# xianlopez/optical_flow

Measured on AMD Instinct MI355X. Metric: image-pairs/sec training, 384x512 batch=8 per GPU, higher is better.
Workload: dtype fp32

## Files before the change

include/oflow.h:

```cpp
#ifndef OFLOW_H
#define OFLOW_H

#include <stddef.h>
#include <stdint.h>

#ifdef __cplusplus
extern "C" {
#endif

#define OF_ABI_VERSION 1

enum { OF_OK = 0, OF_EINVAL = 1, OF_EHIP = 2, OF_EUNSUPPORTED = 3, OF_ETIMEOUT = 4 };
enum { OF_ACT_NONE = 0, OF_ACT_RELU = 1, OF_ACT_LEAKY = 2 };

typedef struct of_conv_desc {
  int32_t n, h, w;
  int32_t cin;
  int32_t cin_p;
  int32_t cout;
  int32_t kh, kw, stride;
  int32_t pad_top, pad_left;
  int32_t ho, wo;
} of_conv_desc;

int         of_abi_version(void);
const char* of_last_error(void);
int of_same_pads(int n, int k, int s, int* before, int* after, int* out);

int64_t of_conv_wfwd_elems(const of_conv_desc* d);
int64_t of_conv_wbwd_elems(const of_conv_desc* d);
int of_conv_pack_weights(const of_conv_desc* d, const float* w_hwio, float* w_fwd,
                         float* w_bwd, void* stream);

size_t of_conv_pack_table_bytes(int nconv);
int of_conv_pack_table(int nconv, const of_conv_desc* descs, const float* const* w_hwio,
                       float* const* w_fwd, float* const* w_bwd, void* host_table);
int of_conv_pack_many(const void* dev_table, int64_t total_work, void* stream);

size_t of_conv2d_fwd_workspace(const of_conv_desc* d);
int of_conv2d_fwd(const of_conv_desc* d, const float* x, int ldx, const float* w_fwd,
                  const float* bias, const float* bn_gamma, const float* bn_beta,
                  const float* bn_mean, const float* bn_var, float bn_eps,
                  const float* residual, int ldr, int act, float alpha,
                  float* z, int ldz, float* y, int ldy, void* workspace, size_t ws_bytes,
                  void* stream);


size_t of_conv2d_dgrad_workspace(const of_conv_desc* d);
int of_conv2d_dgrad(const of_conv_desc* d, const float* dy, int lddy, const float* w_bwd,
                    const float* act_src, int ld_act, int act, float alpha,
                    float* dx, int lddx, void* workspace, size_t ws_bytes, void* stream);

size_t of_conv2d_wgrad_workspace(const of_conv_desc* d);
int of_conv2d_wgrad(const of_conv_desc* d, const float* x, int ldx, const float* dy, int lddy,
                    float* dw, float* db, int accumulate, void* workspace, size_t ws_bytes,
                    void* stream);

int of_conv_path(const of_conv_desc* d);
int64_t of_conv_wfwd16_elems(const of_conv_desc* d);
int64_t of_conv_wbwd16_elems(const of_conv_desc* d);
int of_conv_pack_weights_bf16(const of_conv_desc* d, const float* w_hwio, void* w16_fwd,
                              void* w16_bwd, void* stream);
int of_conv_pack_table_ex(int nconv, const of_conv_desc* descs, const float* const* w_hwio,
                          void* const* w_fwd, void* const* w_bwd, const int* bf16,
                          void* host_table);
size_t of_conv2d_fwd_bf16_workspace(const of_conv_desc* d);
int of_conv2d_fwd_bf16(const of_conv_desc* d, const float* x, int ldx, const void* w16_fwd,
                       const float* bias, const float* bn_gamma, const float* bn_beta,
                       const float* bn_mean, const float* bn_var, float bn_eps,
                       const float* residual, int ldr, int act, float alpha, float* z, int ldz,
                       float* y, int ldy, void* workspace, size_t ws_bytes, void* stream);
size_t of_conv2d_wgrad_bf16_workspace(const of_conv_desc* d);
int of_conv2d_wgrad_bf16(const of_conv_desc* d, const float* x, int ldx, const float* dy,
                         int lddy, float* dw, float* db, int accumulate, void* workspace,
                         size_t ws_bytes, void* stream);
int of_conv2d_dgrad_add(const of_conv_desc* d, const float* dy, int lddy, const float* w_bwd,
                        const float* add, int ld_add, float* dx, int lddx, void* workspace,
                        size_t ws_bytes, void* stream);
int of_conv2d_dgrad_add_bf16(const of_conv_desc* d, const float* dy, int lddy,
                             const void* w16_bwd, const float* add, int ld_add, float* dx,
                             int lddx, void* workspace, size_t ws_bytes, void* stream);
size_t of_conv2d_dgrad_bf16_workspace(const of_conv_desc* d);
int of_conv2d_dgrad_bf16(const of_conv_desc* d, const float* dy, int lddy, const void* w16_bwd,
                         const float* act_src, int ld_act, int act, float alpha, float* dx,
                         int lddx, void* workspace, size_t ws_bytes, void* stream);

int of_conv_pack_weights_x3(const of_conv_desc* d, const float* w_hwio, void* w3_fwd,
                            void* w3_bwd, void* stream);
size_t of_conv2d_fwd_x3_workspace(const of_conv_desc* d);
size_t of_conv2d_dgrad_x3_workspace(const of_conv_desc* d);
int of_conv2d_fwd_x3(const of_conv_desc* d, const float* x, int ldx, const void* w3_fwd,
                     const float* bias, const float* bn_gamma, const float* bn_beta,
                     const float* bn_mean, const float* bn_var, float bn_eps,
                     const float* residual, int ldr, int act, float alpha, float* z, int ldz,
                     float* y, int ldy, void* workspace, size_t ws_bytes, void* stream);
int of_conv2d_dgrad_x3(const of_conv_desc* d, const float* dy, int lddy, const void* w3_bwd,
                       const float* act_src, int ld_act, int act, float alpha, float* dx,
                       int lddx, void* workspace, size_t ws_bytes, void* stream);
int of_conv2d_dgrad_add_x3(const of_conv_desc* d, const float* dy, int lddy,
                           const void* w3_bwd, const float* add, int ld_add, float* dx,
                           int lddx, void* workspace, size_t ws_bytes, void* stream);
size_t of_conv2d_wgrad_x3_workspace(const of_conv_desc* d);
int of_conv2d_wgrad_x3(const of_conv_desc* d, const float* x, int ldx, const float* dy,
                       int lddy, float* dw, float* db, int accumulate, void* workspace,
                       size_t ws_bytes, void* stream);

int of_act_bwd(const float* dy, const float* y, int act, float alpha, float* dz, int64_t n,
               void* stream);

size_t of_colsum_workspace(int64_t npix, int c);
int of_colsum(const float* x, int64_t npix, int c, int ld, float* out, int accumulate,
              void* workspace, void* stream);

size_t of_bn_act_bwd_workspace(int64_t npix, int c);
int of_bn_act_bwd(int64_t npix, int c, int act, const float* dy, const float* y,
                  const float* z, const float* gamma, const float* mean, const float* var,
                  float eps, float* dz, float* dres, float* dgamma, float* dbeta, float* dbias,
                  int accumulate, void* workspace, void* stream);
size_t of_maxpool_bn_act_bwd_workspace(int n, int h, int w, int c);
int of_maxpool_bn_act_bwd(int n, int h, int w, int c, const float* dyp, const float* g,
                          const float* y, const float* z, const float* gamma, const float* mean,
                          const float* var, float eps, float* dz, float* dgamma, float* dbeta,
                          float* dbias, int accumulate, void* workspace, void* stream);

int of_maxpool2_fwd(const float* x, int n, int h, int w, int c, float* y, void* stream);
int of_maxpool2_bwd(const float* x, const float* dy, int n, int h, int w, int c, float* dx,
                    void* stream);

size_t of_corr_fwd_workspace(int n, int h, int w, int c, int max_disp);
int of_corr_fwd(const float* f1, int ld1, const float* f2, int ld2, int n, int h, int w,
                int c, int max_disp, float* out, int ldo, void* workspace, size_t ws_bytes,
                void* stream);
int of_corr_bwd(const float* dcv, int lddcv, const float* f1, int ld1, const float* f2,
                int ld2, int n, int h, int w, int c, int max_disp, float* df1, int lddf1,
                int acc1, float* df2, int lddf2, int acc2, void* stream);
int of_corr_concat_fwd(const float* f1, const float* f2, const float* flow, int n, int h, int w,
                       int c, int max_disp, float* cat, int cp, void* workspace,
                       size_t ws_bytes, void* stream);
int of_corr_concat_fwd16(const float* f1, const float* f2, const float* flow, int n, int h,
                         int w, int c, int max_disp, void* cat16, int ld16, void* stream);
int of_corr_concat_fwd16_ok(int n, int h, int w, int c);
int of_corr_concat_bwd(const float* dcat, int cp, const float* f1, const float* f2, int n,
                       int h, int w, int c, int max_disp, float* df1, float* df2, float* dflow,
                       void* stream);

int of_warp_fwd(const float* inp, int n, int h, int w, int c, const float* flow, float* out,
                void* stream);
int of_warp_bwd(const float* dout, const float* inp, int n, int h, int w, int c,
                const float* flow, float* dinp, float* dflow, void* stream);
int of_warp_bwd_add(const float* dout, const float* inp, int n, int h, int w, int c,
                    const float* flow, float* dinp, float* dflow, const float* dflow_add,
                    int ld_add, void* stream);
int of_bilinear_fwd(const float* inp, int n, int h, int w, int c, const float* pts, float* out,
                    void* stream);
int of_bilinear_bwd(const float* dout, const float* inp, int n, int h, int w, int c,
                    const float* pts, float* dinp, float* dpts, void* stream);
size_t of_warp_bwd_det_workspace(int n, int h, int w, int c);
size_t of_warp_bwd_det_header(int n, int h, int w, int c);
int of_warp_bwd_det(const float* dout, const float* inp, int n, int h, int w, int c,
                    const float* flow, int absolute, float* dinp, float* dflow,
                    const float* dflow_add, int ld_add, void* workspace, size_t ws_bytes,
                    void* stream);

#define OF_WARP_REFERENCE 0
#define OF_WARP_IMAGE 1
int of_warp_fwd_cv(const float* inp, int n, int h, int w, int c, const float* flow, float* out,
                   int convention, void* stream);
int of_warp_bwd_cv(const float* dout, const float* inp, int n, int h, int w, int c,
                   const float* flow, float* dinp, float* dflow, const float* dflow_add,
                   int ld_add, int convention, void* stream);
int of_warp_bwd_det_cv(const float* dout, const float* inp, int n, int h, int w, int c,
                       const float* flow, float* dinp, float* dflow, const float* dflow_add,
                       int ld_add, int convention, void* workspace, size_t ws_bytes,
                       void* stream);

int of_upscale2x_fwd(const float* in, int n, int h, int w, int c, float scale, float* out,
                     int ldo, void* stream);
int of_upscale2x_bwd(const float* dout, int lddo, int n, int h, int w, int c, float scale,
                     float* din, int accumulate, void* stream);
int of_upscale2x_bwd_ld(const float* dout, int lddo, int n, int h, int w, int c, float scale,
                        float* din, int lddi, int accumulate, void* stream);

int of_pyramid6(const float* batch, int n, int h, int w, int levels, float* const* outs,
                void* stream);
int of_split_pair(const float* batch, int n, int h, int w, float* out, void* stream);

int of_photo_l1_partials(int n, int h, int w);
int of_photo_l1_fwd(const float* img6, const float* flow, int n, int h, int w,
                    float* partials, void* stream);
int of_photo_l1_bwd(const float* img6, const float* flow, int n, int h, int w, float coef,
                    const float* dloss, float* dflow, void* stream);
int of_photo_l1_bwd_ld(const float* img6, const float* flow, int n, int h, int w, float coef,
                       const float* dloss, float* dflow, int lddf, void* stream);
int of_photo_l1_fwd_multi(const float* const* img6s, const float* const* flows, int n,
                          const int* hs, const int* ws, int levels, float* partials,
                          void* stream);
int of_photo_l1_bwd_multi(const float* const* img6s, const float* const* flows, int n,
                          const int* hs, const int* ws, int levels, const float* coefs,
                          const float* dloss, float* const* dflows, const int* lds,
                          void* stream);
int of_photo_l1_fwd_multi_cv(const float* const* img6s, const float* const* flows, int n,
                             const int* hs, const int* ws, int levels, float* partials,
                             int convention, void* stream);
int of_photo_l1_bwd_multi_cv(const float* const* img6s, const float* const* flows, int n,
                             const int* hs, const int* ws, int levels, const float* coefs,
                             const float* dloss, float* const* dflows, const int* lds,
                             int convention, void* stream);
int of_sum_partials(const float* const* parts, const int* counts, const float* coefs,
                    int ngroups, float* out, void* stream);

int of_flow_smooth_partials(int n, int h, int w);
int of_flow_smooth_fwd_multi(const float* const* img6s, const float* const* flows, int n,
                             const int* hs, const int* ws, int levels, float edge_alpha,
                             float eps, const float* coefs_v, const float* coefs_h,
                             float* partials, void* stream);
int of_flow_smooth_bwd_multi(const float* const* img6s, const float* const* flows, int n,
                             const int* hs, const int* ws, int levels, float edge_alpha,
                             float eps, const float* coefs_v, const float* coefs_h,
                             const float* dloss, float* const* dflows, const int* lds,
                             int accumulate, void* stream);

int of_flow_smooth2_partials(int n, int h, int w);
int of_flow_smooth2_fwd_multi(const float* const* img6s, const float* const* flows, int n,
                              const int* hs, const int* ws, int levels, float edge_alpha,
                              float eps, const float* coefs_v, const float* coefs_h,
                              float* partials, void* stream);
int of_flow_smooth2_bwd_multi(const float* const* img6s, const float* const* flows, int n,
                              const int* hs, const int* ws, int levels, float edge_alpha,
                              float eps, const float* coefs_v, const float* coefs_h,
                              const float* dloss, float* const* dflows, const int* lds,
                              int accumulate, void* stream);

int of_census_partials(int n, int h, int w);
int of_census_workspace_floats(int n, int h, int w);
int of_census_fwd_multi(const float* const* img6s, const float* const* flows, int n,
                        const int* hs, const int* ws, int levels, int radius,
                        const float* coefs, float* const* workspaces, float* const* dcdfs,
                        float* partials, void* stream);
int of_census_fwd_multi_cv(const float* const* img6s, const float* const* flows, int n,
                           const int* hs, const int* ws, int levels, int radius,
                           const float* coefs, float* const* workspaces, float* const* dcdfs,
                           float* partials, int convention, void* stream);
int of_census_bwd_multi(const float* const* dcdfs, int n, const int* hs, const int* ws,
                        int levels, const float* coefs, const float* dloss,
                        float* const* dflows, const int* lds, int accumulate, void* stream);

#define OF_OCC_BORDER 1
#define OF_OCC_FB 2
int of_occ_mask_multi(const float* const* flows, int n, int pair_stride, const int* hs,
                      const int* ws, int levels, int mode, float alpha1, const float* alpha2s,
                      float* const* masks, void* stream);

int of_photo_l1_fwd_multi_w(const float* const* img6s, const float* const* flows,
                            const float* const* weights, int n, const int* hs, const int* ws,
                            int levels, float* partials, int convention, void* stream);
int of_photo_l1_bwd_multi_w(const float* const* img6s, const float* const* flows,
                            const float* const* weights, int n, const int* hs, const int* ws,
                            int levels, const float* coefs, const float* dloss,
                            float* const* dflows, const int* lds, int convention, void* stream);
int of_census_fwd_multi_w(const float* const* img6s, const float* const* flows,
                          const float* const* weights, int n, const int* hs, const int* ws,
                          int levels, int radius, const float* coefs, float* const* workspaces,
                          float* const* dcdfs, float* partials, int convention, void* stream);

int of_adam_keras(float* p, const float* g, float* m, float* v, int64_t n, float lr_t,
                  float beta1, float beta2, float eps, float gscale, void* stream);
int of_adam_keras_dev(float* p, const float* g, float* m, float* v, int64_t n, float* sched,
                      int32_t* iter, float beta1, float beta2, float eps, float gscale,
                      void* stream);

int of_grad_sumsq_partials(int64_t n);
int of_grad_sumsq(const float* g, int64_t n, double* partials, void* stream);
size_t of_adam_clip_state_bytes(void);
int of_adam_keras_dev_clip(float* p, const float* g, float* m, float* v, int64_t n, float* sched,
                           int32_t* iter, float beta1, float beta2, float eps, float grad_scale,
                           const double* partials, int npartials, float clip_norm,
                           int skip_nonfinite, void* state, void* stream);

int of_add_inplace(float* y, const float* x, int64_t n, void* stream);
int of_copy_strided(const float* src, int lds, float* dst, int ldd, int64_t npix, int c,
                    void* stream);
int of_fill(float* y, float v, int64_t n, void* stream);
int of_stream_wait(void* waiter, void* signaller);

int of_timing_enable(int on);
int of_set_tuning(int key, int value);
int of_timing_read(int max, int* kinds, double* flops, float* ms);

int of_to_bf16_image(const float* x, int64_t npix, int c, int ldx, void* y16, int ldo,
                     void* stream);
typedef struct of_b16i_io {
  const void* a16; int lda16;
  float* y; int ldy;
  void* y16; int ldy16;
  const float* aux; int ldr;
  const float* act_src; int ld_act;
  const void* act16; int ld_act16;
  float* col_part;
  void* mask_out;
  const void* mask_in;
} of_b16i_io;
int of_conv2d_b16i_tiles(int mode, const of_conv_desc* d);
size_t of_conv2d_b16i_mask_bytes(const of_conv_desc* d);
int of_conv2d_b16i(int mode, const of_conv_desc* d, const of_b16i_io* io, const void* w16,
                   const float* bias, const float* bn_gamma, const float* bn_beta,
                   const float* bn_mean, const float* bn_var, float bn_eps, int act, float alpha,
                   void* stream);
size_t of_conv2d_wgrad_b16i_workspace(const of_conv_desc* d);
int of_conv2d_wgrad_b16i(const of_conv_desc* d, const void* x16, int ldx16, const void* dy16,
                         int lddy16, float* dw, int accumulate, const float* bn_gamma,
                         const float* bn_var, float bn_eps, void* workspace, size_t ws_bytes,
                         void* stream);
int of_col_part_reduce(const float* part, int rows, int n, float* out, int accumulate,
                       void* stream);


typedef struct of_image_desc {
  int64_t offset;
  int32_t h, w;
} of_image_desc;

int of_png_info(const char* path, int* h, int* w, int* channels, int* depth);
int of_png_read_bgr(const char* path, uint8_t* out, int64_t cap, int* h, int* w);
int of_png_write(const char* path, const uint8_t* img, int h, int w, int c, int flags);
int of_png_scan(int n, const char* const* paths, int nthreads, int* max_h, int* max_w);

typedef struct of_reader of_reader;
int of_reader_create(int npairs, const char* const* path1, const char* const* path2, int batch,
                     int nworkers, int nslots, int max_h, int max_w, uint64_t seed, int pinned,
                     of_reader** out);
int64_t of_reader_raw_bytes(const of_reader* r);
int of_reader_nbatches(const of_reader* r);
int of_reader_next(of_reader* r, void* dev_raw, int64_t cap, float* out, int out_h, int out_w,
                   int32_t* pair_index, int32_t* swapped, void* stream);
int of_reader_next_host(of_reader* r, void* dst, int64_t cap, int32_t* pair_index,
                        int32_t* swapped);
int of_reader_destroy(of_reader* r);

int of_preprocess_pairs(const void* dev_raw, int npairs, int out_h, int out_w, float* out,
                        void* stream);

typedef struct of_augment {
  float m[6];
  float gain[3];
  float brightness;
  float contrast;
  float saturation;
  int32_t flags;
  int32_t pad[3];
} of_augment;
int of_augment_pairs(const void* dev_raw, int npairs, int out_h, int out_w,
                     const of_augment* dev_params, float* out, void* stream);
int of_reader_next_aug(of_reader* r, void* dev_raw, int64_t cap, const of_augment* host_params,
                       of_augment* dev_params, float* out, int out_h, int out_w,
                       int32_t* pair_index, int32_t* swapped, void* stream);


int of_png_read_u16(const char* path, uint16_t* out, int64_t cap, int* h, int* w);
int of_png_write_u16(const char* path, const uint16_t* rgb, int h, int w, int flags);

typedef struct of_flow_eval_result {
// ... 104 lines not shown
```

optical_flow_amd/_lib.py:

```python
from __future__ import annotations

import ctypes as C
import os
import threading

HERE = os.path.dirname(os.path.abspath(__file__))
LIB_PATH = os.environ.get("OFLOW_LIB") or os.path.join(HERE, "liboflow.so")

OF_OK, OF_EINVAL, OF_EHIP, OF_EUNSUPPORTED, OF_ETIMEOUT = 0, 1, 2, 3, 4
OF_REDUCE_SUM, OF_REDUCE_AVG = 0, 1
ACT_NONE, ACT_RELU, ACT_LEAKY = 0, 1, 2
WARP_REFERENCE, WARP_IMAGE = 0, 1
OCC_BORDER, OCC_FB = 1, 2


class B16iIO(C.Structure):
    _fields_ = [("a16", C.c_void_p), ("lda16", C.c_int), ("y", C.c_void_p), ("ldy", C.c_int),
                ("y16", C.c_void_p), ("ldy16", C.c_int), ("aux", C.c_void_p), ("ldr", C.c_int),
                ("act_src", C.c_void_p), ("ld_act", C.c_int), ("act16", C.c_void_p),
                ("ld_act16", C.c_int), ("col_part", C.c_void_p), ("mask_out", C.c_void_p),
                ("mask_in", C.c_void_p)]


class ConvDesc(C.Structure):
    _fields_ = [(n, C.c_int32) for n in
                ("n", "h", "w", "cin", "cin_p", "cout", "kh", "kw", "stride", "pad_top",
                 "pad_left", "ho", "wo")]


P = C.c_void_p
I = C.c_int
I64 = C.c_int64
F = C.c_float
SZ = C.c_size_t
PD = C.POINTER(ConvDesc)

PROTOTYPES = {
    "of_abi_version": (I, []),
    "of_last_error": (C.c_char_p, []),
    "of_same_pads": (I, [I, I, I, C.POINTER(I), C.POINTER(I), C.POINTER(I)]),
    "of_conv_wfwd_elems": (I64, [PD]),
    "of_conv_wbwd_elems": (I64, [PD]),
    "of_conv_pack_weights": (I, [PD, P, P, P, P]),
    "of_conv_pack_table_bytes": (SZ, [I]),
    "of_conv_pack_table": (I, [I, PD, C.POINTER(P), C.POINTER(P), C.POINTER(P), P]),
    "of_conv_pack_many": (I, [P, I64, P]),
    "of_conv2d_fwd_workspace": (SZ, [PD]),
    "of_conv2d_fwd": (I, [PD, P, I, P, P, P, P, P, P, F, P, I, I, F, P, I, P, I, P, SZ, P]),
    "of_conv2d_dgrad_workspace": (SZ, [PD]),
    "of_conv2d_dgrad": (I, [PD, P, I, P, P, I, I, F, P, I, P, SZ, P]),
    "of_conv2d_wgrad_workspace": (SZ, [PD]),
    "of_conv2d_wgrad": (I, [PD, P, I, P, I, P, P, I, P, SZ, P]),
    "of_conv_path": (I, [PD]),
    "of_conv_wfwd16_elems": (I64, [PD]),
    "of_conv_wbwd16_elems": (I64, [PD]),
    "of_conv_pack_weights_bf16": (I, [PD, P, P, P, P]),
    "of_conv_pack_table_ex": (I, [I, PD, C.POINTER(P), C.POINTER(P), C.POINTER(P),
                                  C.POINTER(I), P]),
    "of_conv2d_fwd_bf16_workspace": (SZ, [PD]),
    "of_conv2d_fwd_bf16": (I, [PD, P, I, P, P, P, P, P, P, F, P, I, I, F, P, I, P, I, P, SZ, P]),
    "of_conv2d_wgrad_bf16_workspace": (SZ, [PD]),
    "of_conv2d_wgrad_bf16": (I, [PD, P, I, P, I, P, P, I, P, SZ, P]),
    "of_conv2d_dgrad_bf16_workspace": (SZ, [PD]),
    "of_conv2d_dgrad_bf16": (I, [PD, P, I, P, P, I, I, F, P, I, P, SZ, P]),
    "of_conv2d_dgrad_add": (I, [PD, P, I, P, P, I, P, I, P, SZ, P]),
    "of_conv2d_dgrad_add_bf16": (I, [PD, P, I, P, P, I, P, I, P, SZ, P]),
    "of_conv_pack_weights_x3": (I, [PD, P, P, P, P]),
    "of_conv2d_fwd_x3_workspace": (SZ, [PD]),
    "of_conv2d_dgrad_x3_workspace": (SZ, [PD]),
    "of_conv2d_fwd_x3": (I, [PD, P, I, P, P, P, P, P, P, F, P, I, I, F, P, I, P, I, P, SZ, P]),
    "of_conv2d_dgrad_x3": (I, [PD, P, I, P, P, I, I, F, P, I, P, SZ, P]),
    "of_conv2d_dgrad_add_x3": (I, [PD, P, I, P, P, I, P, I, P, SZ, P]),
    "of_conv2d_wgrad_x3_workspace": (SZ, [PD]),
    "of_conv2d_wgrad_x3": (I, [PD, P, I, P, I, P, P, I, P, SZ, P]),
    "of_act_bwd": (I, [P, P, I, F, P, I64, P]),
    "of_colsum_workspace": (SZ, [I64, I]),
    "of_colsum": (I, [P, I64, I, I, P, I, P, P]),
    "of_bn_act_bwd_workspace": (SZ, [I64, I]),
    "of_bn_act_bwd": (I, [I64, I, I, P, P, P, P, P, P, F, P, P, P, P, P, I, P, P]),
    "of_min_abs_segments": (I, [P, P, I, P, P]),
    "of_maxpool_bn_act_bwd_workspace": (SZ, [I, I, I, I]),
    "of_maxpool_bn_act_bwd": (I, [I, I, I, I, P, P, P, P, P, P, P, F, P, P, P, P, I, P, P]),
    "of_maxpool2_fwd": (I, [P, I, I, I, I, P, P]),
    "of_maxpool2_bwd": (I, [P, P, I, I, I, I, P, P]),
    "of_corr_fwd_workspace": (SZ, [I, I, I, I, I]),
    "of_corr_fwd": (I, [P, I, P, I, I, I, I, I, I, P, I, P, SZ, P]),
    "of_corr_bwd": (I, [P, I, P, I, P, I, I, I, I, I, I, P, I, I, P, I, I, P]),
    "of_corr_concat_fwd": (I, [P, P, P, I, I, I, I, I, P, I, P, SZ, P]),
    "of_corr_concat_bwd": (I, [P, I, P, P, I, I, I, I, I, P, P, P, P]),
    "of_corr_concat_fwd16": (I, [P, P, P, I, I, I, I, I, P, I, P]),
    "of_corr_concat_fwd16_ok": (I, [I, I, I, I]),
    "of_warp_fwd": (I, [P, I, I, I, I, P, P, P]),
    "of_warp_bwd": (I, [P, P, I, I, I, I, P, P, P, P]),
    "of_warp_bwd_add": (I, [P, P, I, I, I, I, P, P, P, P, I, P]),
    "of_bilinear_fwd": (I, [P, I, I, I, I, P, P, P]),
    "of_bilinear_bwd": (I, [P, P, I, I, I, I, P, P, P, P]),
    "of_to_bf16_image": (I, [P, I64, I, I, P, I, P]),
    "of_conv2d_b16i_tiles": (I, [I, PD]),
    "of_conv2d_b16i_mask_bytes": (SZ, [PD]),
    "of_conv2d_b16i": (I, [I, PD, P, P, P, P, P, P, P, F, I, F, P]),
    "of_col_part_reduce": (I, [P, I, I, P, I, P]),
    "of_conv2d_wgrad_b16i_workspace": (SZ, [PD]),
    "of_conv2d_wgrad_b16i": (I, [PD, P, I, P, I, P, I, P, P, F, P, SZ, P]),
    "of_warp_bwd_det_workspace": (SZ, [I, I, I, I]),
    "of_warp_bwd_det_header": (SZ, [I, I, I, I]),
    "of_warp_bwd_det": (I, [P, P, I, I, I, I, P, I, P, P, P, I, P, SZ, P]),
    "of_warp_fwd_cv": (I, [P, I, I, I, I, P, P, I, P]),
    "of_warp_bwd_cv": (I, [P, P, I, I, I, I, P, P, P, P, I, I, P]),
    "of_warp_bwd_det_cv": (I, [P, P, I, I, I, I, P, P, P, P, I, I, P, SZ, P]),
    "of_upscale2x_fwd": (I, [P, I, I, I, I, F, P, I, P]),
    "of_upscale2x_bwd": (I, [P, I, I, I, I, I, F, P, I, P]),
    "of_upscale2x_bwd_ld": (I, [P, I, I, I, I, I, F, P, I, I, P]),
    "of_pyramid6": (I, [P, I, I, I, I, C.POINTER(P), P]),
    "of_split_pair": (I, [P, I, I, I, P, P]),
    "of_photo_l1_partials": (I, [I, I, I]),
    "of_photo_l1_fwd": (I, [P, P, I, I, I, P, P]),
    "of_photo_l1_bwd": (I, [P, P, I, I, I, F, P, P, P]),
    "of_photo_l1_bwd_ld": (I, [P, P, I, I, I, F, P, P, I, P]),
    "of_sum_partials": (I, [C.POINTER(P), C.POINTER(I), C.POINTER(F), I, P, P]),
    "of_adam_keras": (I, [P, P, P, P, I64, F, F, F, F, F, P]),
    "of_adam_keras_dev": (I, [P, P, P, P, I64, P, P, F, F, F, F, P]),
    "of_grad_sumsq_partials": (I, [I64]),
    "of_grad_sumsq": (I, [P, I64, P, P]),
    "of_adam_clip_state_bytes": (SZ, []),
    "of_adam_keras_dev_clip": (I, [P, P, P, P, I64, P, P, F, F, F, F, P, I, F, I, P, P]),
    "of_add_inplace": (I, [P, P, I64, P]),
    "of_copy_strided": (I, [P, I, P, I, I64, I, P]),
    "of_fill": (I, [P, F, I64, P]),
    "of_stream_wait": (I, [P, P]),
    "of_timing_enable": (I, [I]),
    "of_set_tuning": (I, [I, I]),
    "of_timing_read": (I, [I, C.POINTER(I), C.POINTER(C.c_double), C.POINTER(F)]),
    "of_png_info": (I, [C.c_char_p, C.POINTER(I), C.POINTER(I), C.POINTER(I), C.POINTER(I)]),
    "of_png_read_bgr": (I, [C.c_char_p, P, I64, C.POINTER(I), C.POINTER(I)]),
    "of_png_write": (I, [C.c_char_p, P, I, I, I, I]),
    "of_png_scan": (I, [I, C.POINTER(C.c_char_p), I, C.POINTER(I), C.POINTER(I)]),
    "of_reader_create": (I, [I, C.POINTER(C.c_char_p), C.POINTER(C.c_char_p), I, I, I, I, I,
                             C.c_uint64, I, C.POINTER(P)]),
    "of_reader_raw_bytes": (I64, [P]),
    "of_reader_nbatches": (I, [P]),
    "of_reader_next": (I, [P, P, I64, P, I, I, C.POINTER(C.c_int32), C.POINTER(C.c_int32), P]),
    "of_reader_next_host": (I, [P, P, I64, C.POINTER(C.c_int32), C.POINTER(C.c_int32)]),
    "of_reader_destroy": (I, [P]),
    "of_preprocess_pairs": (I, [P, I, I, I, P, P]),
    "of_augment_pairs": (I, [P, I, I, I, P, P, P]),
    "of_reader_next_aug": (I, [P, P, I64, P, P, P, I, I, C.POINTER(C.c_int32),
                               C.POINTER(C.c_int32), P]),
    "of_png_read_u16": (I, [C.c_char_p, P, I64, C.POINTER(I), C.POINTER(I)]),
    "of_png_write_u16": (I, [C.c_char_p, P, I, I, I]),
    "of_flow_eval_partials": (I, [I, I, I]),
    "of_flow_eval": (I, [P, I, I, I, P, P, I64, P, I, P, P]),
    "of_flow_upsample": (I, [P, I, I, I, I, I, P, P]),
    "of_flow_color": (I, [P, I, I, I, P, P, P]),
    "of_flow_intensity": (I, [P, I64, P, P]),
    "of_crc32c": (C.c_uint32, [P, I64, C.c_uint32]),
    "of_conv_pack_weights_bn": (I, [PD, I, P, P, P, P, P, F, P]),
    "of_conv_pack_table_bn": (I, [I, PD, C.POINTER(P), C.POINTER(P), C.POINTER(P), C.POINTER(I),
                                  C.POINTER(P), C.POINTER(P), F, P]),
    "of_conv2d_wgrad_bn_workspace": (SZ, [PD, I]),
    "of_conv2d_wgrad_bn": (I, [PD, I, P, I, P, I, P, I, P, P, F, P, SZ, P]),
    "of_conv2d_dgrad_add_act": (I, [PD, I, P, I, P, P, I, P, I, I, F, P, I, P, SZ, P]),
    "of_conv2d_dgrad_bnp_bytes": (SZ, [PD]),
    "of_conv2d_dgrad_add_act_bnp": (I, [PD, I, P, I, P, P, I, P, I, I, F, P, I, P, P, P, I, P,
                                        SZ, P, P, SZ, P]),
    "of_bn_bwd_final": (I, [P, I, I, P, P, F, P, P, P, I, P]),
    "of_bn_bwd_reduce": (I, [I64, I, I, P, P, P, P, P, P, F, P, P, P, P, I, P, P]),
    "of_maxpool_bn_relu_bwd": (I, [I, I, I, I, P, P, P, P, P, P, F, P, P, P, P, I, P, P]),
    "of_conv2d_fwd_pool": (I, [PD, I, P, I, P, P, P, P, P, P, F, I, F, P, I, P, I, P, P, SZ, P]),
    "of_photo_l1_fwd_multi": (I, [C.POINTER(P), C.POINTER(P), I, C.POINTER(I), C.POINTER(I), I, P,
                                  P]),
    "of_photo_l1_bwd_multi": (I, [C.POINTER(P), C.POINTER(P), I, C.POINTER(I), C.POINTER(I), I,
                                  C.POINTER(F), P, C.POINTER(P), C.POINTER(I), P]),
    "of_photo_l1_fwd_multi_cv": (I, [C.POINTER(P), C.POINTER(P), I, C.POINTER(I), C.POINTER(I), I,
                                     P, I, P]),
    "of_photo_l1_bwd_multi_cv": (I, [C.POINTER(P), C.POINTER(P), I, C.POINTER(I), C.POINTER(I), I,
                                     C.POINTER(F), P, C.POINTER(P), C.POINTER(I), I, P]),
    "of_flow_smooth_partials": (I, [I, I, I]),
    "of_flow_smooth_fwd_multi": (I, [C.POINTER(P), C.POINTER(P), I, C.POINTER(I), C.POINTER(I), I,
                                     F, F, C.POINTER(F), C.POINTER(F), P, P]),
    "of_flow_smooth_bwd_multi": (I, [C.POINTER(P), C.POINTER(P), I, C.POINTER(I), C.POINTER(I), I,
                                     F, F, C.POINTER(F), C.POINTER(F), P, C.POINTER(P),
                                     C.POINTER(I), I, P]),
    "of_flow_smooth2_partials": (I, [I, I, I]),
    "of_flow_smooth2_fwd_multi": (I, [C.POINTER(P), C.POINTER(P), I, C.POINTER(I), C.POINTER(I), I,
                                      F, F, C.POINTER(F), C.POINTER(F), P, P]),
    "of_flow_smooth2_bwd_multi": (I, [C.POINTER(P), C.POINTER(P), I, C.POINTER(I), C.POINTER(I), I,
                                      F, F, C.POINTER(F), C.POINTER(F), P, C.POINTER(P),
                                      C.POINTER(I), I, P]),
    "of_census_partials": (I, [I, I, I]),
    "of_census_workspace_floats": (I, [I, I, I]),
    "of_census_fwd_multi": (I, [C.POINTER(P), C.POINTER(P), I, C.POINTER(I), C.POINTER(I), I, I,
                                C.POINTER(F), C.POINTER(P), C.POINTER(P), P, P]),
    "of_census_fwd_multi_cv": (I, [C.POINTER(P), C.POINTER(P), I, C.POINTER(I), C.POINTER(I), I, I,
                                   C.POINTER(F), C.POINTER(P), C.POINTER(P), P, I, P]),
    "of_census_bwd_multi": (I, [C.POINTER(P), I, C.POINTER(I), C.POINTER(I), I, C.POINTER(F), P,
                                C.POINTER(P), C.POINTER(I), I, P]),
    "of_occ_mask_multi": (I, [C.POINTER(P), I, I, C.POINTER(I), C.POINTER(I), I, I, F,
                              C.POINTER(F), C.POINTER(P), P]),
    "of_photo_l1_fwd_multi_w": (I, [C.POINTER(P), C.POINTER(P), C.POINTER(P), I, C.POINTER(I),
                                    C.POINTER(I), I, P, I, P]),
    "of_photo_l1_bwd_multi_w": (I, [C.POINTER(P), C.POINTER(P), C.POINTER(P), I, C.POINTER(I),
                                    C.POINTER(I), I, C.POINTER(F), P, C.POINTER(P), C.POINTER(I),
                                    I, P]),
    "of_census_fwd_multi_w": (I, [C.POINTER(P), C.POINTER(P), C.POINTER(P), I, C.POINTER(I),
                                  C.POINTER(I), I, I, C.POINTER(F), C.POINTER(P), C.POINTER(P), P,
                                  I, P]),
    "of_stem_bwd_fused_workspace": (SZ, [PD, I]),
    "of_stem_bwd_fused": (I, [PD, I, P, I, P, P, P, P, P, P, F, P, P, P, P, I, P, SZ, P]),
    "of_bn_train_workspace": (SZ, [I64, I, I]),
    "of_bn_train_stats": (I, [I64, I, I, P, F, F, P, P, P, P, P, P]),
    "of_bn_train_apply": (I, [I64, I, I, P, P, P, P, P, P, I, P, P]),
    "of_bn_train_bwd": (I, [I64, I, I, I, P, P, P, P, P, P, P, P, P, P, I, P, P]),
    "of_comm_id_bytes": (I, []),
    "of_comm_get_unique_id": (I, [P]),
    "of_comm_probe": (I, []),
    "of_comm_init": (I, [C.POINTER(P), P, I, I]),
    "of_comm_init_timeout": (I, [C.POINTER(P), P, I, I, C.c_double]),
    "of_comm_info": (I, [P, C.POINTER(I), C.POINTER(I), C.POINTER(I)]),
    "of_comm_allreduce_async": (I, [P, P, P, I64, P]),
    "of_comm_allreduce_ex_async": (I, [P, P, P, I64, I, P]),
    "of_comm_async_error": (I, [P]),
    "of_comm_abort": (I, [P]),
    "of_comm_destroy": (I, [P, I]),
}


class OflowError(RuntimeError):
    pass


class OflowTimeout(OflowError):
    """OF_ETIMEOUT: a collective setup or wait passed its deadline (and was aborted)."""


_lib = None
_lock = threading.Lock()


def load(path: str = LIB_PATH):
    global _lib
    with _lock:
        if _lib is not None:
            return _lib
        if not os.path.exists(path):
            raise OflowError("liboflow.so not found at %s: run `python -m optical_flow_amd.build` "
                             "(the HIP path has no fallback)" % path)
        lib = C.CDLL(path)
        for name, (res, args) in PROTOTYPES.items():
            fn = getattr(lib, name)
            fn.restype = res
            fn.argtypes = args
        if lib.of_abi_version() != 1:
            raise OflowError("liboflow ABI mismatch")
        for kv in filter(None, os.environ.get("OFLOW_TUNE", "").split(",")):
            k, v = kv.split("=")
            if lib.of_set_tuning(int(k), int(v)) != OF_OK:
                raise OflowError("OFLOW_TUNE: " + lib.of_last_error().decode(errors="replace"))
        _lib = lib
        return lib


def lib():
    return _lib if _lib is not None else load()


def check(status: int, what: str = ""):
    if status != OF_OK:
        msg = lib().of_last_error().decode(errors="replace")
        if status == OF_EINVAL:
            raise AssertionError("%s: %s" % (what, msg))
        if status == OF_ETIMEOUT:
            raise OflowTimeout("%s timed out: %s" % (what, msg))
        raise OflowError("%s failed (%d): %s" % (what, status, msg))


def call(name: str, *args):
    st = getattr(lib(), name)(*args)
    check(st, name)
    return st
```

optical_flow_amd/csrc/conv_f32.hip:

```cpp
#include "common.h"
#include "conv_dev.h"
#include "conv_narrow.h"

#include <algorithm>

namespace oflow {

template <int BM, int BN, int WAVES_M, int WAVES_N, int MODE>
__global__ __launch_bounds__(256, 2) void conv_gemm_f32(GemmArgs a) {
  constexpr int WM = BM / WAVES_M, WN = BN / WAVES_N;
  constexpr int TM = WM / 32, TN = WN / 32;
  static_assert(WAVES_M * WAVES_N == 4, "4 waves");
  static_assert(TM >= 1 && TN >= 1 && WM % 32 == 0 && WN % 32 == 0, "tile");
  constexpr bool A_KCONTIG = (MODE != MODE_WGRAD);
  constexpr int SA = BM + 4;
  constexpr int SB = BN + 4;
  constexpr int A_SLOTS = BM * BK / 4 / 256;
  constexpr int B_QUADS = BK * BN / 4;
  constexpr int B_SLOTS = (B_QUADS + 255) / 256;
  static_assert(A_SLOTS >= 1, "BM >= 64");

  static_assert(2 * BK * (SA + SB) >= 4 * 1024, "epilogue images fit LDS");
  __shared__ float smem[2 * BK * (SA + SB)];
  float (*As)[BK * SA] = reinterpret_cast<float (*)[BK * SA]>(smem);
// ... 723 lines not shown
  const int trem = tile_m - b * tiles_x * tiles_y;
  const int oy0 = (trem / tiles_x) * TH, ox0 = (trem % tiles_x) * TF_W;
  const int hy0 = MODE == MODE_FWD ? oy0 - a.pt : oy0 + a.pt - (KS - 1);
  const int hx0 = MODE == MODE_FWD ? ox0 - a.pl : ox0 + a.pl - (KS - 1);
  const int c_begin = split * a.k_per_split;
  const int c_end = min(a.K, c_begin + a.k_per_split);
  const int steps = c_end > c_begin ? (c_end - c_begin) * KS : 0;

  const rsrc_t ra_src = make_rsrc(a.A, a.a_bytes);
  const rsrc_t rb_src = make_rsrc(a.B, a.b_bytes);

  int h_off[HS];
  unsigned h_ok = 0;
  const int hcq = tid & 7;
#pragma unroll
  for (int j = 0; j < HS; ++j) {
    const int q = tid + NT * j;
    const int hp = q >> 3;
    const int sy = hy0 + hp / HW, sx = hx0 + hp % HW;
    const bool ok = q < HQ && (unsigned)sy < (unsigned)SH && (unsigned)sx < (unsigned)SW;
    h_off[j] = ok ? (((b * SH + sy) * SW + sx) * a.lda + 4 * hcq) * 4 : 0;
    h_ok |= (ok ? 1u : 0u) << j;
  }
  float4 hv[HS];
  auto load_halo = [&](int c) {
    const bool cok = 32 * c + 4 * hcq < a.kc;
#pragma unroll
    for (int j = 0; j < HS; ++j)
      hv[j] = bload4(ra_src, cok && ((h_ok >> j) & 1) ? (uint32_t)(h_off[j] + 128 * c) : kOOB);
  };
  auto store_halo = [&]() {
#pragma unroll
    for (int j = 0; j < HS; ++j) {
      const int q = tid + NT * j;
      if (q < HQ) {
        bf16x8 t;
        const float4 v = hv[j];
        typedef __bf16 bf16x4 __attribute__((ext_vector_type(4)));
        bf16x4 u;
        u[0] = (__bf16)v.x;
        u[1] = (__bf16)v.y;
        u[2] = (__bf16)v.z;
        u[3] = (__bf16)v.w;
        (void)t;
        *reinterpret_cast<bf16x4*>(reinterpret_cast<char*>(Ah) + (q >> 3) * (SROW16 * 16) +
                                   8 * (q & 7)) = u;
      }
    }
  };
  uint4 rb[BSL];
  auto load_b = [&](int c, int r) {
#pragma unroll
    for (int j = 0; j < BSL; ++j) {
      const int o = tid + NT * j;
      const int s = o / (BN * 4), rem = o - s * (BN * 4);
      const int n = n0 + (rem >> 2), oct = rem & 3;
      const bool ok = o < BOCT && n < a.nb;
      const int k = (r * KS + s) * a.kc + 32 * c + 8 * oct;
      rb[j] = __builtin_bit_cast(uint4,
                                 bload4(rb_src, ok ? (uint32_t)(((int64_t)n * a.ldb + k) * 2) : kOOB));
    }
  };
  auto store_b = [&](int buf) {
#pragma unroll
    for (int j = 0; j < BSL; ++j) {
      const int o = tid + NT * j;
      if (o < BOCT) {
        const int s = o / (BN * 4), rem = o - s * (BN * 4);
        Bs[buf][(s * BN + (rem >> 2)) * SROW16 + (rem & 3)] = rb[j];
      }
    }
  };

  f32x16 acc[TM][TN];
#pragma unroll
  for (int i = 0; i < TM; ++i)
#pragma unroll
    for (int j = 0; j < TN; ++j)
#pragma unroll
      for (int r = 0; r < 16; ++r) acc[i][j][r] = 0.f;
  const int wm0 = (wave / WAVES_N) * WM;
  const int wn0 = (wave % WAVES_N) * WN;
  const int lrow = lane & 31, lk = lane >> 5;
  int a_hp[TM];
#pragma unroll
  for (int i = 0; i < TM; ++i) {
    const int m = wm0 + 32 * i + lrow;
    const int ty = m / TF_W, tx = m % TF_W;
    a_hp[i] = MODE == MODE_FWD ? ty * HW + tx : (ty + KS - 1) * HW + tx + KS - 1;
  }

  if (steps > 0) {
    load_halo(c_begin);
    load_b(c_begin, 0);
    store_halo();
    store_b(0);
  }
  __syncthreads();
  for (int q = 0; q < steps; ++q) {
    const int r = q % KS, buf = q & 1;
    const bool more = q + 1 < steps;
    const int nq = q + 1;
    const int nc = c_begin + nq / KS, nr = nq % KS;
    if (more) load_b(nc, nr);
    if (r == 0 && q + KS < steps) load_halo(c_begin + q / KS + 1);
    auto frags = [&](int k, bf16x8 (&av)[TM], bf16x8 (&bv)[TN]) {
      const int s = k >> 1, st = k & 1;
      const int dh = MODE == MODE_FWD ? r * HW + s : -(r * HW + s);
#pragma unroll
      for (int i = 0; i < TM; ++i)
        av[i] = __builtin_bit_cast(bf16x8, Ah[(a_hp[i] + dh) * SROW16 + 2 * st + lk]);
#pragma unroll
      for (int j = 0; j < TN; ++j)
        bv[j] = __builtin_bit_cast(
            bf16x8, Bs[buf][(s * BN + wn0 + 32 * j + lrow) * SROW16 + 2 * st + lk]);
    };
    if (g_tile16_pf_dev) {
      bf16x8 av[2][TM], bv[2][TN];
      frags(0, av[0], bv[0]);
#pragma unroll
      for (int k = 0; k < 2 * KS; ++k) {
        const int cur = k & 1;
        if (k + 1 < 2 * KS) frags(k + 1, av[cur ^ 1], bv[cur ^ 1]);
        __builtin_amdgcn_sched_barrier(0);
#pragma unroll
        for (int i = 0; i < TM; ++i)
#pragma unroll
          for (int j = 0; j < TN; ++j)
            acc[i][j] = __builtin_amdgcn_mfma_f32_32x32x16_bf16(av[cur][i], bv[cur][j], acc[i][j],
                                                                0, 0, 0);
        __builtin_amdgcn_sched_barrier(0);
      }
    } else {
#pragma unroll
      for (int k = 0; k < 2 * KS; ++k) {
        bf16x8 av[TM], bv[TN];
        frags(k, av, bv);
#pragma unroll
        for (int i = 0; i < TM; ++i)
#pragma unroll
          for (int j = 0; j < TN; ++j)
            acc[i][j] = __builtin_amdgcn_mfma_f32_32x32x16_bf16(av[i], bv[j], acc[i][j], 0, 0, 0);
      }
    }
    if (more && nr == 0) __syncthreads();
    if (more) {
      store_b(buf ^ 1);
      if (nr == 0) store_halo();
    }
    __syncthreads();
  }

  const int64_t img = (int64_t)b * OH * OW;
  if (a.vec_ep && !EPC_BATCH) {
    float* E = reinterpret_cast<float*>(smem) + wave * 1024;
#pragma unroll
    for (int i = 0; i < TM; ++i)
#pragma unroll
      for (int j = 0; j < TN; ++j)
        transpose32(E, acc[i][j], lane, [&](int row, int c4, float4 v) {
          const int mt = wm0 + 32 * i + row, n = n0 + wn0 + 32 * j + 4 * c4;
          const int oy = oy0 + mt / TF_W, ox = ox0 + mt % TF_W;
          if (oy < OH && ox < OW && n < a.N)
            epilogue_store4<MODE>(a, split, img + (int64_t)oy * OW + ox, n, v);
        });
    return;
  }
  if (MODE == MODE_DGRAD && a.vec_ep && a.bnp != nullptr) {
    float* E = reinterpret_cast<float*>(smem) + wave * 1024;
    const int c4 = lane & 7;
    float4 bsb[TN], bsg[TN], bt[TN], ig[TN];
#pragma unroll
    for (int j = 0; j < TN; ++j) {
      bsb[j] = bsg[j] = bt[j] = ig[j] = make_float4(0.f, 0.f, 0.f, 0.f);
      const int n = n0 + wn0 + 32 * j + 4 * c4;
      if (n < a.N) {
        bt[j] = *reinterpret_cast<const float4*>(&a.bnp_b[n]);
        const float4 gm = *reinterpret_cast<const float4*>(&a.bnp_g[n]);
        ig[j] = make_float4(1.f / gm.x, 1.f / gm.y, 1.f / gm.z, 1.f / gm.w);
      }
    }
#pragma unroll
    for (int i = 0; i < TM; ++i)
#pragma unroll
      for (int j = 0; j < TN; ++j) {
        float4 vv[4];
        int64_t rows[4];
        unsigned ok = 0;
        int ncol = 0;
        transpose32(E, acc[i][j], lane, [&](int row, int c4r, float4 v) {
          const int q = row >> 3;
          const int mt = wm0 + 32 * i + row, n = n0 + wn0 + 32 * j + 4 * c4r;
          const int oy = oy0 + mt / TF_W, ox = ox0 + mt % TF_W;
          rows[q] = img + (int64_t)min(oy, OH - 1) * OW + min(ox, OW - 1);
          ok |= (oy < OH && ox < OW && n < a.N ? 1u : 0u) << q;
          vv[q] = v;
          ncol = n;
        });
        dgrad_rows4c_bnp<4>(a, rows, ok, ncol, min(ncol, a.N - 4), vv, bt[j], ig[j], bsb[j], bsg[j]);
      }
#pragma unroll
    for (int j = 0; j < TN; ++j)
#pragma unroll
      for (int o = 8; o < 64; o <<= 1) {
        bsb[j].x += __shfl_xor(bsb[j].x, o, 64), bsb[j].y += __shfl_xor(bsb[j].y, o, 64);
        bsb[j].z += __shfl_xor(bsb[j].z, o, 64), bsb[j].w += __shfl_xor(bsb[j].w, o, 64);
        bsg[j].x += __shfl_xor(bsg[j].x, o, 64), bsg[j].y += __shfl_xor(bsg[j].y, o, 64);
        bsg[j].z += __shfl_xor(bsg[j].z, o, 64), bsg[j].w += __shfl_xor(bsg[j].w, o, 64);
      }
    __syncthreads();
    float4* red = reinterpret_cast<float4*>(smem);
    const int wmi = wave / WAVES_N;
    if (lane < 8) {
#pragma unroll
      for (int j = 0; j < TN; ++j) {
        const int lq = (wn0 + 32 * j) / 4 + c4;
        red[wmi * (BN / 4) + lq] = bsb[j];
        red[(WAVES_M + wmi) * (BN / 4) + lq] = bsg[j];
      }
    }
    __syncthreads();
    if (tid < BN / 4 && n0 + 4 * tid < a.N) {
      float4 sb = red[tid], sg = red[WAVES_M * (BN / 4) + tid];
      for (int w2 = 1; w2 < WAVES_M; ++w2) {
        add4(sb, red[w2 * (BN / 4) + tid]);
        add4(sg, red[(WAVES_M + w2) * (BN / 4) + tid]);
      }
      float* prow = a.bnp + (int64_t)tile_m * 2 * a.N + n0 + 4 * tid;
      *reinterpret_cast<float4*>(prow) = sb;
      *reinterpret_cast<float4*>(prow + a.N) = sg;
    }
    return;
  }
  if (a.vec_ep) {
    float* E = reinterpret_cast<float*>(smem) + wave * 1024;
#pragma unroll
    for (int i = 0; i < TM; ++i)
#pragma unroll
      for (int j = 0; j < TN; ++j) {
        float4 vv[4];
        int64_t rows[4];
        unsigned ok = 0;
        int ncol = 0;
        transpose32(E, acc[i][j], lane, [&](int row, int c4, float4 v) {
          const int q = row >> 3;
          const int mt = wm0 + 32 * i + row, n = n0 + wn0 + 32 * j + 4 * c4;
          const int oy = oy0 + mt / TF_W, ox = ox0 + mt % TF_W;
          rows[q] = img + (int64_t)min(oy, OH - 1) * OW + min(ox, OW - 1);
          ok |= (oy < OH && ox < OW && n < a.N ? 1u : 0u) << q;
          vv[q] = v;
          ncol = n;
        });
        epilogue_rows4c<MODE, 4>(a, split, rows, ok, ncol, min(ncol, a.N - 4), vv);
      }
    return;
  }
#pragma unroll
  for (int j = 0; j < TN; ++j) {
    const int n = n0 + wn0 + 32 * j + lrow;
    if (n >= a.N) continue;
    float bias = 0.f, scale = 1.f, shift = 0.f;
    if (a.splits == 1) column_params<MODE>(a, n, bias, scale, shift);
#pragma unroll
    for (int i = 0; i < TM; ++i) {
      EpAux aux[16];
#pragma unroll
      for (int rr = 0; rr < 16; ++rr) {
        const int m = wm0 + 32 * i + (rr & 3) + 8 * (rr >> 2) + 4 * lk;
        const int oy = oy0 + m / TF_W, ox = ox0 + m % TF_W;
        aux[rr] = a.splits == 1 && oy < OH && ox < OW
                      ? epilogue_aux<MODE>(a, img + (int64_t)oy * OW + ox, n) : EpAux{0.f, 0.f};
      }
#pragma unroll
      for (int rr = 0; rr < 16; ++rr) {
        const int m = wm0 + 32 * i + (rr & 3) + 8 * (rr >> 2) + 4 * lk;
        const int oy = oy0 + m / TF_W, ox = ox0 + m % TF_W;
        if (oy >= OH || ox >= OW) continue;
        const int64_t row = img + (int64_t)oy * OW + ox;
        if (a.splits > 1)
          a.slab[(int64_t)split * a.split_stride + row * a.slab_ld + n] = acc[i][j][rr];
        else
          epilogue_store<MODE>(a, row, n, acc[i][j][rr], bias, scale, shift, aux[rr]);
      }
    }
  }
}

__device__ __forceinline__ void split3x4(const float4& v, uint2& h, uint2& m, uint2& l) {
  const float x[4] = {v.x, v.y, v.z, v.w};
  uint32_t hb[4], mb[4], lb[4];
#pragma unroll
  for (int e = 0; e < 4; ++e) {
    hb[e] = __float_as_uint(x[e]) & 0xffff0000u;
    const float r = x[e] - __uint_as_float(hb[e]);
    mb[e] = __float_as_uint(r) & 0xffff0000u;
    lb[e] = __float_as_uint(r - __uint_as_float(mb[e]));
  }
  auto hi2 = [](uint32_t e0, uint32_t e1) { return __builtin_amdgcn_perm(e1, e0, 0x07060302u); };
  h = make_uint2(hi2(hb[0], hb[1]), hi2(hb[2], hb[3]));
  m = make_uint2(hi2(mb[0], mb[1]), hi2(mb[2], mb[3]));
  l = make_uint2(hi2(lb[0], lb[1]), hi2(lb[2], lb[3]));
}

template <int BN, int WAVES_M, int WAVES_N, int MODE, int TH, int NB, int NP>
__device__ __forceinline__ void tile_x3_body(const GemmArgs& a) {
  constexpr int BM = TH * TF_W, KS = 3;
  static_assert(NP == 1 || NP == 3, "planes");
  constexpr int HH = TH + KS - 1, HW = TF_W + KS - 1, HP = HH * HW;
  constexpr int WM = BM / WAVES_M, WN = BN / WAVES_N;
  constexpr int SM = WM / 16, SN = WN / 16;
  constexpr int NT = 64 * WAVES_M * WAVES_N;
  static_assert(NT % 64 == 0 && NT <= 1024 && WM % 16 == 0 && WN % 16 == 0 && SM >= 1 && SN >= 1,
                "tile");
  constexpr int HQ = HP * 8, HS = (HQ + NT - 1) / NT;
  constexpr int BOCT = NP * BN * 4, BSL = (BOCT + NT - 1) / NT;
  constexpr int AH_U4 = NP * HP * 4, BS_U4 = NB * NP * BN * 4;
  constexpr int EP1_U4 = (NT / 64) * WM * 16 * 4 / 16;
  constexpr int SM_U4 = AH_U4 + BS_U4 > EP1_U4 ? AH_U4 + BS_U4 : EP1_U4;
  constexpr int LDS_B = SM_U4 * 16;
  constexpr int EJ = (NT / 64) * WM * 16 * SN * 4 <= LDS_B ? SN
                     : (NT / 64) * WM * 8 * SN * 4 <= LDS_B ? SN / 2 : 1;
  constexpr int EPW = 16 * EJ;
  static_assert(SN % EJ == 0 && (NT / 64) * WM * EPW * 4 <= LDS_B, "epilogue image fits LDS");
  __shared__ uint4 smem[SM_U4];
  uint4* Ah = smem;
  uint4* Bs = smem + AH_U4;

  const int tid = threadIdx.x;
  const int lane = tid & 63;
  const int wave = __builtin_amdgcn_readfirstlane(tid >> 6);
  const int wgid = xcd_remap(blockIdx.x, gridDim.x);
  const int split = wgid / a.tiles_total;
  const int tile = wgid - split * a.tiles_total;
  const int tile_n = tile % a.n_tiles;
  const int tile_m = tile / a.n_tiles;
  const int n0 = tile_n * BN;
  const int OH = MODE == MODE_FWD ? a.ho : a.h, OW = MODE == MODE_FWD ? a.wo : a.w;
  const int SH = MODE == MODE_FWD ? a.h : a.ho, SW = MODE == MODE_FWD ? a.w : a.wo;
  const int tiles_x = (OW + TF_W - 1) / TF_W, tiles_y = (OH + TH - 1) / TH;
  const int b = tile_m / (tiles_x * tiles_y);
  const int trem = tile_m - b * tiles_x * tiles_y;
  const int oy0 = (trem / tiles_x) * TH, ox0 = (trem % tiles_x) * TF_W;
  const int hy0 = MODE == MODE_FWD ? oy0 - a.pt : oy0 + a.pt - (KS - 1);
  const int hx0 = MODE == MODE_FWD ? ox0 - a.pl : ox0 + a.pl - (KS - 1);
  const int c_begin = split * a.k_per_split;
  const int c_end = min(a.K, c_begin + a.k_per_split);

  const rsrc_t ra_src = make_rsrc(a.A, a.a_bytes);
  const rsrc_t rb_src = make_rsrc(a.B, a.b_bytes);

  float4 hv[HS];
  constexpr bool HREC = X3_HREC && NT == 256 && NP == 3;
  int h_off[HREC ? 1 : HS];
  unsigned h_ok = 0;
  const int hcq = tid & 7;
  auto halo_slot = [&](int t, int j, bool& ok) {
    const int q = t + NT * j;
    const int hp = q >> 3;
    const int sy = hy0 + hp / HW, sx = hx0 + hp % HW;
    ok = q < HQ && (unsigned)sy < (unsigned)SH && (unsigned)sx < (unsigned)SW;
    return ok ? (((b * SH + sy) * SW + sx) * a.lda + 4 * (t & 7)) * 4 : 0;
  };
  if constexpr (!HREC) {
#pragma unroll
    for (int j = 0; j < HS; ++j) {
      bool ok;
      h_off[j] = halo_slot(tid, j, ok);
      h_ok |= (ok ? 1u : 0u) << j;
    }
  }
  auto load_halo = [&](int c) {
    const bool cok = 32 * c + 4 * hcq < a.kc;
    if constexpr (HREC) {
      int t = tid;
      asm volatile("" : "+v"(t));
#pragma unroll
      for (int j = 0; j < HS; ++j) {
        bool ok;
        const int off = halo_slot(t, j, ok);
        hv[j] = bload4(ra_src, cok && ok ? (uint32_t)(off + 128 * c) : kOOB);
      }
    } else {
#pragma unroll
      for (int jj = 0; jj < HS; ++jj)
        hv[jj] = bload4(ra_src, cok && ((h_ok >> jj) & 1) ? (uint32_t)(h_off[jj] + 128 * c) : kOOB);
    }
  };
  auto store_halo = [&]() {
#pragma unroll
    for (int j = 0; j < HS; ++j) {
      const int q = tid + NT * j;
      if (q < HQ) {
        const int hp = q >> 3;
        const int off = hp * 64 + ((((q & 7) >> 1) ^ x3_sw(hp)) << 4) + 8 * (q & 1);
        char* base = reinterpret_cast<char*>(Ah);
        if constexpr (NP == 1) {
          *reinterpret_cast<uint2*>(base + off) = pack_bf16x4(hv[j]);
        } else {
          uint2 h, m, l;
          split3x4(hv[j], h, m, l);
          *reinterpret_cast<uint2*>(base + off) = h;
          *reinterpret_cast<uint2*>(base + HP * 64 + off) = m;
          *reinterpret_cast<uint2*>(base + 2 * HP * 64 + off) = l;
        }
      }
    }
  };
  uint32_t b_off[BSL];
  int b_lds[BSL];
#pragma unroll
  for (int j = 0; j < BSL; ++j) {
    const int o = tid + NT * j;
    const int p = o / (BN * 4), rem = o - p * (BN * 4);
    const int row = rem >> 2, oct = rem & 3;
    const int n = n0 + row;
    const bool ok = o < BOCT && n < a.nb;
    b_off[j] = ok ? (uint32_t)(((int64_t)p * a.b_plane + (int64_t)n * a.ldb + 8 * oct) * 2) : kOOB;
    b_lds[j] = o < BOCT ? (p * BN + row) * 4 + (oct ^ x3_sw(row)) : -1;
  }
  uint4 rb[BSL];
  auto load_b = [&](int c, int t) {
    const int so = (t * a.kc + 32 * c) * 2;
#pragma unroll
    for (int j = 0; j < BSL; ++j)
      rb[j] = __builtin_bit_cast(uint4, __builtin_amdgcn_raw_buffer_load_b128(rb_src, b_off[j], so, 0));
  };
  auto store_b = [&](int buf) {
#pragma unroll
    for (int j = 0; j < BSL; ++j)
      if (BOCT % NT == 0 || b_lds[j] >= 0) Bs[buf * NP * BN * 4 + b_lds[j]] = rb[j];
  };
  constexpr bool BDMA = X3_BDMA && NB == 2;
  constexpr int NW = NT / 64, BDI = NP * BN / 16, BDW = (BDI + NW - 1) / NW;
  uint32_t bd_off[BDW];
  int bd_lds[BDW];
#pragma unroll
  for (int k = 0; k < BDW; ++k) {
    const int g = wave + NW * k;
    const int p = g / (BN / 16), rbk = g % (BN / 16);
    const int n = rbk * 16 + (lane >> 2), o = (lane & 3) ^ x3_sw(lane >> 2);
    bd_off[k] = g < BDI && n0 + n < a.nb
                    ? (uint32_t)(((int64_t)p * a.b_plane + (int64_t)(n0 + n) * a.ldb + 8 * o) * 2)
                    : kOOB;
    bd_lds[k] = g < BDI ? (p * BN + rbk * 16) * 4 : -1;
  }
  auto dma_b = [&](int c, int t, int buf) {
    const int so = (t * a.kc + 32 * c) * 2;
#pragma unroll
    for (int k = 0; k < BDW; ++k)
      if (BDI % NW == 0 || bd_lds[k] >= 0)
        dma16_to_lds(rb_src, Bs + buf * NP * BN * 4 + bd_lds[k], bd_off[k], so);
  };

  f32x4 acc4[SM][SN];
#pragma unroll
  for (int i = 0; i < SM; ++i)
#pragma unroll
    for (int j = 0; j < SN; ++j)
#pragma unroll
      for (int r = 0; r < 4; ++r) acc4[i][j][r] = 0.f;
  const int wm0 = (wave / WAVES_N) * WM;
  const int wn0 = (wave % WAVES_N) * WN;
  const int l16 = lane & 15, lq = lane >> 4;
  int a_hp16[SM];
#pragma unroll
  for (int i = 0; i < SM; ++i) {
    const int m = wm0 + 16 * i + l16;
    const int ty = m / TF_W, tx = m % TF_W;
    a_hp16[i] = MODE == MODE_FWD ? ty * HW + tx : (ty + KS - 1) * HW + tx + KS - 1;
  }
  const int b_frag = (wn0 + l16) * 4 + (lq ^ x3_sw(l16));

  if (c_end > c_begin) {
    load_halo(c_begin);
    if constexpr (BDMA) dma_b(c_begin, 0, 0);
    else load_b(c_begin, 0);
    store_halo();
    if constexpr (!BDMA) store_b(0);
  }
  if constexpr (BDMA) asm volatile("s_waitcnt vmcnt(0)" ::: "memory");
  __syncthreads();
  for (int c = c_begin; c < c_end; ++c) {
    const int cc = c - c_begin;
    const bool more_c = c + 1 < c_end;
    if (more_c && !(X3_ABL & 4)) load_halo(c + 1);
#pragma unroll
    for (int t = 0; t < KS * KS; ++t) {
      const int buf = NB == 2 ? (cc + t) & 1 : 0;
      const bool more = t + 1 < KS * KS || more_c;
      if (more && !(X3_ABL & 2)) {
        if constexpr (BDMA) dma_b(t + 1 < KS * KS ? c : c + 1, t + 1 < KS * KS ? t + 1 : 0, buf ^ 1);
        else load_b(t + 1 < KS * KS ? c : c + 1, t + 1 < KS * KS ? t + 1 : 0);
      }
      __builtin_amdgcn_sched_barrier(0);
      const int r = t / KS, s = t % KS;
      const int dh = MODE == MODE_FWD ? r * HW + s : -(r * HW + s);
      bf16x8 av[NP][SM], bv[NP][SN];
#pragma unroll
      for (int i = 0; i < SM; ++i) {
        const int px = a_hp16[i] + dh;
        const int ai = px * 4 + (lq ^ x3_sw(px));
#pragma unroll
        for (int p = 0; p < NP; ++p) av[p][i] = __builtin_bit_cast(bf16x8, Ah[p * HP * 4 + ai]);
      }
#pragma unroll
      for (int p = 0; p < NP; ++p)
#pragma unroll
        for (int j = 0; j < SN; ++j)
          bv[p][j] = __builtin_bit_cast(bf16x8, Bs[(buf * NP + p) * BN * 4 + 64 * j + b_frag]);
#pragma unroll
      for (int i = 0; i < SM; ++i)
#pragma unroll
        for (int j = 0; j < SN; ++j) {
          f32x4 x = acc4[i][j];
          if constexpr (NP == 1) {
            acc4[i][j] = __builtin_amdgcn_mfma_f32_16x16x32_bf16(av[0][i], bv[0][j], x, 0, 0, 0);
            continue;
          } else {
          if (X3_ABL & 8) {
            asm volatile("" ::"v"(av[1][i]), "v"(av[2][i]), "v"(bv[1][j]), "v"(bv[2][j]));
            acc4[i][j] = __builtin_amdgcn_mfma_f32_16x16x32_bf16(av[0][i], bv[0][j], x, 0, 0, 0);
            continue;
          }
          x = __builtin_amdgcn_mfma_f32_16x16x32_bf16(av[2][i], bv[0][j], x, 0, 0, 0);
          x = __builtin_amdgcn_mfma_f32_16x16x32_bf16(av[0][i], bv[2][j], x, 0, 0, 0);
          x = __builtin_amdgcn_mfma_f32_16x16x32_bf16(av[1][i], bv[1][j], x, 0, 0, 0);
          x = __builtin_amdgcn_mfma_f32_16x16x32_bf16(av[1][i], bv[0][j], x, 0, 0, 0);
          x = __builtin_amdgcn_mfma_f32_16x16x32_bf16(av[0][i], bv[1][j], x, 0, 0, 0);
          acc4[i][j] = __builtin_amdgcn_mfma_f32_16x16x32_bf16(av[0][i], bv[0][j], x, 0, 0, 0);
          }
        }
      __builtin_amdgcn_sched_barrier(0);
      if (!(X3_ABL & 1) && (NB == 1 ? more : (t + 1 == KS * KS && more_c))) __syncthreads();
      if (more) {
        if (!(X3_ABL & 2) && !BDMA) store_b(NB == 2 ? buf ^ 1 : 0);
        if (t + 1 == KS * KS && more_c && !(X3_ABL & 4)) store_halo();
      }
      if constexpr (BDMA) asm volatile("s_waitcnt vmcnt(0)" ::: "memory");
      if (!(X3_ABL & 1)) __syncthreads();
    }
  }

  const int64_t img = (int64_t)b * OH * OW;
  if constexpr (X3_ABL & 16) {
    float v = 0.f;
#pragma unroll
    for (int i = 0; i < SM; ++i)
#pragma unroll
      for (int j = 0; j < SN; ++j) v += acc4[i][j][0] + acc4[i][j][1] + acc4[i][j][2] + acc4[i][j][3];
    a.C[(img + (int64_t)oy0 * OW + ox0) * a.ldc + (n0 + wn0 + (lane & 31)) % a.N] = v;
    return;
  }
  if constexpr (MODE == MODE_FWD && SM % 2 == 0 &&
                (NT / 64) * (WM / 2) * (WN * 4 + 32) <= LDS_B &&
                ((WM / 2) * (WN / 4)) % 64 == 0) {
    if (a.direct16) {
      direct_fwd_f32<SM, SN, WM, WN, TF_W>(
          a, acc4, reinterpret_cast<char*>(smem) + wave * (WM / 2) * (WN * 4 + 32), lane, wm0,
          wn0, n0, oy0, ox0, OH, OW, img);
      return;
    }
  }
  if constexpr (MODE == MODE_DGRAD && NT >= 512 && SM % 2 == 0 &&
                (NT / 64) * (WM / 2) * (WN * 4 + 32) <= LDS_B &&
                ((WM / 2) * (WN / 4)) % 64 == 0) {
    if (a.direct16) {
      direct_dgrad_f32<SM, SN, WM, WN, TF_W>(
          a, acc4, reinterpret_cast<char*>(smem) + wave * (WM / 2) * (WN * 4 + 32), lane, wm0,
          wn0, n0, oy0, ox0, OH, OW, img);
      return;
    }
  }
  if (a.vec_ep) {
    float* E = reinterpret_cast<float*>(smem) + wave * WM * EPW;
    constexpr int LPR = 4 * EJ, RPI = 64 / LPR;
    const int c4 = lane % LPR, rr = lane / LPR;
    constexpr int NPASS = SN / EJ;
    const bool bnp = MODE == MODE_DGRAD && a.bnp != nullptr;
    float4 bsb[NPASS], bsg[NPASS];
#pragma unroll
    for (int p = 0; p < NPASS; ++p) bsb[p] = bsg[p] = make_float4(0.f, 0.f, 0.f, 0.f);
#pragma unroll
    for (int jp = 0; jp < SN; jp += EJ) {
#pragma unroll
      for (int i = 0; i < SM; ++i)
#pragma unroll
        for (int j = 0; j < EJ; ++j)
#pragma unroll
          for (int r = 0; r < 4; ++r)
            E[(16 * i + 4 * lq + r) * EPW + 16 * j + l16] = acc4[i][jp + j][r];
      __builtin_amdgcn_fence(__ATOMIC_RELEASE, "wavefront");
      __builtin_amdgcn_wave_barrier();
      __builtin_amdgcn_fence(__ATOMIC_ACQUIRE, "wavefront");
      const int n = n0 + wn0 + 16 * jp + 4 * c4;
      if constexpr (X3_EPB > 1 && (WM / RPI) % X3_EPB == 0) {
#pragma unroll
        for (int q0 = 0; q0 < WM / RPI; q0 += X3_EPB) {
          float4 v[X3_EPB];
          int64_t row[X3_EPB];
          unsigned ok = 0;
#pragma unroll
          for (int g = 0; g < X3_EPB; ++g) {
            const int m = (q0 + g) * RPI + rr;
            v[g] = *reinterpret_cast<const float4*>(&E[m * EPW + 4 * c4]);
            const int mt = wm0 + m;
            const int oy = oy0 + mt / TF_W, ox = ox0 + mt % TF_W;
            row[g] = img + (int64_t)min(oy, OH - 1) * OW + min(ox, OW - 1);
            ok |= (oy < OH && ox < OW && n < a.N ? 1u : 0u) << g;
          }
          epilogue_rows4c<MODE, X3_EPB>(a, split, row, ok, n, min(n, a.N - 4), v);
        }
      } else if (MODE == MODE_DGRAD && bnp) {
        float4 bt = make_float4(0.f, 0.f, 0.f, 0.f), ig = bt;
        if (n < a.N) {
          bt = *reinterpret_cast<const float4*>(&a.bnp_b[n]);
          const float4 gm = *reinterpret_cast<const float4*>(&a.bnp_g[n]);
          ig = make_float4(1.f / gm.x, 1.f / gm.y, 1.f / gm.z, 1.f / gm.w);
        }
#pragma unroll
        for (int q = 0; q < WM / RPI; ++q) {
          const int m = q * RPI + rr;
          const float4 v = *reinterpret_cast<const float4*>(&E[m * EPW + 4 * c4]);
          const int mt = wm0 + m;
          const int oy = oy0 + mt / TF_W, ox = ox0 + mt % TF_W;
          if (oy < OH && ox < OW && n < a.N)
            dgrad_store4_bnp(a, img + (int64_t)oy * OW + ox, n, v, bt, ig, bsb[jp / EJ],
                             bsg[jp / EJ]);
        }
      } else {
#pragma unroll
        for (int q = 0; q < WM / RPI; ++q) {
          const int m = q * RPI + rr;
          const float4 v = *reinterpret_cast<const float4*>(&E[m * EPW + 4 * c4]);
          const int mt = wm0 + m;
          const int oy = oy0 + mt / TF_W, ox = ox0 + mt % TF_W;
          if (oy < OH && ox < OW && n < a.N)
            epilogue_store4<MODE>(a, split, img + (int64_t)oy * OW + ox, n, v);
        }
      }
      __builtin_amdgcn_fence(__ATOMIC_RELEASE, "wavefront");
      __builtin_amdgcn_wave_barrier();
      __builtin_amdgcn_fence(__ATOMIC_ACQUIRE, "wavefront");
    }
    if (MODE == MODE_DGRAD && bnp) {
      constexpr int NWM = (NT / 64) / WAVES_N;
#pragma unroll
      for (int p = 0; p < NPASS; ++p)
#pragma unroll
        for (int o = LPR; o < 64; o <<= 1) {
          bsb[p].x += __shfl_xor(bsb[p].x, o, 64), bsb[p].y += __shfl_xor(bsb[p].y, o, 64);
          bsb[p].z += __shfl_xor(bsb[p].z, o, 64), bsb[p].w += __shfl_xor(bsb[p].w, o, 64);
          bsg[p].x += __shfl_xor(bsg[p].x, o, 64), bsg[p].y += __shfl_xor(bsg[p].y, o, 64);
          bsg[p].z += __shfl_xor(bsg[p].z, o, 64), bsg[p].w += __shfl_xor(bsg[p].w, o, 64);
        }
      __syncthreads();
      float4* red = reinterpret_cast<float4*>(smem);
      const int wmi = wave / WAVES_N;
      if (rr == 0) {
#pragma unroll
        for (int p = 0; p < NPASS; ++p) {
          const int lq = (wn0 + 16 * EJ * p) / 4 + c4;
          red[wmi * (BN / 4) + lq] = bsb[p];
          red[(NWM + wmi) * (BN / 4) + lq] = bsg[p];
        }
      }
      __syncthreads();
      const int tid = threadIdx.x;
      if (tid < BN / 4 && n0 + 4 * tid < a.N) {
        float4 sb = red[tid], sg = red[NWM * (BN / 4) + tid];
        for (int w2 = 1; w2 < NWM; ++w2) {
          add4(sb, red[w2 * (BN / 4) + tid]);
          add4(sg, red[(NWM + w2) * (BN / 4) + tid]);
        }
        float* prow = a.bnp + (int64_t)tile_m * 2 * a.N + n0 + 4 * tid;
        *reinterpret_cast<float4*>(prow) = sb;
        *reinterpret_cast<float4*>(prow + a.N) = sg;
      }
    }
    return;
  }
#pragma unroll
  for (int j = 0; j < SN; ++j) {
    const int n = n0 + wn0 + 16 * j + l16;
    if (n >= a.N) continue;
    float bias = 0.f, scale = 1.f, shift = 0.f;
    if (a.splits == 1) column_params<MODE>(a, n, bias, scale, shift);
    EpAux aux[SM * 4];
#pragma unroll
    for (int q = 0; q < SM * 4; ++q) {
      const int m = wm0 + 16 * (q >> 2) + 4 * lq + (q & 3);
      const int oy = oy0 + m / TF_W, ox = ox0 + m % TF_W;
      aux[q] = a.splits == 1 && oy < OH && ox < OW
                   ? epilogue_aux<MODE>(a, img + (int64_t)oy * OW + ox, n) : EpAux{0.f, 0.f};
    }
#pragma unroll
    for (int q = 0; q < SM * 4; ++q) {
      const int m = wm0 + 16 * (q >> 2) + 4 * lq + (q & 3);
      const int oy = oy0 + m / TF_W, ox = ox0 + m % TF_W;
      if (oy >= OH || ox >= OW) continue;
      const int64_t row = img + (int64_t)oy * OW + ox;
      const float v = acc4[q >> 2][j][q & 3];
      if (a.splits > 1)
        a.slab[(int64_t)split * a.split_stride + row * a.slab_ld + n] = v;
      else
        epilogue_store<MODE>(a, row, n, v, bias, scale, shift, aux[q]);
    }
  }
}

template <int BN, int WAVES_M, int WAVES_N, int MODE, int TH, int NB = 2>
__global__ __launch_bounds__(64 * WAVES_M * WAVES_N, NB == 1 ? 2 : 1) void conv_tile_x3(GemmArgs a) {
  tile_x3_body<BN, WAVES_M, WAVES_N, MODE, TH, NB, 3>(a);
}

constexpr int b16_min_waves(int w, int acc) { return w <= 8 && acc <= 48 ? (w + 1) / 2 : (w + 3) / 4; }
template <int BN, int WAVES_M, int WAVES_N, int MODE, int TH>
__global__ __launch_bounds__(64 * WAVES_M * WAVES_N,
                             b16_min_waves(WAVES_M * WAVES_N,
                                           (TH * TF_W / WAVES_M / 16) * (BN / WAVES_N / 16) * 4))
void conv_tile_b16(GemmArgs a) {
  tile_x3_body<BN, WAVES_M, WAVES_N, MODE, TH, 2, 1>(a);
}

constexpr int ST_TH = 8, ST_TW = 32;
constexpr int ST_HH = 2 * ST_TH + 5, ST_HW = 2 * ST_TW + 6, ST_HWP = 72;
constexpr int ST_BROW = 232;

template <int CO, int NP = 3>
__global__ __launch_bounds__(CO * 8, CO == 64 ? 1 : NP == 1 ? 4 : 2) void conv_stem_x3(GemmArgs a, int ntiles) {
  constexpr int SM = 4, SN = 2, WM = 64, WN = 32, NW = CO / 8, NT = 64 * NW;
  static_assert(NP == 3 || NP == 1, "three split planes (fp32) or one (bf16)");
  constexpr int B_U4 = CO * ST_BROW / 8;
  constexpr int HWP = ST_HW;
  constexpr int H_PIX = ST_HH * HWP;
  constexpr int HB_U4 = NP * H_PIX / 2, EP_U4 = NW * WM * WN * 4 / 16;
  constexpr int W_U4 = HB_U4 > EP_U4 ? HB_U4 : EP_U4;
  __shared__ uint4 smem[NP * B_U4 + W_U4];
  char* Bs = reinterpret_cast<char*>(smem);
  char* Hs = reinterpret_cast<char*>(smem + NP * B_U4);

  const int tid = threadIdx.x, lane = tid & 63;
  const int wave = __builtin_amdgcn_readfirstlane(tid >> 6);
  constexpr int GROUPS = 64 / CO;
  const int wgid0 = xcd_remap(blockIdx.x, gridDim.x);
  const int co0 = (wgid0 % GROUPS) * CO;
  const int tstride = gridDim.x / GROUPS;
  const int tiles_x = (a.wo + ST_TW - 1) / ST_TW, tiles_y = (a.ho + ST_TH - 1) / ST_TH;
  int t = wgid0 / GROUPS;
  if (t >= ntiles) return;

  constexpr int BE = NP * CO * 28, BQ = (BE + NT - 1) / NT;
  constexpr int HE = ST_HH * ST_HW, HQ = (HE + NT - 1) / NT;
  const rsrc_t rb = make_rsrc(a.B, a.b_bytes);
  const rsrc_t ra = make_rsrc(a.A, a.a_bytes);
  float4 hv[HQ];
  auto load_halo = [&](int tt) {
    const int b = tt / (tiles_x * tiles_y);
    const int trem = tt - b * tiles_x * tiles_y;
    const int iy0 = 2 * ((trem / tiles_x) * ST_TH) - a.pt, ix0 = 2 * ((trem % tiles_x) * ST_TW) - a.pl;
#pragma unroll
    for (int k = 0; k < HQ; ++k) {
      const int q = tid + NT * k;
      const int hy = q / ST_HW, hx = q - hy * ST_HW;
      const int iy = iy0 + hy, ix = ix0 + hx;
      const bool ok = q < HE && (unsigned)iy < (unsigned)a.h && (unsigned)ix < (unsigned)a.w;
      hv[k] = bload4(ra, ok ? (uint32_t)((((int64_t)b * a.h + iy) * a.w + ix) * a.lda * 4) : kOOB);
    }
  };
  auto store_halo = [&]() {
#pragma unroll
    for (int k = 0; k < HQ; ++k) {
      const int q = tid + NT * k;
      if (HE % NT == 0 || q < HE) {
        const int hy = q / ST_HW, hx = q - hy * ST_HW;
        const int o = (hy * HWP + hx) * 8;
        if (NP == 1) {
          *reinterpret_cast<uint2*>(Hs + o) = pack_bf16x4(hv[k]);
        } else {
          uint2 h, m, l;
          split3x4(hv[k], h, m, l);
          *reinterpret_cast<uint2*>(Hs + o) = h;
          *reinterpret_cast<uint2*>(Hs + H_PIX * 8 + o) = m;
          *reinterpret_cast<uint2*>(Hs + 2 * H_PIX * 8 + o) = l;
        }
      }
    }
  };
  {
    uint2 blo[BQ], bhi[BQ];
#pragma unroll
    for (int k = 0; k < BQ; ++k) {
      const int e = tid + NT * k;
      const int p = e / (CO * 28), rem = e - p * (CO * 28);
      const int co = rem / 28, rs = rem - co * 28, r = rs >> 2, sp = rs & 3;
      const uint32_t src =
          (uint32_t)((p * a.b_plane + (int64_t)(co0 + co) * a.ldb + (r * 7 + 2 * sp) * 4) * 2);
      const bool ok = e < BE && co0 + co < a.nb;
      blo[k] = __builtin_bit_cast(uint2, __builtin_amdgcn_raw_buffer_load_b64(rb, ok ? src : kOOB, 0, 0));
      bhi[k] = __builtin_bit_cast(uint2, __builtin_amdgcn_raw_buffer_load_b64(rb, ok && sp < 3 ? src + 8 : kOOB, 0, 0));
    }
    load_halo(t);
#pragma unroll
    for (int k = 0; k < BQ; ++k) {
      const int e = tid + NT * k;
      if (BE % NT == 0 || e < BE) {
        const int p = e / (CO * 28), rem = e - p * (CO * 28);
        const int co = rem / 28, rs = rem - co * 28, r = rs >> 2, sp = rs & 3;
        *reinterpret_cast<uint4*>(Bs + ((p * CO + co) * ST_BROW + r * 32 + sp * 8) * 2) =
            make_uint4(blo[k].x, blo[k].y, bhi[k].x, bhi[k].y);
      }
    }
  }

  const int wm = CO == 64 ? wave >> 1 : wave, wn = CO == 64 ? wave & 1 : 0;
  const int l16 = lane & 15, sp = lane >> 4;
  int a_off[SM];
#pragma unroll
  for (int i = 0; i < SM; ++i)
    a_off[i] = ((2 * (2 * wm + (i >> 1))) * HWP + 2 * (16 * (i & 1) + l16) + 2 * sp) * 8;
  const int b_off = ((wn * WN + l16) * ST_BROW + sp * 8) * 2;
  constexpr int EPW = 32, LPR = 8, RPI = 8;
  float* E = reinterpret_cast<float*>(smem + NP * B_U4) + wave * WM * EPW;
  const int lq = lane >> 4;
  const int c4 = lane % LPR, rr = lane / LPR;
  const int n = co0 + wn * WN + 4 * c4;

  for (; t < ntiles; t += tstride) {
    const int b = t / (tiles_x * tiles_y);
    const int trem = t - b * tiles_x * tiles_y;
    const int oy0 = (trem / tiles_x) * ST_TH, ox0 = (trem % tiles_x) * ST_TW;
    store_halo();
    __syncthreads();
    if (t + tstride < ntiles) load_halo(t + tstride);

    f32x4 acc4[SM][SN];
#pragma unroll
    for (int i = 0; i < SM; ++i)
#pragma unroll
      for (int j = 0; j < SN; ++j)
#pragma unroll
        for (int r = 0; r < 4; ++r) acc4[i][j][r] = 0.f;
#pragma unroll
    for (int r = 0; r < 7; ++r) {
      bf16x8 av[NP][SM], bv[NP][SN];
#pragma unroll
      for (int p = 0; p < NP; ++p) {
#pragma unroll
        for (int i = 0; i < SM; ++i)
          av[p][i] = *reinterpret_cast<const bf16x8*>(Hs + p * H_PIX * 8 + a_off[i] + r * HWP * 8);
#pragma unroll
        for (int j = 0; j < SN; ++j)
          bv[p][j] = *reinterpret_cast<const bf16x8*>(Bs + p * B_U4 * 16 + b_off + (16 * j * ST_BROW + r * 32) * 2);
      }
#pragma unroll
      for (int i = 0; i < SM; ++i)
#pragma unroll
        for (int j = 0; j < SN; ++j) {
          f32x4 x = acc4[i][j];
          if (NP == 3) {
            x = __builtin_amdgcn_mfma_f32_16x16x32_bf16(av[NP - 1][i], bv[0][j], x, 0, 0, 0);
            x = __builtin_amdgcn_mfma_f32_16x16x32_bf16(av[0][i], bv[NP - 1][j], x, 0, 0, 0);
            x = __builtin_amdgcn_mfma_f32_16x16x32_bf16(av[NP / 2][i], bv[NP / 2][j], x, 0, 0, 0);
            x = __builtin_amdgcn_mfma_f32_16x16x32_bf16(av[NP / 2][i], bv[0][j], x, 0, 0, 0);
            x = __builtin_amdgcn_mfma_f32_16x16x32_bf16(av[0][i], bv[NP / 2][j], x, 0, 0, 0);
          }
          acc4[i][j] = __builtin_amdgcn_mfma_f32_16x16x32_bf16(av[0][i], bv[0][j], x, 0, 0, 0);
        }
    }
    __syncthreads();

#pragma unroll
    for (int i = 0; i < SM; ++i)
#pragma unroll
      for (int j = 0; j < SN; ++j)
#pragma unroll
        for (int r = 0; r < 4; ++r) E[(16 * i + 4 * lq + r) * EPW + 16 * j + l16] = acc4[i][j][r];
    __builtin_amdgcn_fence(__ATOMIC_RELEASE, "wavefront");
    __builtin_amdgcn_wave_barrier();
    __builtin_amdgcn_fence(__ATOMIC_ACQUIRE, "wavefront");
    const int64_t img = (int64_t)b * a.ho * a.wo;
#pragma unroll
    for (int q = 0; q < WM / RPI; ++q) {
      const int m = q * RPI + rr;
      const float4 v = *reinterpret_cast<const float4*>(&E[m * EPW + 4 * c4]);
      const int oy = oy0 + 2 * wm + m / 32, ox = ox0 + m % 32;
      if (oy < a.ho && ox < a.wo && n < a.N)
        epilogue_store4<MODE_FWD>(a, 0, img + (int64_t)oy * a.wo + ox, n, v);
    }
    if (a.pool_out) {
      const int pho = a.ho / 2, pwo = a.wo / 2;
#pragma unroll
      for (int u = 0; u < 2; ++u) {
        const int it = lane + 64 * u;
        const int pc = it >> 3, qq = it & 7;
        const int nn = co0 + wn * WN + 4 * qq;
        const int py = (oy0 + 2 * wm) / 2, px = ox0 / 2 + pc;
        if (py >= pho || px >= pwo || nn >= a.N) continue;
        float bias[4], scale[4], shift[4];
#pragma unroll
        for (int e = 0; e < 4; ++e) column_params<MODE_FWD>(a, nn + e, bias[e], scale[e], shift[e]);
        float rv[4][4];
#pragma unroll
        for (int k = 0; k < 4; ++k) {
          const int m = (k >> 1) * 32 + 2 * pc + (k & 1);
          const float4 v = *reinterpret_cast<const float4*>(&E[m * EPW + 4 * qq]);
          const float vv[4] = {v.x, v.y, v.z, v.w};
#pragma unroll
          for (int e = 0; e < 4; ++e) {
            float x = vv[e] + bias[e];
            if (a.bn_g) x = x * scale[e] + shift[e];
            rv[k][e] = act_fwd(x, a.act, a.alpha);
          }
        }
        float o[4];
#pragma unroll
        for (int e = 0; e < 4; ++e) o[e] = fmaxf(fmaxf(rv[0][e], rv[1][e]), fmaxf(rv[2][e], rv[3][e]));
        *reinterpret_cast<float4*>(&a.pool_out[(((int64_t)b * pho + py) * pwo + px) * a.N + nn]) =
            make_float4(o[0], o[1], o[2], o[3]);
      }
    }
    __syncthreads();
  }
}

static int g_stem_x3 = 1;
static int g_stem_persist = -1;
static int g_stem_bf16 = 1;
static int g_tall16_dgrad = 0;
static int g_tile16_pf = 1;
bool stem_x3_ok(const of_conv_desc* d) {
  return d->kh == 7 && d->kw == 7 && d->stride == 2 && d->cin_p == 4 && d->cout == 64 &&
         d->pad_top >= 0 && d->pad_top <= 3 && d->pad_left >= 0 && d->pad_left <= 3;
}

template <int BM, int BN, int WAVES_M, int WAVES_N, int MODE, int NP = 3, int RING = 3>
__global__ __launch_bounds__(64 * WAVES_M * WAVES_N, NP == 1 || RING == 2 ? 2 : 1)
void conv_gemm_x3(GemmArgs a) {
  static_assert(MODE == MODE_FWD || MODE == MODE_DGRAD, "x3 GEMM: fwd / dgrad");
  static_assert(NP == 3 || NP == 1, "three split planes (fp32) or one (bf16)");
  constexpr int NT = 64 * WAVES_M * WAVES_N, NW = NT / 64;
  constexpr int WM = BM / WAVES_M, WN = BN / WAVES_N, SM = WM / 16, SN = WN / 16;
  static_assert(NW % 4 == 0 && SM >= 1 && SN >= 1 && WM % 16 == 0 && WN % 16 == 0, "tile");
  constexpr int RG = NW / 4;
  constexpr int A_SL = BM / (64 * RG);
  static_assert(A_SL >= 1 && BM % (64 * RG) == 0, "BM");
  constexpr int A_U4 = NP * BM * 4, B_U4 = NP * BN * 4;
  constexpr int BDI = NP * BN / 16, BDW = (BDI + NW - 1) / NW;
  constexpr int OP_U4 = 2 * (A_U4 + B_U4), EP_U4 = NW * WM * WN * 4 / 16;
  constexpr int AF_U4 = BM * 8, SLOT_U4 = AF_U4 + B_U4;
  constexpr int NS = RING == 2 && 2 * 2 * SLOT_U4 * 16 <= 160 * 1024 ? 2
                   : RING && 3 * SLOT_U4 * 16 * (NP == 1 ? 2 : 1) <= 160 * 1024 ? 3 : 0;
  constexpr bool DA = NS > 0;
  constexpr int OPS_U4 = DA ? NS * SLOT_U4 : OP_U4;
  __shared__ uint4 smem[OPS_U4 > EP_U4 ? OPS_U4 : EP_U4];

  const int tid = threadIdx.x;
  const int lane = tid & 63;
  const int wave = __builtin_amdgcn_readfirstlane(tid >> 6);
  const int wgid = a.phase ? (int)blockIdx.x : xcd_remap(blockIdx.x, gridDim.x);
  const int split = wgid / a.tiles_total;
  const int tile = wgid - split * a.tiles_total;
  const int tile_n = tile % a.n_tiles;
  const int tile_mg = tile / a.n_tiles;
  int gi = 0;
#pragma unroll
  for (int g = 1; g < MAX_GROUPS; ++g)
    if (g < a.ngroups && tile_mg >= a.grp[g].tiles_begin) gi = g;
  const Group& G = a.grp[gi];
  const int tile_m = tile_mg - G.tiles_begin;
  const int m0 = tile_m * BM, n0 = tile_n * BN;
  const int M = G.M;
  const int k_begin = split * a.k_per_split;
  const int k_end = min(G.K, k_begin + a.k_per_split);
  const int nchunks = k_end > k_begin ? (k_end - k_begin + BKH - 1) / BKH : 0;
  const rsrc_t ra_src = make_rsrc(a.A, a.a_bytes);
  const rsrc_t rb_src = make_rsrc(a.B, a.b_bytes);

  const int oct = wave & 3, rgrp = wave >> 2;
  const int src_h = (MODE == MODE_DGRAD) ? a.ho : a.h;
  const int src_w = (MODE == MODE_DGRAD) ? a.wo : a.w;
  int a_off[A_SL];
  uint64_t a_msk[A_SL];
#pragma unroll
  for (int i = 0; i < A_SL; ++i) {
    const int m = m0 + 64 * (rgrp + RG * i) + lane;
    const bool okm = m < M;
    const int mm = okm ? m : 0;
    int b, yb, xb;
    if (MODE == MODE_FWD) {
      const int hw = a.ho * a.wo;
      b = mm / hw;
      const int rem = mm - b * hw;
      const int oy = rem / a.wo, ox = rem - oy * a.wo;
      yb = oy * a.stride - a.pt;
      xb = ox * a.stride - a.pl;
    } else if (a.phase) {
      const int hw = G.hc * G.wc;
      b = mm / hw;
      const int rem = mm - b * hw;
      const int u = rem / G.wc, v = rem - u * G.wc;
      yb = (2 * u + G.ry + a.pt - G.r0) >> 1;
      xb = (2 * v + G.rx + a.pl - G.s0) >> 1;
    } else {
      const int hw = a.h * a.w;
      b = mm / hw;
      const int rem = mm - b * hw;
      const int iy = rem / a.w, ix = rem - iy * a.w;
      yb = iy + a.pt;
      xb = ix + a.pl;
    }
    a_off[i] = (int)(((int64_t)(b * src_h + yb) * src_w + xb) * a.lda * 4);
    uint64_t msk = 0;
    if (okm) {
      uint64_t colmask = 0;
      for (int ts = 0; ts < G.ns; ++ts) {
// ... 2678 lines not shown
  a.nb = bf16 ? d->cout : g.nf;
  return a;
}

GemmArgs dgrad_args(const of_conv_desc* d, const Geo& g, bool bf16 = false,
                    bool skip_empty = false) {
  GemmArgs a = base_args(d);
  a.kc = g.cout_p;
  a.N = g.cin_p;
  a.ldb = bf16 ? (int)g.kd16 : g.nd;
  a.nb = g.nd;
  int kmax = 0;
  if (g.phase) {
    a.phase = 1;
    a.dt = 2;
    a.ngroups = 4;
    a.bm = pick_bm(a.N);
    a.n_tiles = (int)cdiv(a.N, pick_bn(a.N));
    int tiles = 0;
    for (int c = 0; c < 4; ++c) {
      Group& G = a.grp[c];
      G = Group{};
      const int qy = c >> 1, qx = c & 1;
      G.ry = (((qy - d->pad_top) % 2) + 2) % 2;
      G.rx = (((qx - d->pad_left) % 2) + 2) % 2;
      G.hc = std::max(0, (d->h - G.ry + 1) / 2);
      G.wc = std::max(0, (d->w - G.rx + 1) / 2);
      G.M = d->n * G.hc * G.wc;
      G.m_tiles = (int)cdiv(G.M, a.bm);
      G.tiles_begin = tiles;
      tiles += G.m_tiles;
      G.r0 = g.pg.r0[c];
      G.s0 = g.pg.s0[c];
      G.ns = g.pg.ns[c];
      G.ntaps = g.pg.ntaps[c];
      const int64_t* rb = bf16 ? g.pg.row_begin16 : g.pg.row_begin;
      G.K = (int)(rb[c + 1] - rb[c]);
      G.b_off = rb[c];
      kmax = std::max(kmax, G.K);
    }
    a.tiles_total = tiles * a.n_tiles;
    a.M = d->n * d->h * d->w;
  } else {
    a.M = d->n * d->h * d->w;
    kmax = (int)(bf16 ? g.kd16 : g.kd);
    single_group(a, d, a.M, kmax);
  }
  plan_splits(a, kmax, bf16 ? BKH : BK);
  if (skip_empty && a.phase) {
    int tiles = 0;
    for (int c = 0; c < 4; ++c) {
      Group& G = a.grp[c];
      if (G.ntaps == 0) G.m_tiles = 0;
      G.tiles_begin = tiles;
      tiles += G.m_tiles;
    }
    a.tiles_total = tiles * a.n_tiles;
  }
  return a;
}

bool al16(const void* p) { return ((uintptr_t)p & 15) == 0; }

static int g_vec_ep = 1;
static int g_wgx3b = 1;
static int g_wgx3b_mi = 1;
static int g_wgx3b_stage = 1;
static int g_wgx3_min_tiles = 2;
static int g_wgx3_c4 = 1;
static int g_wgx3_gemm = 1;
static int g_wgrad_b16 = 0;
bool vec_ep_ok(const GemmArgs& a) {
  if (!g_vec_ep || a.N % 4) return false;
  if (a.slab && !(a.slab_ld % 4 == 0 && a.split_stride % 4 == 0 && al16(a.slab))) return false;
  if (a.splits > 1) return a.slab != nullptr;
  auto ok = [](const float* p, int ld) { return !p || (ld % 4 == 0 && al16(p)); };
  return ok(a.C, a.ldc) && ok(a.res, a.ldr) && ok(a.z, a.ldz) && ok(a.act_src, a.ld_act);
}

template <int MODE>
int launch_splitk_epilogue(const GemmArgs& a, hipStream_t s) {
  const int64_t items = slab_rows(a) * cdiv(a.N, 4);
  if (a.splits > 8 && items < 65536) {
    hipLaunchKernelGGL(splitk_epilogue_kernel<MODE>, dim3(cdiv(items, EP_ITEMS)), dim3(256), 0,
                       s, a);
    return check_launch("conv_splitk_epilogue");
  }
  bool vec = a.N % 4 == 0 && a.ldc % 4 == 0 && al16(a.C);
  if (a.res) vec = vec && a.ldr % 4 == 0 && al16(a.res);
  if (MODE == MODE_FWD && a.z) vec = vec && a.ldz % 4 == 0 && al16(a.z);
  if (MODE == MODE_DGRAD && a.act_src) vec = vec && a.ld_act % 4 == 0 && al16(a.act_src);
  const dim3 grid((unsigned)std::min<int64_t>(cdiv(items, 256), 8 * device_cus()));
  if (vec) hipLaunchKernelGGL((splitk_epilogue_flat<MODE, true>), grid, dim3(256), 0, s, a);
  else hipLaunchKernelGGL((splitk_epilogue_flat<MODE, false>), grid, dim3(256), 0, s, a);
  return check_launch("conv_splitk_epilogue");
}

constexpr int KIND_F32 = 0, KIND_TILE_F32 = 32, KIND_BF16 = 64, KIND_TILE_BF16 = 96,
              KIND_TILE_X3 = 128, KIND_GEMM_X3 = 160, KIND_TILE_B16 = 192, KIND_WGRAD_B16 = 216,
              KIND_TILE_WS = 224, KIND_GEMM_B16 = 240;
constexpr int KIND_STEM_X3 = 184, KIND_STEM_WG_X3 = 185;
constexpr int KIND_STEM_B16 = 186, KIND_STEM_WG_B16 = 187;
constexpr int KIND_NARROW = 7;
constexpr int kind(int base, int mode, int cfg) { return base + mode * 8 + cfg; }
constexpr int KIND_WGRAD_X3B = kind(KIND_TILE_X3, MODE_WGRAD, 4);

constexpr Launch with_cfg(Launch l, int cfg) { return {l.fn, l.threads, l.kind + cfg, l.name}; }

template <int MODE>
int launch(const Launch& l, const GemmArgs& a, hipStream_t s, double flops, unsigned grid = 0) {
  if (timing_on()) timing_begin(s);
  hipLaunchKernelGGL(l.fn, dim3(grid ? grid : a.tiles_total * a.splits), dim3(l.threads), 0, s, a);
  if (timing_on()) timing_end(s, l.kind, flops);
  int st = check_launch(l.name);
  if (st || MODE == MODE_WGRAD || a.splits == 1) return st;
  return launch_splitk_epilogue<MODE>(a, s);
}
struct StemLaunch {
  void (*fn)(GemmArgs, int);
  int threads, kind;
};
template <int CO, int NP = 3>
constexpr StemLaunch stem_rec() {
  return {conv_stem_x3<CO, NP>, CO * 8, NP == 1 ? KIND_STEM_B16 : KIND_STEM_X3};
}

int bn_cfg(int N) { return N > 96 ? 0 : N > 64 ? 1 : N > 32 ? 2 : 3; }

template <int BM, int BN, int WM, int WN, int MODE>
constexpr Launch gemm_f32_rec() {
  return {conv_gemm_f32<BM, BN, WM, WN, MODE>, 256, kind(KIND_F32, MODE, 0), "conv_gemm_f32"};
}
template <int BM, int BN, int WM, int WN, int MODE>
constexpr Launch gemm_bf16_rec() {
  return {conv_gemm_bf16<BM, BN, WM, WN, MODE>, 256, kind(KIND_BF16, MODE, 0), "conv_gemm_bf16"};
}
template <int BM, int BN, int WM, int WN>
constexpr Launch wgrad_bf16_rec() {
  return {conv_wgrad_bf16<BM, BN, WM, WN>, 256, kind(KIND_BF16, MODE_WGRAD, 0), "conv_wgrad_bf16"};
}

template <int MODE>
Launch gemm_f32_launch(const GemmArgs& a) {
  static const Launch T[4] = {gemm_f32_rec<128, 128, 2, 2, MODE>(), gemm_f32_rec<128, 96, 4, 1, MODE>(),
                              gemm_f32_rec<256, 64, 4, 1, MODE>(), gemm_f32_rec<256, 32, 4, 1, MODE>()};
  return with_cfg(T[bn_cfg(a.N)], bn_cfg(a.N));
}
template <int MODE>
Launch gemm_bf16_launch(const GemmArgs& a) {
  static const Launch T[4] = {gemm_bf16_rec<128, 128, 2, 2, MODE>(), gemm_bf16_rec<128, 96, 4, 1, MODE>(),
                              gemm_bf16_rec<256, 64, 4, 1, MODE>(), gemm_bf16_rec<256, 32, 4, 1, MODE>()};
  return with_cfg(T[bn_cfg(a.N)], bn_cfg(a.N));
}
Launch wgrad_bf16_launch(const GemmArgs& a) {
  static const Launch T[4] = {wgrad_bf16_rec<128, 128, 2, 2>(), wgrad_bf16_rec<128, 96, 4, 1>(),
                              wgrad_bf16_rec<256, 64, 4, 1>(), wgrad_bf16_rec<256, 32, 4, 1>()};
  return with_cfg(T[bn_cfg(a.N)], bn_cfg(a.N));
}

bool tile_ok(const of_conv_desc* d) { return d->kh == 3 && d->kw == 3 && d->stride == 1; }

bool x3_tall(int n, int oh, int ow, int N) {
  const int bn = pick_bn(N);
  return (bn == 128 || bn == 96) && (int64_t)n * cdiv(oh, X3_TH0) * cdiv(ow, TF_W) >= 4 * device_cus();
}

constexpr int X3_NB1_MIN = 384;
bool x3_nb1_candidate(const GemmArgs& a, bool tall) {
  return !tall && a.bn_tile == 0 && pick_bn(a.N) == 128 && a.tiles_total >= X3_NB1_MIN;
}
bool x3_nb1(const GemmArgs& a) {
  return a.bm != X3_TH0 * TF_W && a.splits == 1 && x3_nb1_candidate(a, false);
}

static int g_tile_b16 = 0;
bool ws_ok(const of_conv_desc* d, int mode) {
  const int N = mode == MODE_FWD ? d->cout : d->cin_p;
  return (g_tile_b16 == 2 || (g_tile_b16 == 3 && mode == MODE_FWD)) && pick_bn(N) >= 96;
}

static int g_x3t_ep = 5;
static int g_x3g_ep = 5;
static int g_x3_small_bn = 1200;
static int g_x3_bn64 = 0;
static int g_abl_noact = 0;
int best_split(int chunks, int64_t tiles, int slots, int ep) {
  int best = 1;
  double best_cost = 1e30;
  for (int sp = 1; sp <= std::min(8, chunks); ++sp) {
    const int per = (int)cdiv(chunks, sp);
    if (cdiv(chunks, per) != sp) continue;
    const double cost = (double)cdiv(tiles * sp, slots) * (per + 1.0) +
                        (sp > 1 ? 0.1 * ep * sp * tiles / (double)slots : 0.0);
    if (cost < best_cost - 1e-9) {
      best_cost = cost;
      best = sp;
    }
  }
  return best;
}

GemmArgs tile_args(const of_conv_desc* d, const Geo& g, int mode, bool x3 = false,
                   bool b16 = false, bool ws = false) {
  GemmArgs a = base_args(d);
  const bool fwd = mode == MODE_FWD;
  a.kc = fwd ? g.cin_p : g.cout_p;
  a.N = fwd ? d->cout : g.cin_p;
  a.nb = fwd ? d->cout : g.nd;
  a.ldb = fwd ? g.kf16 : (int)g.kd16;
  const int OH = fwd ? d->ho : d->h, OW = fwd ? d->wo : d->w;
  if (x3 && !b16 && !ws && g_x3_small_bn > 0 && pick_bn(a.N) == 128 &&
      (int64_t)d->n * cdiv(OH, TF_H) * cdiv(OW, TF_W) * cdiv(a.N, 128) < g_x3_small_bn)
    a.bn_tile = 64;
  const bool tall64 = x3 && !b16 && !ws && !a.bn_tile && g_x3_bn64 == 1 && pick_bn(a.N) == 64 &&
                      (int64_t)d->n * cdiv(OH, X3_TH0) * cdiv(OW, TF_W) >= 4 * device_cus();
  const bool tall = tall64 ? true : a.bn_tile ? false : ws ? true
                  : x3 || b16 ? x3_tall(d->n, OH, OW, a.N)
                             : (fwd || g_tall16_dgrad) && pick_bn(a.N) == 128 &&
                                   x3_tall(d->n, OH, OW, a.N);
  const int th = tall ? X3_TH0 : TF_H;
  const int m_tiles = d->n * (int)cdiv(OH, th) * (int)cdiv(OW, TF_W);
  a.bm = th * TF_W;
  a.ngroups = 1;
  Group& G = a.grp[0];
  G = Group{};
  G.M = d->n * OH * OW;
  G.m_tiles = m_tiles;
  G.ns = 3;
  G.ntaps = 9;
  a.M = G.M;
  a.n_tiles = (int)cdiv(a.N, a.bn_tile ? a.bn_tile : pick_bn(a.N));
  a.tiles_total = m_tiles * a.n_tiles;
  a.K = (int)cdiv(a.kc, 32);
  G.K = a.K;
  a.splits = 1;
  a.k_per_split = a.K;
  if (x3 || b16 || ws) {
    const bool bn64 = x3 && !b16 && !ws && (a.bn_tile ? a.bn_tile : pick_bn(a.N)) == 64;
    const int slots = !ws && ((b16 && !tall) || x3_nb1_candidate(a, tall) || a.bn_tile == 64 ||
                              (g_x3_bn64 && bn64))
                          ? 2 * device_cus() : device_cus();
    a.k_per_split = (int)cdiv(a.K, best_split(a.K, a.tiles_total, slots, g_x3t_ep));
    a.splits = (int)cdiv(a.K, a.k_per_split);
  } else if (a.tiles_total < 2 * device_cus()) {
    int sp = std::max(1, (4 * device_cus()) / a.tiles_total);
    sp = std::min(sp, std::max(1, a.K / 2));
    a.k_per_split = (int)cdiv(a.K, sp);
    a.splits = (int)cdiv(a.K, a.k_per_split);
  }
  return a;
}

bool tall_tile(const GemmArgs& a) { return a.bm == X3_TH0 * TF_W; }

template <int BN, int WM, int WN, int MODE, int TH = OF_TF_H, int PF = 1>
constexpr Launch tile_bf16_rec() {
  return {conv_tile_bf16<BN, WM, WN, MODE, TH, PF>, 64 * WM * WN, kind(KIND_TILE_BF16, MODE, 0),
          "conv_tile_bf16"};
}
template <int BN, int WM, int WN, int MODE, int TH, int NB = 2>
constexpr Launch tile_x3_rec() {
  return {conv_tile_x3<BN, WM, WN, MODE, TH, NB>, 64 * WM * WN, kind(KIND_TILE_X3, MODE, 0), "conv_tile_x3"};
}
template <int BN, int WM, int WN, int MODE, int TH>
constexpr Launch tile_b16_rec() {
  return {conv_tile_b16<BN, WM, WN, MODE, TH>, 64 * WM * WN, kind(KIND_TILE_B16, MODE, 0), "conv_tile_b16"};
}

template <int MODE>
Launch tile_bf16_launch(const GemmArgs& a) {
  static const Launch T[2][5] = {
      {tile_bf16_rec<128, 2, 2, MODE, OF_TF_H, 0>(), tile_bf16_rec<96, 4, 1, MODE, OF_TF_H, 0>(),
       tile_bf16_rec<64, 2, 2, MODE, OF_TF_H, 0>(), tile_bf16_rec<32, 4, 1, MODE, OF_TF_H, 0>(),
       tile_bf16_rec<128, 4, 2, MODE, X3_TH0, 0>()},
      {tile_bf16_rec<128, 2, 2, MODE>(), tile_bf16_rec<96, 4, 1, MODE>(), tile_bf16_rec<64, 2, 2, MODE>(),
       tile_bf16_rec<32, 4, 1, MODE>(), tile_bf16_rec<128, 4, 2, MODE, X3_TH0>()}};
  const int cfg = bn_cfg(a.N) == 0 && tall_tile(a) ? 4 : bn_cfg(a.N);
  return with_cfg(T[g_tile16_pf != 0][cfg], cfg);
}

struct WgradPlan {
  int splits, k_per_split, M, ldc;
  int64_t split_stride;
};

template <int MODE>
Launch tile_x3_launch(const GemmArgs& a) {
  static const Launch T[7] = {
      tile_x3_rec<128, 4, 2, MODE, X3_TH0>(), tile_x3_rec<96, 2, 3, MODE, 4>(),
      tile_x3_rec<64, 4, 2, MODE, 4>(), tile_x3_rec<32, 4, 1, MODE, 4>(),
      tile_x3_rec<128, 2, 2, MODE, 4, 1>(), tile_x3_rec<96, 4, 3, MODE, X3_TH0>(),
      tile_x3_rec<128, 2, 4, MODE, 4>()};
  static const Launch T7[3] = {tile_x3_rec<64, 4, 1, MODE, X3_TH0, 1>(),
                               tile_x3_rec<64, 4, 1, MODE, 4, 1>(),
                               tile_x3_rec<64, 2, 2, MODE, 4, 1>()};
  const int bn = a.bn_tile ? a.bn_tile : pick_bn(a.N);
  const bool tall = tall_tile(a);
  if (bn == 64 && (tall || g_x3_bn64 >= 2))
    return with_cfg(T7[tall ? 0 : g_x3_bn64 == 2 ? 1 : 2], 7);
  const int cfg = bn == 128 ? (tall ? 0 : x3_nb1(a) ? 4 : 6) : bn == 96 ? (tall ? 5 : 1) : bn == 64 ? 2 : 3;
  return with_cfg(T[cfg], cfg);
}

template <int MODE>
Launch tile_b16_launch(const GemmArgs& a) {
  static const Launch T[7] = {
      tile_b16_rec<128, 4, 2, MODE, X3_TH0>(), tile_b16_rec<96, 2, 3, MODE, 4>(),
      tile_b16_rec<64, 4, 2, MODE, 4>(), tile_b16_rec<32, 4, 1, MODE, 4>(), Launch{},
      tile_b16_rec<96, 4, 3, MODE, X3_TH0>(), tile_b16_rec<128, 2, 4, MODE, 4>()};
  const int bn = bn_cfg(a.N);
  const int cfg = bn == 0 ? (tall_tile(a) ? 0 : 6) : bn == 1 ? (tall_tile(a) ? 5 : 1) : bn;
  return with_cfg(T[cfg], cfg);
}

void gemm_x3_plan(GemmArgs& a) {
  const int bm = a.N > 64 ? 128 : 256, bn = a.N > 64 ? 128 : 64;
  int tiles = 0, tiles_all = 0, kmax = 0;
  for (int g = 0; g < a.ngroups; ++g) {
    Group& G = a.grp[g];
    if (G.m_tiles) G.m_tiles = (int)cdiv(G.M, bm);
    G.tiles_begin = tiles;
    tiles += G.m_tiles;
    tiles_all += (int)cdiv(G.M, bm);
    kmax = std::max(kmax, G.K);
  }
  a.bm = bm;
  a.n_tiles = (int)cdiv(a.N, bn);
  a.tiles_total = tiles * a.n_tiles;
  const int64_t plan_tiles = (int64_t)tiles_all * a.n_tiles;
  const int chunks = (int)cdiv(kmax, BKH);
  const int best = best_split(chunks, plan_tiles, device_cus(), g_x3g_ep);
  a.k_per_split = (int)cdiv(chunks, best) * BKH;
  a.splits = (int)cdiv(kmax, a.k_per_split);
}

static int g_gx3_ring = 2;
template <int BM, int BN, int WM, int WN, int MODE, int NP, int RING>
constexpr Launch gemm_x3_rec() {
  return {conv_gemm_x3<BM, BN, WM, WN, MODE, NP, RING>, 64 * WM * WN,
          kind(NP == 1 ? KIND_GEMM_B16 : KIND_GEMM_X3, MODE, 0), "conv_gemm_x3"};
}
template <int BM, int BN, int WM, int WN, int NP>
constexpr Launch wgrad_x3_rec() {
  return {conv_wgrad_x3<BM, BN, WM, WN, NP>, 64 * WM * WN,
          kind(NP == 1 ? KIND_GEMM_B16 : KIND_GEMM_X3, MODE_WGRAD, 0),
          NP == 1 ? "conv_wgrad_x3_b16" : "conv_wgrad_x3"};
}
template <int MODE, int NP = 3>
Launch gemm_x3_launch(const GemmArgs& a) {
  static const Launch T[3][2] = {
      {gemm_x3_rec<128, 128, 4, 2, MODE, NP, 0>(), gemm_x3_rec<256, 64, 8, 1, MODE, NP, 0>()},
      {gemm_x3_rec<128, 128, 4, 2, MODE, NP, 3>(), gemm_x3_rec<256, 64, 8, 1, MODE, NP, 3>()},
      {gemm_x3_rec<128, 128, 4, 2, MODE, NP, 2>(), gemm_x3_rec<256, 64, 8, 1, MODE, NP, 2>()}};
  const int cfg = a.N > 64 ? 0 : 1;
  return with_cfg(T[g_gx3_ring][cfg], cfg);
}
template <int NP>
Launch wgrad_x3_launch(const of_conv_desc* d) {
  static const Launch T[2] = {wgrad_x3_rec<128, 128, 4, 2, NP>(), wgrad_x3_rec<128, 64, 4, 2, NP>()};
  const int cfg = d->cout > 64 ? 0 : 1;
  return with_cfg(T[cfg], cfg);
}

bool wgt_ok(const of_conv_desc* d, bool bf16) {
  if (!tile_ok(d)) return false;
  if (bf16) return true;
  const int64_t npix = (int64_t)d->n * d->ho * d->wo;
  return d->cout == 64 || (d->cout % 128 == 0 && npix <= 8 * 96 * 128);
}
int wgt_cfg(const of_conv_desc* d) { return d->cout > 64 ? 0 : 2; }
void wgt_blocks(const of_conv_desc* d, int& cib, int& cob) {
  cib = wgt_cfg(d) == 0 ? 32 : 64;
  cob = wgt_cfg(d) == 0 ? 128 : 64;
}

int wgx3_cfg(const of_conv_desc* d) {
  if (!tile_ok(d)) return -1;
  if (d->cout == 64) return d->cin_p % 64 == 0 || !g_wgx3_c4 ? 2 : 4;
  return d->cout % 128 == 0 ? 0 : d->cout == 96 ? 1 : d->cout == 32 ? 3 : -1;
}
bool wgx3_ok(const of_conv_desc* d) { return wgx3_cfg(d) >= 0; }
void wgx3_blocks(const of_conv_desc* d, int& cib, int& cob) {
  const int c = wgx3_cfg(d);
  cib = c == 2 || c == 3 ? 64 : 32;
  cob = c == 0 ? 128 : c == 1 ? 96 : c == 2 || c == 4 ? 64 : 32;
}

static int g_stem_wg = 1;
bool stem_wg_ok(const of_conv_desc* d) { return g_stem_wg && stem_x3_ok(d) && d->cin == 3; }
int stem_wg_tiles(const of_conv_desc* d) {
  return d->n * (int)cdiv(d->ho, SW_TH) * (int)cdiv(d->wo, SW_TW);
}

static int g_wgrad_wgs = 4;
static int g_x3_direct = 1;
static int g_bnp_b16 = 0;

static int g_gemm_b16 = 6;
static int g_wgt_pf = 1;

enum class Fam { narrow, gemm_f32, gemm_bf16, gemm_x3, gemm_b16, tile_bf16, tile_x3, tile_b16,
                 tile_ws, stem };
enum class WFam { narrow, stem, tile_x3, tile_b16, gemm_x3, gemm_b16, tile, gemm_bf16, gemm_f32 };

Fam gemm_family(int prec, int mode) {
  if (!prec) return Fam::gemm_f32;
  if (prec == 2) return Fam::gemm_x3;
  return (g_gemm_b16 & (mode == MODE_FWD ? 1 : 2)) ? Fam::gemm_b16 : Fam::gemm_bf16;
}
Fam tile_family(const of_conv_desc* d, int prec, int mode, bool bnp = false) {
  if (prec == 2) return Fam::tile_x3;
  if (ws_ok(d, mode)) return Fam::tile_ws;
  return g_tile_b16 == 1 || (bnp && g_bnp_b16) ? Fam::tile_b16 : Fam::tile_bf16;
}
Fam fwd_family(const of_conv_desc* d, int prec, bool plain, bool stem_kernel = true) {
  if (!prec) return narrow_ok(d) && plain ? Fam::narrow : Fam::gemm_f32;
  if (tile_ok(d)) return tile_family(d, prec, MODE_FWD);
  if (stem_kernel && (prec == 2 || g_stem_bf16) && g_stem_x3 && stem_x3_ok(d)) return Fam::stem;
  return gemm_family(prec, MODE_FWD);
}
Fam dgrad_family(const of_conv_desc* d, int prec, bool bnp = false) {
  if (!prec) return narrow_ok(d) ? Fam::narrow : Fam::gemm_f32;
  return tile_ok(d) ? tile_family(d, prec, MODE_DGRAD, bnp) : gemm_family(prec, MODE_DGRAD);
}

GemmArgs plan_args(const of_conv_desc* d, const Geo& g, int mode, Fam f, bool in_place = false) {
  if (f == Fam::tile_bf16 || f == Fam::tile_x3 || f == Fam::tile_b16 || f == Fam::tile_ws)
    return tile_args(d, g, mode, f == Fam::tile_x3, f == Fam::tile_b16, f == Fam::tile_ws);
  const bool k16 = f != Fam::gemm_f32 && f != Fam::narrow;
  GemmArgs a = mode == MODE_FWD ? fwd_args(d, g, k16) : dgrad_args(d, g, k16, in_place);
  if (f == Fam::gemm_x3 || f == Fam::gemm_b16) gemm_x3_plan(a);
  return a;
}

template <int MODE>
int launch_family(Fam f, const GemmArgs& a, hipStream_t s, double flops) {
  switch (f) {
    case Fam::tile_x3: return launch<MODE>(tile_x3_launch<MODE>(a), a, s, flops);
    case Fam::tile_ws:
      return launch<MODE>(with_cfg(tile_ws_launch(a, MODE), kind(KIND_TILE_WS, MODE, 0)), a, s, flops);
    case Fam::tile_b16: return launch<MODE>(tile_b16_launch<MODE>(a), a, s, flops);
    case Fam::tile_bf16: return launch<MODE>(tile_bf16_launch<MODE>(a), a, s, flops);
    case Fam::gemm_x3: return launch<MODE>(gemm_x3_launch<MODE>(a), a, s, flops);
    case Fam::gemm_b16: return launch<MODE>(gemm_x3_launch<MODE, 1>(a), a, s, flops);
    case Fam::gemm_bf16: return launch<MODE>(gemm_bf16_launch<MODE>(a), a, s, flops);
    case Fam::gemm_f32: return launch<MODE>(gemm_f32_launch<MODE>(a), a, s, flops);
    default: return fail(OF_EINVAL, "conv: no GEMM launch for this family");
  }
}

WFam wgrad_family(const of_conv_desc* d, int prec) {
  const bool bf16 = prec == 1;
  if (narrow_ok(d)) return WFam::narrow;
  if (stem_wg_ok(d) && (!bf16 || g_stem_bf16)) return WFam::stem;
  if (prec == 2 && wgx3_ok(d)) return WFam::tile_x3;
  if (bf16 && g_wgrad_b16 && wgx3_ok(d)) return WFam::tile_b16;
  if (prec == 2 && g_wgx3_gemm) return WFam::gemm_x3;
  if (bf16 && (g_gemm_b16 & 4) && !tile_ok(d)) return WFam::gemm_b16;
  if (wgt_ok(d, bf16)) return WFam::tile;
  return bf16 ? WFam::gemm_bf16 : WFam::gemm_f32;
}

void wgrad_tiles(GemmArgs& a, const of_conv_desc* d, const Geo& g, bool x3) {
  int cib, cob;
  x3 ? wgx3_blocks(d, cib, cob) : wgt_blocks(d, cib, cob);
  a.K = d->n * (int)cdiv(d->ho, x3 ? wgx3_rows(wgx3_cfg(d)) : TT_H) * (int)cdiv(d->wo, TT_W);
  a.n_tiles = (int)cdiv(d->cout, cob);
  a.tiles_total = (int)cdiv(g.cin_p, cib) * a.n_tiles;
}

WgradPlan wgrad_plan(const of_conv_desc* d, int prec) {
  Geo g = geo(d);
  const WFam f = wgrad_family(d, prec);
  WgradPlan p;
  p.M = g.taps * g.cin_p;
  p.ldc = g.cout_p;
  p.split_stride = (int64_t)(p.M + 1) * p.ldc;
  auto slice = [&p](int units, int splits, int step = 1) {
    p.k_per_split = (int)round_up(cdiv(units, std::max(1, splits)), step);
    p.splits = (int)cdiv(units, p.k_per_split);
    return p;
  };
  if (f == WFam::stem)
    return slice(stem_wg_tiles(d), std::min(stem_wg_tiles(d), SW_WGS_PER_CU * device_cus()));
  if (f == WFam::tile_x3 || f == WFam::tile_b16 || f == WFam::tile) {
    GemmArgs t{};
    wgrad_tiles(t, d, g, f != WFam::tile);
    const int splits = std::min(t.K, device_cus() / t.tiles_total);
    return slice(t.K, f == WFam::tile ? splits : std::min(splits, t.K / g_wgx3_min_tiles));
  }
  const int K = d->n * d->ho * d->wo;
  if (f == WFam::gemm_x3 || f == WFam::gemm_b16) {
    const int tiles = (int)(cdiv(p.M, 128) * cdiv(d->cout, d->cout > 64 ? 128 : 64));
    const int splits = std::max(1, (f == WFam::gemm_b16 ? 2 : 1) * device_cus() / tiles);
    return slice(K, std::min(splits, (int)std::max<int64_t>(1, cdiv(K, 8 * BKH))), BKH);
  }
  const int bk = prec == 1 ? BKH : BK;
  const int tiles = (int)(cdiv(p.M, pick_bm(d->cout)) * cdiv(d->cout, pick_bn(d->cout)));
  const int splits = std::max(1, (g_wgrad_wgs * device_cus()) / tiles);
  return slice(K, std::min(splits, (int)std::max<int64_t>(1, cdiv(K, 8 * bk))), bk);
}
size_t wgrad_workspace(const of_conv_desc* d, int prec) {
  if (validate(d) != OF_OK) return 0;
  if (narrow_ok(d)) return narrow_wgrad_ws(d);
  const WgradPlan p = wgrad_plan(d, prec);
  return (size_t)p.splits * p.split_stride * sizeof(float);
}

template <int NP, bool FUSED = false>
constexpr Launch wgrad_stem_rec() {
  return {conv_wgrad_stem_x3<NP, FUSED>, SW_NT, NP == 1 ? KIND_STEM_WG_B16 : KIND_STEM_WG_X3,
          FUSED ? "conv_wgrad_stem_x3 fused" : "conv_wgrad_stem_x3"};
}
template <int STAGE, int CI, int CO, int R, int XH>
constexpr Launch wgrad_tile_x3_rec() {
  return {STAGE ? conv_wgrad_tile_x3<CI, CO, R, XH> : conv_wgrad_tile_x3_c3<CI, CO, R, XH>,
          64 * CI * CO * R, kind(KIND_TILE_X3, MODE_WGRAD, 0), "conv_wgrad_tile_x3"};
}
template <int STAGE, int CI, int CO, int XH, int MI = 1>
constexpr Launch wgrad_x3b_rec() {
  return {STAGE ? conv_wgrad_tile_x3b<CI, CO, XH, MI> : conv_wgrad_tile_x3b_c3<CI, CO, XH, MI>,
          64 * CI * CO, KIND_WGRAD_X3B, "conv_wgrad_tile_x3"};
}
template <int STAGE, int CI, int CO, int XH>
constexpr Launch wgrad_b16_rec() {
  return {STAGE ? conv_wgrad_tile_b16<CI, CO, XH> : conv_wgrad_tile_b16_c3<CI, CO, XH>,
          64 * CI * CO, KIND_WGRAD_B16, "conv_wgrad_tile_b16"};
}
template <int CI, int CO, int PF = 1>
constexpr Launch wgrad_tile_bf16_rec() {
  return {conv_wgrad_tile_bf16<CI, CO, PF>, 256, kind(KIND_TILE_BF16, MODE_WGRAD, 0), "conv_wgrad_tile"};
}
template <int CI, int CO>
constexpr Launch wgrad_tile_f32_rec() {
  return {conv_wgrad_tile_f32<CI, CO>, 256, kind(KIND_TILE_F32, MODE_WGRAD, 0), "conv_wgrad_tile"};
}

Launch wgrad_tile_x3_launch(int cfg) {
  static const Launch B[2][2][5] = {
      {{wgrad_x3b_rec<0, 2, 4, 8>(), wgrad_x3b_rec<0, 2, 3, 8>(), wgrad_x3b_rec<0, 4, 2, 4>(),
        wgrad_x3b_rec<0, 4, 1, 4>(), wgrad_x3b_rec<0, 2, 2, 8>()},
       {wgrad_x3b_rec<0, 1, 8, 8, 2>(), wgrad_x3b_rec<0, 1, 6, 8, 2>(), wgrad_x3b_rec<0, 2, 4, 4, 2>(),
        wgrad_x3b_rec<0, 2, 2, 4, 2>(), wgrad_x3b_rec<0, 1, 4, 8, 2>()}},
      {{wgrad_x3b_rec<1, 2, 4, 8>(), wgrad_x3b_rec<1, 2, 3, 8>(), wgrad_x3b_rec<1, 4, 2, 4>(),
        wgrad_x3b_rec<1, 4, 1, 4>(), wgrad_x3b_rec<1, 2, 2, 8>()},
       {wgrad_x3b_rec<1, 1, 8, 8, 2>(), wgrad_x3b_rec<1, 1, 6, 8, 2>(), wgrad_x3b_rec<1, 2, 4, 4, 2>(),
        wgrad_x3b_rec<1, 2, 2, 4, 2>(), wgrad_x3b_rec<1, 1, 4, 8, 2>()}}};
  static const Launch T[2][4] = {
      {wgrad_tile_x3_rec<0, 1, 4, 3, 8>(), wgrad_tile_x3_rec<0, 1, 3, 3, 8>(),
       wgrad_tile_x3_rec<0, 2, 2, 3, 4>(), wgrad_tile_x3_rec<0, 2, 1, 3, 4>()},
      {wgrad_tile_x3_rec<1, 1, 4, 3, 8>(), wgrad_tile_x3_rec<1, 1, 3, 3, 8>(),
       wgrad_tile_x3_rec<1, 2, 2, 3, 4>(), wgrad_tile_x3_rec<1, 2, 1, 3, 4>()}};
  const bool x3b = g_wgx3b == 2 || (g_wgx3b == 1 && cfg == 0) || cfg == 4;
  return with_cfg(x3b ? B[g_wgx3b_stage][g_wgx3b_mi - 1][cfg] : T[g_wgx3b_stage][cfg], cfg);
}
Launch wgrad_tile_b16_launch(int cfg) {
  static const Launch T[2][5] = {
      {wgrad_b16_rec<0, 2, 4, 8>(), wgrad_b16_rec<0, 2, 3, 8>(), wgrad_b16_rec<0, 4, 2, 4>(),
       wgrad_b16_rec<0, 4, 1, 4>(), wgrad_b16_rec<0, 2, 2, 8>()},
      {wgrad_b16_rec<1, 2, 4, 8>(), wgrad_b16_rec<1, 2, 3, 8>(), wgrad_b16_rec<1, 4, 2, 4>(),
       wgrad_b16_rec<1, 4, 1, 4>(), wgrad_b16_rec<1, 2, 2, 8>()}};
  return with_cfg(T[g_wgx3b_stage][cfg], cfg);
}
Launch wgrad_tile_launch(int cfg, bool bf16) {
  static const Launch T16[2][2] = {{wgrad_tile_bf16_rec<1, 4, 0>(), wgrad_tile_bf16_rec<2, 2, 0>()},
                                   {wgrad_tile_bf16_rec<1, 4>(), wgrad_tile_bf16_rec<2, 2>()}};
  static const Launch T32[2] = {wgrad_tile_f32_rec<1, 4>(), wgrad_tile_f32_rec<2, 2>()};
  return with_cfg(bf16 ? T16[g_wgt_pf != 0][cfg / 2] : T32[cfg / 2], cfg);
}

}
}

using namespace oflow;

extern "C" {

int64_t of_conv_wfwd_elems(const of_conv_desc* d) {
  if (validate(d) != OF_OK) return -1;
  Geo g = geo(d);
  return (int64_t)g.kf * g.nf;
}

int64_t of_conv_wbwd_elems(const of_conv_desc* d) {
  if (validate(d) != OF_OK) return -1;
  Geo g = geo(d);
  return g.kd * g.nd;
}

int64_t of_conv_wfwd16_elems(const of_conv_desc* d) {
  if (validate(d) != OF_OK) return -1;
  Geo g = geo(d);
  return (int64_t)g.cout_p * g.kf16;
}

int64_t of_conv_wbwd16_elems(const of_conv_desc* d) {
  if (validate(d) != OF_OK) return -1;
  Geo g = geo(d);
  return g.kd16 * g.nd;
}

static PackEntry pack_entry(const of_conv_desc* d, const float* w, void* wf, void* wd,
                            int bf16) {
  const Geo g = geo(d);
  PackEntry E{};
  E.w = w;
  E.wf = static_cast<float*>(wf);
  E.wd = static_cast<float*>(wd);
  E.taps = g.taps;
  E.kw = d->kw;
  E.cin = d->cin;
  E.cout = d->cout;
  E.cin_p = g.cin_p;
  E.cout_p = g.cout_p;
  E.kf = g.kf;
  E.nf = g.nf;
  E.nd = g.nd;
  E.bf16 = bf16;
  E.kf16 = g.kf16;
  E.kd16 = g.kd16;
  E.pg = g.pg;
  return E;
}

static int64_t pack_work(const of_conv_desc* d, int bf16) {
  const Geo g = geo(d);
  return bf16 ? (int64_t)g.cout_p * g.kf16 + g.kd16 * g.nd : (int64_t)g.kf * g.nf + g.kd * g.nd;
}

static int64_t pack_work_many(const of_conv_desc* d, int bf16) {
  const Geo g = geo(d);
  return bf16 ? g.kd16 * g.nd : (int64_t)g.kf * g.nf + g.kd * g.nd;
}
static int64_t pack_tiles16(const of_conv_desc* d, int bf16) {
  const Geo g = geo(d);
  return bf16 ? cdiv(g.cout_p, PK_TN) * cdiv(g.kf16, PK_TK) : 0;
}

int of_conv_pack_weights_bf16(const of_conv_desc* d, const float* w_hwio, void* w16_fwd,
                              void* w16_bwd, void* stream) {
  int st = validate(d);
  if (st) return st;
  OF_CHECK_ARG(w_hwio && w16_fwd && w16_bwd, "pack bf16: NULL pointer");
  const int64_t total = pack_work(d, 1);
  OF_CHECK_ARG(total < INT32_MAX, "pack: layer too large");
  const int blocks = (int)std::min<int64_t>(cdiv(total, 256), 4096);
  hipLaunchKernelGGL(pack_one_kernel, dim3(blocks), dim3(256), 0, as_stream(stream),
                     pack_entry(d, w_hwio, w16_fwd, w16_bwd, 1), total);
  return check_launch("pack_bf16");
}

int of_conv_pack_weights(const of_conv_desc* d, const float* w_hwio, float* w_fwd,
                         float* w_bwd, void* stream) {
  int st = validate(d);
  if (st) return st;
  OF_CHECK_ARG(w_hwio && w_fwd, "pack: NULL pointer");
  Geo g = geo(d);
  hipStream_t s = as_stream(stream);
  {
    const int64_t total = (int64_t)g.kf * g.nf;
    const int blocks = (int)std::min<int64_t>(cdiv(total, 256), 4096);
    hipLaunchKernelGGL(pack_fwd_kernel, dim3(blocks), dim3(256), 0, s, w_hwio, g.taps, d->cin,
                       d->cout, g.cin_p, g.kf, g.nf, w_fwd);
    if ((st = check_launch("pack_fwd"))) return st;
  }
  if (w_bwd) {
    const int64_t total = g.kd * g.nd;
    const int blocks = (int)std::min<int64_t>(cdiv(total, 256), 4096);
    hipLaunchKernelGGL(pack_bwd_kernel, dim3(blocks), dim3(256), 0, s, w_hwio, g.pg, d->kw,
                       d->cin, d->cout, g.cout_p, g.nd, w_bwd);
    if ((st = check_launch("pack_bwd"))) return st;
  }
  return OF_OK;
}

int of_set_tuning(int key, int value) {
  if (key == 8 && value >= 0 && value <= 2) { g_stem_x3 = value; return OF_OK; }
  if (key == 7 && (value == 0 || value == 1)) { g_warp_win = value; return OF_OK; }
  if (key == 9 && value >= 0 && value <= 7) { g_corr_blk = value; return OF_OK; }
  if (key == 19 && (value == 0 || value == 1)) { g_corr_ty8 = value; return OF_OK; }
  if (key == 10 && value >= 1 && value <= 16) { g_wgrad_wgs = value; return OF_OK; }
  if (key == 11 && (value == 0 || value == 1)) { g_wgx3_c4 = value; return OF_OK; }
  if (key == 1 && value >= 1 && value <= 16) { g_split_wgs = value; return OF_OK; }
  if (key == 2 && value >= 2 && value <= 64) { g_split_min_chunks = value; return OF_OK; }
  if (key == 3 && (value == 0 || value == 1)) { g_vec_ep = value; return OF_OK; }
  if (key == 4 && value >= 0 && value <= 2) { g_wgx3b = value; return OF_OK; }
  if (key == 5 && (value == 1 || value == 2)) { g_wgx3b_mi = value; return OF_OK; }
  if (key == 6 && (value == 0 || value == 1)) { g_wgx3_gemm = value; return OF_OK; }
  if (key == 12 && value >= 0 && value <= 3) { g_tile_b16 = value; return OF_OK; }
  if (key == 13 && (value == 0 || value == 1)) { g_wgrad_b16 = value; return OF_OK; }
  if (key == 14 && (value == 0 || value == 1)) { g_stem_wg = value; return OF_OK; }
  if (key == 15 && (value == 0 || value == 1)) { g_stem_bf16 = value; return OF_OK; }
  if (key == 16 && value >= 0 && value <= 7) { g_gemm_b16 = value; return OF_OK; }
  if (key == 18 && (value == 0 || value == 1)) { g_tall16_dgrad = value; return OF_OK; }
  if (key == 17 && (value == 0 || value == 1)) { g_wgt_pf = value; return OF_OK; }
  if (key == 20 && (value == 0 || value == 1)) { g_tile16_pf = value; return OF_OK; }
  if (key == 21 && value >= 0 && value <= 3) { g_b16i_abl = value; return OF_OK; }
  if (key == 22 && (value == 0 || value == 1)) { g_b16i_direct = value; return OF_OK; }
  if (key == 23 && value >= 0 && value <= 3) { g_x3_direct = value; return OF_OK; }
  if (key == 24 && value >= 0 && value <= 2) { g_b16i_persist = value; return OF_OK; }
  if (key == 25 && value >= 0 && value <= 1000) { g_x3t_ep = value; return OF_OK; }
  if (key == 26 && value >= 0 && value <= 1000) { g_x3g_ep = value; return OF_OK; }
  if (key == 27 && value >= 0 && value <= 100000) { g_x3_small_bn = value; return OF_OK; }
  if (key == 28 && value >= 0 && value <= 64) { g_det_rmax = value; return OF_OK; }
  if (key == 29 && value >= 0 && value <= 4) { g_wgr_lanes = value; return OF_OK; }
  if (key == 30 && value >= 0 && value <= 2) { g_gx3_ring = value; return OF_OK; }
  if (key == 31 && value >= -1 && value <= 8) { g_stem_persist = value; return OF_OK; }
  if (key == 32 && (value == 0 || value == 1)) { g_bnp_b16 = value; return OF_OK; }
  if (key == 33 && value >= 1 && value <= 256) { g_wgx3_min_tiles = value; return OF_OK; }
  if (key == 34 && value >= 0 && value <= 2) { g_det_tile = value; return OF_OK; }
  if (key == 35 && (value == 0 || value == 1)) { g_det_tpre = value; return OF_OK; }
  if (key == 36 && value >= 0 && value <= 3) { g_x3_bn64 = value; return OF_OK; }
  if (key == 37 && value >= 0 && value <= 16) { g_det_fx_grid = value; return OF_OK; }
  if (key == 38 && value >= 0 && value <= 131072) { g_det_lds_probe = value; return OF_OK; }
  if (key == 39 && (value == 0 || value == 1)) { g_abl_noact = value; return OF_OK; }
  if (key == 40 && (value == 0 || value == 1)) { g_wgx3b_stage = value; return OF_OK; }
  return fail(OF_EINVAL, "of_set_tuning: unknown key/value " + std::to_string(key));
}

size_t of_conv_pack_table_bytes(int nconv) {
  return sizeof(PackTableHeader) + (size_t)std::max(nconv, 0) * sizeof(PackEntry);
}

int of_conv_pack_table_ex(int nconv, const of_conv_desc* descs, const float* const* w_hwio,
                          void* const* w_fwd, void* const* w_bwd, const int* bf16,
                          void* host_table) {
  OF_CHECK_ARG(nconv > 0 && descs && w_hwio && w_fwd && w_bwd && host_table, "pack table: args");
  PackTableHeader* h = static_cast<PackTableHeader*>(host_table);
  PackEntry* e = reinterpret_cast<PackEntry*>(static_cast<char*>(host_table) +
                                              sizeof(PackTableHeader));
  int64_t work = 0, tiles = 0;
  for (int i = 0; i < nconv; ++i) {
    int st = validate(&descs[i]);
    if (st) return st;
    OF_CHECK_ARG(w_hwio[i] && w_fwd[i] && w_bwd[i], "pack table: NULL weight pointer");
    const int b16 = bf16 ? (bf16[i] == 2 ? 2 : bf16[i] != 0) : 0;
    e[i] = pack_entry(&descs[i], w_hwio[i], w_fwd[i], w_bwd[i], b16);
    e[i].work_begin = work;
    e[i].tile_begin = (int)tiles;
    OF_CHECK_ARG(pack_work(&descs[i], b16) < INT32_MAX, "pack table: layer too large");
    work += pack_work_many(&descs[i], b16);
    tiles += pack_tiles16(&descs[i], b16);
    OF_CHECK_ARG(tiles < INT32_MAX, "pack table: too many tiles");
  }
  h->nconv = nconv;
  h->ntiles16 = (int)tiles;
  h->total = work;
  return OF_OK;
}

int of_conv_pack_table(int nconv, const of_conv_desc* descs, const float* const* w_hwio,
                       float* const* w_fwd, float* const* w_bwd, void* host_table) {
  return of_conv_pack_table_ex(nconv, descs, w_hwio, reinterpret_cast<void* const*>(w_fwd),
                               reinterpret_cast<void* const*>(w_bwd), nullptr, host_table);
}

int of_conv_pack_many(const void* dev_table, int64_t total_work, void* stream) {
  OF_CHECK_ARG(dev_table && total_work > 0, "pack many: args");
  const int64_t blocks = cdiv(total_work, 256 * PACK_PT);
  OF_CHECK_ARG(blocks < INT32_MAX / 2, "pack many: too much work");
  hipLaunchKernelGGL(pack_many_kernel, dim3((unsigned)(2 * blocks)), dim3(256), 0,
                     as_stream(stream), static_cast<const char*>(dev_table), (int)blocks);
  return check_launch("pack_many");
}

double conv_flops(const of_conv_desc* d) {
  return 2.0 * d->n * d->ho * d->wo * (double)d->cout * d->kh * d->kw * d->cin;
}

size_t of_conv2d_fwd_workspace(const of_conv_desc* d) {
  if (validate(d) != OF_OK) return 0;
  return fd_workspace(plan_args(d, geo(d), MODE_FWD, Fam::gemm_f32));
}

size_t of_conv2d_dgrad_workspace(const of_conv_desc* d) {
  if (validate(d) != OF_OK) return 0;
  return fd_workspace(plan_args(d, geo(d), MODE_DGRAD, Fam::gemm_f32));
}

size_t of_conv2d_fwd_bf16_workspace(const of_conv_desc* d) {
  if (validate(d) != OF_OK) return 0;
  if (tile_ok(d)) return fd_workspace(plan_args(d, geo(d), MODE_FWD, tile_family(d, 1, MODE_FWD)));
  return std::max(fd_workspace(plan_args(d, geo(d), MODE_FWD, gemm_family(1, MODE_FWD))),
                  fd_workspace(plan_args(d, geo(d), MODE_FWD, Fam::gemm_bf16)));
}

size_t of_conv2d_dgrad_bf16_workspace(const of_conv_desc* d) {
  if (validate(d) != OF_OK) return 0;
  if (tile_ok(d)) return fd_workspace(plan_args(d, geo(d), MODE_DGRAD, tile_family(d, 1, MODE_DGRAD)));
  return std::max(fd_workspace(plan_args(d, geo(d), MODE_DGRAD, gemm_family(1, MODE_DGRAD))),
                  fd_workspace(plan_args(d, geo(d), MODE_DGRAD, Fam::gemm_bf16)));
}

int of_conv_path(const of_conv_desc* d) {
  if (validate(d) != OF_OK) return -1;
  return narrow_ok(d) ? 1 : 0;
}

static int conv_fwd_impl(int prec, const of_conv_desc* d, const float* x, int ldx,
                         const void* w_fwd, const float* bias, const float* bn_gamma,
                         const float* bn_beta, const float* bn_mean, const float* bn_var,
                         float bn_eps, const float* residual, int ldr, int act, float alpha,
                         float* z, int ldz, float* y, int ldy, void* workspace, size_t ws_bytes,
                         void* stream, float* pool = nullptr) {
  int st = validate(d);
  if (st) return st;
  const bool bf16 = prec == 1, x3 = prec == 2;
  OF_CHECK_ARG(!x3 || !narrow_ok(d), "conv fwd x3: the Cout <= 4 layers take the fp32 kernels");
  OF_CHECK_ARG(x && w_fwd && y, "conv fwd: NULL pointer");
  OF_CHECK_ARG(ldx >= d->cin_p && ldx % 4 == 0, "conv fwd: ldx");
  OF_CHECK_ARG(ldy >= d->cout, "conv fwd: ldy");
  OF_CHECK_ARG(!bn_gamma || (bn_beta && bn_mean && bn_var), "conv fwd: incomplete BN params");
  OF_CHECK_ARG(!residual || ldr >= d->cout, "conv fwd: ldr");
  OF_CHECK_ARG(!z || ldz >= d->cout, "conv fwd: ldz");
  OF_CHECK_ARG(((uintptr_t)x & 15) == 0 && ((uintptr_t)w_fwd & 15) == 0,
               "conv fwd: x / w must be 16-byte aligned");
  Fam f = fwd_family(d, prec, !bn_gamma && !residual && !z);
  if (f == Fam::narrow) {
    hipStream_t s = as_stream(stream);
    if (timing_on()) timing_begin(s);
    st = narrow_fwd(d, x, ldx, static_cast<const float*>(w_fwd), bias, act, alpha, y, ldy, s);
    if (timing_on()) timing_end(s, kind(KIND_F32, MODE_FWD, KIND_NARROW), conv_flops(d));
    return st;
  }
  Geo g = geo(d);
  GemmArgs a = plan_args(d, g, MODE_FWD, f);
  a.C = y;
  a.ldc = ldy;
  a.res = residual;
  a.ldr = ldr;
  a.z = z;
  a.ldz = ldz;
  if (f == Fam::stem) {
    a.splits = 1;
    a.k_per_split = a.K;
    a.slab = nullptr;
    if (!vec_ep_ok(a)) {
      f = gemm_family(prec, MODE_FWD);
      if (f != Fam::gemm_bf16) gemm_x3_plan(a);
    }
  }
  const bool tile = prec && tile_ok(d);
  if (f != Fam::stem) attach_slab(a, workspace, ws_bytes, tile ? 1 : prec ? BKH : BK);
  a.A = x;
  a.lda = ldx;
  a.a_bytes = (int64_t)d->n * d->h * d->w * ldx * 4;
  a.B = static_cast<const float*>(w_fwd);
  a.b_plane = (int64_t)g.cout_p * g.kf16;
  a.b_bytes = x3 ? 3 * a.b_plane * 2 : bf16 ? a.b_plane * 2 : (int64_t)g.kf * g.nf * 4;
  OF_CHECK_ARG(a.a_bytes < INT32_MAX && a.b_bytes < INT32_MAX,
               "conv fwd: tensors must be < 2 GiB (32-bit buffer offsets)");
  a.bias = bias;
  a.bn_g = bn_gamma;
  a.bn_b = bn_beta;
  a.bn_m = bn_mean;
  a.bn_v = bn_var;
  a.bn_eps = bn_eps;
  a.act = act;
  a.alpha = alpha;
  hipStream_t s = as_stream(stream);
  const double flops = 2.0 * d->n * d->ho * d->wo * (double)d->cout * g.taps * d->cin;
  a.vec_ep = vec_ep_ok(a);
  a.direct16 = f == Fam::tile_x3 && (g_x3_direct & 1) && a.splits == 1 && a.vec_ep && !residual &&
               !z && d->cout % 4 == 0 && ldy % 4 == 0 && ((uintptr_t)y & 15) == 0;
  if (pool) {
    if (f != Fam::stem || d->ho % 2 || d->wo % 2 || d->cout % 4)
      return fail(OF_EUNSUPPORTED, "conv fwd pool: only the stem kernel with an even output");
    OF_CHECK_ARG(((uintptr_t)pool & 15) == 0, "conv fwd pool: 16-byte alignment");
    a.pool_out = pool;
  }
  if (f != Fam::stem) return launch_family<MODE_FWD>(f, a, s, flops);
  const int64_t tiles = (int64_t)d->n * cdiv(d->ho, ST_TH) * cdiv(d->wo, ST_TW);
  OF_CHECK_ARG(tiles < INT32_MAX, "conv stem: too many tiles");
  const int groups = bf16 || g_stem_x3 != 2 ? 2 : 1;
  const int per_cu = g_stem_persist < 0 ? (bf16 ? 3 : g_stem_x3 == 2 ? 1 : 2) : g_stem_persist;
  const int64_t cap = per_cu > 0 ? (int64_t)per_cu * device_cus() : tiles * groups;
  const unsigned grid = (unsigned)(std::min(tiles * groups, cap) / groups * groups);
  const StemLaunch l = bf16 ? stem_rec<32, 1>() : g_stem_x3 == 2 ? stem_rec<64>() : stem_rec<32>();
  if (timing_on()) timing_begin(s);
  hipLaunchKernelGGL(l.fn, dim3(grid), dim3(l.threads), 0, s, a, (int)tiles);
  if (timing_on()) timing_end(s, l.kind, flops);
  return check_launch("conv_stem_x3");
}

int of_conv2d_fwd(const of_conv_desc* d, const float* x, int ldx, const float* w_fwd,
                  const float* bias, const float* bn_gamma, const float* bn_beta,
                  const float* bn_mean, const float* bn_var, float bn_eps,
                  const float* residual, int ldr, int act, float alpha, float* z, int ldz,
                  float* y, int ldy, void* workspace, size_t ws_bytes, void* stream) {
  return conv_fwd_impl(0, d, x, ldx, w_fwd, bias, bn_gamma, bn_beta, bn_mean, bn_var,
                       bn_eps, residual, ldr, act, alpha, z, ldz, y, ldy, workspace, ws_bytes,
                       stream);
}

int of_conv2d_fwd_pool(const of_conv_desc* d, int precision, const float* x, int ldx,
                       const void* w_fwd, const float* bias, const float* bn_gamma,
                       const float* bn_beta, const float* bn_mean, const float* bn_var,
                       float bn_eps, int act, float alpha, float* z, int ldz, float* y, int ldy,
                       float* pool, void* workspace, size_t ws_bytes, void* stream) {
  OF_CHECK_ARG(pool && (precision == 1 || precision == 2), "conv fwd pool: args");
  return conv_fwd_impl(precision, d, x, ldx, w_fwd, bias, bn_gamma, bn_beta, bn_mean, bn_var,
                       bn_eps, nullptr, 0, act, alpha, z, ldz, y, ldy, workspace, ws_bytes,
                       stream, pool);
}

int of_conv2d_fwd_bf16(const of_conv_desc* d, const float* x, int ldx, const void* w16_fwd,
                       const float* bias, const float* bn_gamma, const float* bn_beta,
                       const float* bn_mean, const float* bn_var, float bn_eps,
                       const float* residual, int ldr, int act, float alpha, float* z, int ldz,
                       float* y, int ldy, void* workspace, size_t ws_bytes, void* stream) {
  return conv_fwd_impl(1, d, x, ldx, w16_fwd, bias, bn_gamma, bn_beta, bn_mean, bn_var,
                       bn_eps, residual, ldr, act, alpha, z, ldz, y, ldy, workspace, ws_bytes,
                       stream);
}

struct BnpArgs {
  const float* gamma; const float* beta; const float* res; int ld_res;
  float* part; size_t part_bytes; int* nblk;
};

static int conv_dgrad_impl(int prec, const of_conv_desc* d, const float* dy, int lddy,
                           const void* w_bwd, const float* act_src, int ld_act, int act,
                           float alpha, const float* add, int ld_add, float* dx, int lddx,
                           void* workspace, size_t ws_bytes, void* stream, int act_post = 0,
                           const BnpArgs* bnp = nullptr) {
  int st = validate(d);
  if (st) return st;
  Geo g = geo(d);
  const bool bf16 = prec == 1, x3 = prec == 2;
  OF_CHECK_ARG(!x3 || !narrow_ok(d), "conv dgrad x3: the Cout <= 4 layers take the fp32 kernels");
  OF_CHECK_ARG(dy && w_bwd && dx, "conv dgrad: NULL pointer");
  OF_CHECK_ARG(lddy >= g.cout_p && lddy % 4 == 0, "conv dgrad: lddy (>= round_up(cout,4))");
  OF_CHECK_ARG(lddx >= d->cin_p, "conv dgrad: lddx");
  OF_CHECK_ARG(!act_src || ld_act >= d->cin_p, "conv dgrad: ld_act");
  OF_CHECK_ARG(!add || ld_add >= d->cin_p, "conv dgrad: ld_add");
  OF_CHECK_ARG(((uintptr_t)dy & 15) == 0 && ((uintptr_t)w_bwd & 15) == 0,
               "conv dgrad: dy / w must be 16-byte aligned");
  OF_CHECK_ARG(d->stride == 1 || d->stride == 2, "conv dgrad: stride must be 1 or 2");
  const Fam f = dgrad_family(d, prec, bnp != nullptr);
  if (f == Fam::narrow) {
    OF_CHECK_ARG(!add && !act_post, "conv dgrad: the Cout <= 4 kernels take no added gradient");
    hipStream_t s = as_stream(stream);
    if (timing_on()) timing_begin(s);
    st = narrow_dgrad(d, dy, lddy, static_cast<const float*>(w_bwd), act_src, ld_act, act,
                      alpha, dx, lddx, s);
    if (timing_on()) timing_end(s, kind(KIND_F32, MODE_DGRAD, KIND_NARROW), conv_flops(d));
    return st;
  }
  const bool tile = prec && tile_ok(d);
  const bool in_place = add && add == dx && ld_add == lddx;
  GemmArgs a = plan_args(d, g, MODE_DGRAD, f, in_place);
  if (a.tiles_total == 0)
    return bnp ? fail(OF_EUNSUPPORTED, "conv dgrad bnp: no GEMM tiles") : OF_OK;
  attach_slab(a, workspace, ws_bytes, tile ? 1 : prec ? BKH : BK);
  a.A = dy;
  a.lda = lddy;
  a.a_bytes = (int64_t)d->n * d->ho * d->wo * lddy * 4;
  a.B = static_cast<const float*>(w_bwd);
  a.b_plane = g.kd16 * g.nd;
  a.b_bytes = x3 ? 3 * a.b_plane * 2 : bf16 ? a.b_plane * 2 : g.kd * g.nd * 4;
  OF_CHECK_ARG(a.a_bytes < INT32_MAX && a.b_bytes < INT32_MAX,
               "conv dgrad: tensors must be < 2 GiB (32-bit buffer offsets)");
  a.C = dx;
  a.ldc = lddx;
  a.act_src = act_src;
  a.ld_act = ld_act;
  a.act = act;
  a.alpha = alpha;
  a.res = add;
  a.ldr = ld_add;
  a.act_post = act_post;
  hipStream_t s = as_stream(stream);
  const double flops = 2.0 * d->n * d->ho * d->wo * (double)d->cout * g.taps * d->cin;
  a.vec_ep = vec_ep_ok(a);
  if (g_abl_noact && f == Fam::tile_x3 && !bnp) a.act_src = nullptr;
  a.direct16 = f == Fam::tile_x3 && (g_x3_direct & 2) && a.splits == 1 && a.vec_ep;
  if (bnp) {
    const int64_t m_tiles = a.n_tiles > 0 ? a.tiles_total / a.n_tiles : 0;
    int64_t rows = 0;
    for (int gq = 0; gq < a.ngroups; ++gq) rows += a.grp[gq].M;
    const bool form = f == Fam::tile_x3 || f == Fam::tile_b16 ? X3_EPB == 1
                      : f == Fam::tile_bf16 ? (bool)EPC_BATCH
                      : f == Fam::gemm_x3 && EPC_BATCH && rows == (int64_t)d->n * d->h * d->w;
    if (!(form && a.splits == 1 && a.vec_ep && act_src) ||
        a.N % 4 || ((uintptr_t)bnp->gamma & 15) || ((uintptr_t)bnp->beta & 15) ||
        ((uintptr_t)bnp->part & 15) || (bnp->res && (((uintptr_t)bnp->res & 15) || bnp->ld_res % 4)))
      return fail(OF_EUNSUPPORTED, "conv dgrad bnp: not the one-slice split-tile input gradient");
    OF_CHECK_ARG(bnp->gamma && bnp->beta && bnp->part && bnp->nblk, "conv dgrad bnp: args");
    OF_CHECK_ARG(bnp->part_bytes >= (size_t)m_tiles * 2 * a.N * 4, "conv dgrad bnp: part too small");
    a.direct16 = 0;
    a.bnp = bnp->part;
    a.bnp_res = bnp->res;
    a.ld_bnp_res = bnp->ld_res;
    a.bnp_g = bnp->gamma;
    a.bnp_b = bnp->beta;
    *bnp->nblk = (int)m_tiles;
  }
  return launch_family<MODE_DGRAD>(f, a, s, flops);
}

int of_conv2d_dgrad(const of_conv_desc* d, const float* dy, int lddy, const float* w_bwd,
                    const float* act_src, int ld_act, int act, float alpha, float* dx,
                    int lddx, void* workspace, size_t ws_bytes, void* stream) {
  return conv_dgrad_impl(0, d, dy, lddy, w_bwd, act_src, ld_act, act, alpha, nullptr, 0,
                         dx, lddx, workspace, ws_bytes, stream);
}

int of_conv2d_dgrad_add(const of_conv_desc* d, const float* dy, int lddy, const float* w_bwd,
                        const float* add, int ld_add, float* dx, int lddx, void* workspace,
                        size_t ws_bytes, void* stream) {
  return conv_dgrad_impl(0, d, dy, lddy, w_bwd, nullptr, 0, OF_ACT_NONE, 0.f, add, ld_add,
                         dx, lddx, workspace, ws_bytes, stream);
}

int of_conv2d_dgrad_bf16(const of_conv_desc* d, const float* dy, int lddy, const void* w16_bwd,
                         const float* act_src, int ld_act, int act, float alpha, float* dx,
                         int lddx, void* workspace, size_t ws_bytes, void* stream) {
  return conv_dgrad_impl(1, d, dy, lddy, w16_bwd, act_src, ld_act, act, alpha, nullptr, 0,
                         dx, lddx, workspace, ws_bytes, stream);
}

int of_conv2d_dgrad_add_bf16(const of_conv_desc* d, const float* dy, int lddy,
                             const void* w16_bwd, const float* add, int ld_add, float* dx,
                             int lddx, void* workspace, size_t ws_bytes, void* stream) {
  return conv_dgrad_impl(1, d, dy, lddy, w16_bwd, nullptr, 0, OF_ACT_NONE, 0.f, add, ld_add,
                         dx, lddx, workspace, ws_bytes, stream);
}

int of_conv_pack_weights_x3(const of_conv_desc* d, const float* w_hwio, void* w3_fwd,
                            void* w3_bwd, void* stream) {
  int st = validate(d);
  if (st) return st;
  OF_CHECK_ARG(w_hwio && w3_fwd && w3_bwd, "pack x3: NULL pointer");
  const int64_t total = pack_work(d, 1);
  OF_CHECK_ARG(total < INT32_MAX, "pack: layer too large");
  const int blocks = (int)std::min<int64_t>(cdiv(total, 256), 4096);
  hipLaunchKernelGGL(pack_one_kernel, dim3(blocks), dim3(256), 0, as_stream(stream),
                     pack_entry(d, w_hwio, w3_fwd, w3_bwd, 2), total);
  return check_launch("pack_x3");
}

size_t of_conv2d_fwd_x3_workspace(const of_conv_desc* d) {
  if (validate(d) != OF_OK || narrow_ok(d)) return 0;
  return fd_workspace(plan_args(d, geo(d), MODE_FWD, fwd_family(d, 2, false, false)));
}

size_t of_conv2d_dgrad_x3_workspace(const of_conv_desc* d) {
  if (validate(d) != OF_OK || narrow_ok(d)) return 0;
  return fd_workspace(plan_args(d, geo(d), MODE_DGRAD, dgrad_family(d, 2)));
}

int of_conv2d_fwd_x3(const of_conv_desc* d, const float* x, int ldx, const void* w3_fwd,
                     const float* bias, const float* bn_gamma, const float* bn_beta,
                     const float* bn_mean, const float* bn_var, float bn_eps,
                     const float* residual, int ldr, int act, float alpha, float* z, int ldz,
                     float* y, int ldy, void* workspace, size_t ws_bytes, void* stream) {
  return conv_fwd_impl(2, d, x, ldx, w3_fwd, bias, bn_gamma, bn_beta, bn_mean, bn_var,
                       bn_eps, residual, ldr, act, alpha, z, ldz, y, ldy, workspace, ws_bytes,
                       stream);
}

int of_conv2d_dgrad_x3(const of_conv_desc* d, const float* dy, int lddy, const void* w3_bwd,
                       const float* act_src, int ld_act, int act, float alpha, float* dx,
                       int lddx, void* workspace, size_t ws_bytes, void* stream) {
  return conv_dgrad_impl(2, d, dy, lddy, w3_bwd, act_src, ld_act, act, alpha, nullptr, 0,
                         dx, lddx, workspace, ws_bytes, stream);
}

int of_conv2d_dgrad_add_x3(const of_conv_desc* d, const float* dy, int lddy,
                           const void* w3_bwd, const float* add, int ld_add, float* dx,
                           int lddx, void* workspace, size_t ws_bytes, void* stream) {
  return conv_dgrad_impl(2, d, dy, lddy, w3_bwd, nullptr, 0, OF_ACT_NONE, 0.f, add, ld_add,
                         dx, lddx, workspace, ws_bytes, stream);
}

size_t of_conv2d_wgrad_workspace(const of_conv_desc* d) { return wgrad_workspace(d, 0); }
size_t of_conv2d_wgrad_bf16_workspace(const of_conv_desc* d) { return wgrad_workspace(d, 1); }
size_t of_conv2d_wgrad_x3_workspace(const of_conv_desc* d) { return wgrad_workspace(d, 2); }

static int conv_wgrad_impl(int prec, const of_conv_desc* d, const float* x, int ldx,
                           const float* dy, int lddy, float* dw, float* db, int accumulate,
                           void* workspace, size_t ws_bytes, void* stream,
                           const float* bn_g = nullptr, const float* bn_v = nullptr,
                           float bn_eps = 0.f) {
  int st = validate(d);
  if (st) return st;
  Geo g = geo(d);
  const WFam f = wgrad_family(d, prec);
  OF_CHECK_ARG(x && dy && dw && workspace, "conv wgrad: NULL pointer");
  OF_CHECK_ARG(ldx >= d->cin_p && ldx % 4 == 0, "conv wgrad: ldx");
  OF_CHECK_ARG(lddy >= g.cout_p && lddy % 4 == 0, "conv wgrad: lddy");
  OF_CHECK_ARG(((uintptr_t)x & 15) == 0 && ((uintptr_t)dy & 15) == 0,
               "conv wgrad: x / dy must be 16-byte aligned");
  if (f == WFam::narrow) {
    OF_CHECK_ARG(!bn_g, "conv wgrad: the Cout <= 4 kernels take no BN scale");
    OF_CHECK_ARG(ws_bytes >= narrow_wgrad_ws(d), "conv wgrad: workspace too small");
    hipStream_t s = as_stream(stream);
    if (timing_on()) timing_begin(s);
    st = narrow_wgrad(d, x, ldx, dy, lddy, dw, db, accumulate, workspace, s);
    if (timing_on()) timing_end(s, kind(KIND_F32, MODE_WGRAD, KIND_NARROW), conv_flops(d));
    return st;
  }
  WgradPlan p = wgrad_plan(d, prec);
  OF_CHECK_ARG(ws_bytes >= (size_t)p.splits * p.split_stride * sizeof(float),
               "conv wgrad: workspace too small");
  GemmArgs a = base_args(d);
  a.kc = g.cin_p;
  a.N = d->cout;
  a.K = d->n * d->ho * d->wo;
  single_group(a, d, p.M, a.K);
  a.M = p.M;
  a.A = x;
  a.lda = ldx;
  a.a_bytes = (int64_t)d->n * d->h * d->w * ldx * 4;
  a.B = dy;
  a.ldb = lddy;
  a.b_bytes = (int64_t)a.K * lddy * 4;
  OF_CHECK_ARG(a.a_bytes < INT32_MAX && a.b_bytes < INT32_MAX,
               "conv wgrad: tensors must be < 2 GiB (32-bit buffer offsets)");
  a.nb = g.cout_p;
  a.slab = static_cast<float*>(workspace);
  a.slab_ld = p.ldc;
  a.splits = p.splits;
  a.k_per_split = p.k_per_split;
  a.split_stride = p.split_stride;
  a.colsum = db != nullptr;
  a.vec_ep = vec_ep_ok(a);
  hipStream_t s = as_stream(stream);
  const double flops = 2.0 * a.K * (double)d->cout * g.taps * d->cin;
  Launch l{};
  unsigned grid = 0;
  switch (f) {
    case WFam::stem:
      a.K = stem_wg_tiles(d);
      l = prec == 1 ? wgrad_stem_rec<1>() : wgrad_stem_rec<3>();
      grid = a.splits;
      break;
    case WFam::tile_b16:
    case WFam::tile_x3:
      wgrad_tiles(a, d, g, true);
      l = f == WFam::tile_b16 ? wgrad_tile_b16_launch(wgx3_cfg(d)) : wgrad_tile_x3_launch(wgx3_cfg(d));
      break;
    case WFam::gemm_x3:
    case WFam::gemm_b16:
      a.n_tiles = (int)cdiv(d->cout, d->cout > 64 ? 128 : 64);
      a.tiles_total = (int)cdiv(a.M, 128) * a.n_tiles;
      l = f == WFam::gemm_b16 ? wgrad_x3_launch<1>(d) : wgrad_x3_launch<3>(d);
      break;
    case WFam::tile:
      wgrad_tiles(a, d, g, false);
      l = wgrad_tile_launch(wgt_cfg(d), prec == 1);
      break;
    case WFam::gemm_bf16: l = wgrad_bf16_launch(a); break;
    default: l = gemm_f32_launch<MODE_WGRAD>(a); break;
  }
  st = launch<MODE_WGRAD>(l, a, s, flops, grid);
  if (st) return st;
  launch_wgrad_reduce(s, static_cast<const float*>(workspace), p.splits, p.split_stride, g.taps,
                      g.cin_p, d->cin, d->cout, p.ldc, dw, db, accumulate, bn_g, bn_v, bn_eps);
  return check_launch("wgrad_reduce");
}

static bool stem_fused_ok(const of_conv_desc* d, int prec) {
  return (prec == 2 || (prec == 1 && g_stem_bf16)) && stem_wg_ok(d) && d->ho % 2 == 0 &&
         d->wo % 2 == 0 && d->cout == 64;
}

size_t of_stem_bwd_fused_workspace(const of_conv_desc* d, int precision) {
  if (validate(d) != OF_OK || !stem_fused_ok(d, precision)) return 0;
  WgradPlan p = wgrad_plan(d, precision);
  return (size_t)p.splits * (p.M + 2) * p.ldc * sizeof(float);
}

int of_stem_bwd_fused(const of_conv_desc* d, int precision, const float* x, int ldx,
                      const float* dyp, const float* g, const float* y, const float* gamma,
                      const float* beta, const float* var, float eps, float* dw, float* dbias,
                      float* dgamma, float* dbeta, int accumulate, void* workspace,
                      size_t ws_bytes, void* stream) {
  int st = validate(d);
  if (st) return st;
  if (!stem_fused_ok(d, precision))
    return fail(OF_EUNSUPPORTED, "stem bwd fused: not the 7x7/2 3->64 stem on the split / bf16 "
                                 "kernels with an even output");
  OF_CHECK_ARG(x && dyp && y && gamma && beta && var && dw && workspace, "stem bwd fused: NULL");
  OF_CHECK_ARG(ldx >= d->cin_p && ldx % 4 == 0, "stem bwd fused: ldx");
  WgradPlan p = wgrad_plan(d, precision);
  const int64_t stride = (int64_t)(p.M + 2) * p.ldc;
  OF_CHECK_ARG(ws_bytes >= (size_t)p.splits * stride * sizeof(float),
               "stem bwd fused: workspace too small");
  GemmArgs a = base_args(d);
  a.kc = d->cin_p;
  a.N = d->cout;
  a.M = p.M;
  a.A = x;
  a.lda = ldx;
  a.a_bytes = (int64_t)d->n * d->h * d->w * ldx * 4;
  a.B = y;
  a.ldb = 64;
  a.b_bytes = (int64_t)d->n * d->ho * d->wo * 64 * 4;
  OF_CHECK_ARG(a.a_bytes < INT32_MAX && a.b_bytes < INT32_MAX, "stem bwd fused: < 2 GiB tensors");
  a.nb = 64;
  a.slab = static_cast<float*>(workspace);
  a.slab_ld = p.ldc;
  a.splits = p.splits;
  a.k_per_split = p.k_per_split;
  a.split_stride = stride;
  a.colsum = 0;
  a.K = stem_wg_tiles(d);
  a.bn_g = gamma;
  a.bn_b = beta;
  a.bn_v = var;
  a.bn_eps = eps;
  a.st_dyp = dyp;
  a.st_g = g;
  a.st_y = y;
  hipStream_t s = as_stream(stream);
  const double flops = 2.0 * (double)d->n * d->ho * d->wo * d->cout * 49 * d->cin;
  st = launch<MODE_WGRAD>(precision == 1 ? wgrad_stem_rec<1, true>() : wgrad_stem_rec<3, true>(),
                          a, s, flops, a.splits);
  if (st) return st;
  Geo gg = geo(d);
  launch_wgrad_reduce(s, static_cast<const float*>(workspace), p.splits, stride, gg.taps,
                      gg.cin_p, d->cin, d->cout, p.ldc, dw, nullptr, accumulate, nullptr, nullptr,
                      0.f);
  st = check_launch("wgrad_reduce");
  if (st) return st;
  hipLaunchKernelGGL(stem_bn_final, dim3(1), dim3(256), 0, s, static_cast<const float*>(workspace),
                     p.splits, stride, p.ldc, d->cout, gamma, var, eps, dgamma, dbeta, dbias,
                     accumulate);
  return check_launch("stem_bn_final");
}

int of_conv2d_wgrad(const of_conv_desc* d, const float* x, int ldx, const float* dy, int lddy,
                    float* dw, float* db, int accumulate, void* workspace, size_t ws_bytes,
                    void* stream) {
  return conv_wgrad_impl(0, d, x, ldx, dy, lddy, dw, db, accumulate, workspace, ws_bytes,
                         stream);
}

int of_conv2d_wgrad_bf16(const of_conv_desc* d, const float* x, int ldx, const float* dy,
                         int lddy, float* dw, float* db, int accumulate, void* workspace,
                         size_t ws_bytes, void* stream) {
  return conv_wgrad_impl(1, d, x, ldx, dy, lddy, dw, db, accumulate, workspace, ws_bytes,
                         stream);
}

int of_conv2d_wgrad_x3(const of_conv_desc* d, const float* x, int ldx, const float* dy,
                       int lddy, float* dw, float* db, int accumulate, void* workspace,
                       size_t ws_bytes, void* stream) {
  return conv_wgrad_impl(2, d, x, ldx, dy, lddy, dw, db, accumulate, workspace, ws_bytes,
                         stream);
}


int of_conv_pack_weights_bn(const of_conv_desc* d, int precision, const float* w_hwio,
                            void* w_fwd, void* w_bwd, const float* bn_gamma,
                            const float* bn_var, float bn_eps, void* stream) {
  int st = validate(d);
  if (st) return st;
  OF_CHECK_ARG(precision >= 0 && precision <= 2, "pack bn: precision 0, 1 or 2");
  OF_CHECK_ARG(w_hwio && w_fwd && w_bwd, "pack bn: NULL pointer");
  OF_CHECK_ARG(!bn_gamma || bn_var, "pack bn: gamma without var");
  const int64_t total = pack_work(d, precision ? 1 : 0);
  OF_CHECK_ARG(total < INT32_MAX, "pack: layer too large");
  PackEntry E = pack_entry(d, w_hwio, w_fwd, w_bwd, precision);
  E.bn_g = bn_gamma;
  E.bn_v = bn_var;
  E.bn_eps = bn_eps;
  const int blocks = (int)std::min<int64_t>(cdiv(total, 256), 4096);
  hipLaunchKernelGGL(pack_one_kernel, dim3(blocks), dim3(256), 0, as_stream(stream), E, total);
  return check_launch("pack_bn");
}

int of_conv_pack_table_bn(int nconv, const of_conv_desc* descs, const float* const* w_hwio,
                          void* const* w_fwd, void* const* w_bwd, const int* precision,
                          const float* const* bn_gamma, const float* const* bn_var,
                          float bn_eps, void* host_table) {
  int st = of_conv_pack_table_ex(nconv, descs, w_hwio, w_fwd, w_bwd, precision, host_table);
  if (st || !bn_gamma) return st;
  OF_CHECK_ARG(bn_var != nullptr, "pack table bn: gamma without var");
  PackEntry* e = reinterpret_cast<PackEntry*>(static_cast<char*>(host_table) +
                                              sizeof(PackTableHeader));
  for (int i = 0; i < nconv; ++i) {
    OF_CHECK_ARG(!bn_gamma[i] || bn_var[i], "pack table bn: gamma without var");
    e[i].bn_g = bn_gamma[i];
    e[i].bn_v = bn_var[i];
    e[i].bn_eps = bn_eps;
  }
  return OF_OK;
}

size_t of_conv2d_wgrad_bn_workspace(const of_conv_desc* d, int precision) {
  return wgrad_workspace(d, precision == 1 || precision == 2 ? precision : 0);
}

int of_conv2d_wgrad_bn(const of_conv_desc* d, int precision, const float* x, int ldx,
                       const float* t, int ldt, float* dw, int accumulate, const float* bn_gamma,
                       const float* bn_var, float bn_eps, void* workspace, size_t ws_bytes,
                       void* stream) {
  OF_CHECK_ARG(precision >= 0 && precision <= 2, "wgrad bn: precision 0, 1 or 2");
  OF_CHECK_ARG(bn_gamma && bn_var, "wgrad bn: gamma / var");
  return conv_wgrad_impl(precision, d, x, ldx, t, ldt, dw, nullptr, accumulate, workspace,
                         ws_bytes, stream, bn_gamma, bn_var, bn_eps);
}

int of_conv2d_dgrad_add_act(const of_conv_desc* d, int precision, const float* dy, int lddy,
                            const void* w_bwd, const float* add, int ld_add,
                            const float* act_src, int ld_act, int act, float alpha, float* dx,
                            int lddx, void* workspace, size_t ws_bytes, void* stream) {
  OF_CHECK_ARG(precision >= 0 && precision <= 2, "dgrad add act: precision 0, 1 or 2");
  OF_CHECK_ARG(act_src && (act == OF_ACT_RELU || act == OF_ACT_LEAKY),
               "dgrad add act: act_src and a relu / leaky act");
  return conv_dgrad_impl(precision, d, dy, lddy, w_bwd, act_src, ld_act, act, alpha, add,
                         ld_add, dx, lddx, workspace, ws_bytes, stream, 1);
}

size_t of_conv2d_dgrad_bnp_bytes(const of_conv_desc* d) {
  if (validate(d)) return 0;
  Geo g = geo(d);
  size_t bytes = 0;
  for (int f = 0; f < 3; ++f) {
    const Fam tiles[3] = {Fam::tile_x3, Fam::tile_b16, Fam::tile_bf16};
    const GemmArgs a = plan_args(d, g, MODE_DGRAD, tile_ok(d) ? tiles[f] : Fam::gemm_x3, f == 1);
    if (a.n_tiles > 0) bytes = std::max(bytes, (size_t)(a.tiles_total / a.n_tiles) * 2 * a.N * 4);
  }
  return bytes;
}

int of_conv2d_dgrad_add_act_bnp(const of_conv_desc* d, int precision, const float* dy, int lddy,
                                const void* w_bwd, const float* add, int ld_add,
                                const float* act_src, int ld_act, int act, float alpha,
                                float* dx, int lddx, const float* bn_gamma, const float* bn_beta,
                                const float* bn_res, int ld_bn_res, float* part,
                                size_t part_bytes, int* nblk, void* workspace, size_t ws_bytes,
                                void* stream) {
  OF_CHECK_ARG(precision >= 0 && precision <= 2, "dgrad add act bnp: precision 0, 1 or 2");
  OF_CHECK_ARG(act_src && (act == OF_ACT_RELU || act == OF_ACT_LEAKY),
               "dgrad add act bnp: act_src and a relu / leaky act");
  const BnpArgs b{bn_gamma, bn_beta, bn_res, ld_bn_res, part, part_bytes, nblk};
  return conv_dgrad_impl(precision, d, dy, lddy, w_bwd, act_src, ld_act, act, alpha, add,
                         ld_add, dx, lddx, workspace, ws_bytes, stream, 1, &b);
}

}
```

Measured before the change: 663.9.

## Add halo-tiled x3 kernel for stride-2 3x3 conv forward and dgrad

Adds a stride-2 variant of the halo-tiled x3 (three-plane bf16) conv kernel. Forward stages the input halo in LDS split into even/odd row and column parity blocks. Dgrad uses a four-phase sub-pixel decomposition with a separate accumulator set per phase. It is selected for large 3x3 stride-2 convs at x3 precision (dgrad only when no K-split is needed), replacing the im2col-style gemm_x3 path so input data is reused from LDS instead of re-gathered per tap. The cost is extra accumulator registers in dgrad, parity-remap address arithmetic, and a fallback path with workspace sizing taken as the max of both plans.

Result: no change. 663.0 (-0.1%).

```diff
diff --git a/include/oflow.h b/include/oflow.h
--- a/include/oflow.h
+++ b/include/oflow.h
@@ -57,6 +57,7 @@
                     void* stream);
 
 int of_conv_path(const of_conv_desc* d);
+int of_conv_s2_halo(const of_conv_desc* d, int mode);
 int64_t of_conv_wfwd16_elems(const of_conv_desc* d);
 int64_t of_conv_wbwd16_elems(const of_conv_desc* d);
 int of_conv_pack_weights_bf16(const of_conv_desc* d, const float* w_hwio, void* w16_fwd,
diff --git a/optical_flow_amd/_lib.py b/optical_flow_amd/_lib.py
--- a/optical_flow_amd/_lib.py
+++ b/optical_flow_amd/_lib.py
@@ -52,6 +52,7 @@
     "of_conv2d_wgrad_workspace": (SZ, [PD]),
     "of_conv2d_wgrad": (I, [PD, P, I, P, I, P, P, I, P, SZ, P]),
     "of_conv_path": (I, [PD]),
+    "of_conv_s2_halo": (I, [PD, I]),
     "of_conv_wfwd16_elems": (I64, [PD]),
     "of_conv_wbwd16_elems": (I64, [PD]),
     "of_conv_pack_weights_bf16": (I, [PD, P, P, P, P]),
diff --git a/optical_flow_amd/csrc/conv_f32.hip b/optical_flow_amd/csrc/conv_f32.hip
--- a/optical_flow_amd/csrc/conv_f32.hip
+++ b/optical_flow_amd/csrc/conv_f32.hip
@@ -1049,11 +1049,18 @@
   l = make_uint2(hi2(lb[0], lb[1]), hi2(lb[2], lb[3]));
 }
 
-template <int BN, int WAVES_M, int WAVES_N, int MODE, int TH, int NB, int NP>
+template <int BN, int WAVES_M, int WAVES_N, int MODE, int TH, int NB, int NP, int S = 1>
 __device__ __forceinline__ void tile_x3_body(const GemmArgs& a) {
   constexpr int BM = TH * TF_W, KS = 3;
   static_assert(NP == 1 || NP == 3, "planes");
-  constexpr int HH = TH + KS - 1, HW = TF_W + KS - 1, HP = HH * HW;
+  static_assert(S == 1 || S == 2, "stride");
+  constexpr bool S2F = S == 2 && MODE == MODE_FWD, S2D = S == 2 && MODE == MODE_DGRAD;
+  constexpr int NPH = S2D ? 4 : 1;
+  constexpr int HH = S2F ? 2 * TH + 1 : S2D ? TH + 1 : TH + KS - 1;
+  constexpr int HW = S2F ? 2 * TF_W + 1 : S2D ? TF_W + 1 : TF_W + KS - 1, HP = HH * HW;
+  constexpr int CW0 = TF_W + 1, CW1 = TF_W;
+  constexpr int PB[2][2] = {{0, (TH + 1) * CW0},
+                            {(TH + 1) * (CW0 + CW1), (TH + 1) * (CW0 + CW1) + TH * CW0}};
   constexpr int WM = BM / WAVES_M, WN = BN / WAVES_N;
   constexpr int SM = WM / 16, SN = WN / 16;
   constexpr int NT = 64 * WAVES_M * WAVES_N;
@@ -1084,12 +1091,30 @@
   const int n0 = tile_n * BN;
   const int OH = MODE == MODE_FWD ? a.ho : a.h, OW = MODE == MODE_FWD ? a.wo : a.w;
   const int SH = MODE == MODE_FWD ? a.h : a.ho, SW = MODE == MODE_FWD ? a.w : a.wo;
-  const int tiles_x = (OW + TF_W - 1) / TF_W, tiles_y = (OH + TH - 1) / TH;
+  const int GH = S2D ? (OH - 1 + a.pt) / 2 + 1 : OH, GW = S2D ? (OW - 1 + a.pl) / 2 + 1 : OW;
+  const int tiles_x = (GW + TF_W - 1) / TF_W, tiles_y = (GH + TH - 1) / TH;
   const int b = tile_m / (tiles_x * tiles_y);
   const int trem = tile_m - b * tiles_x * tiles_y;
   const int oy0 = (trem / tiles_x) * TH, ox0 = (trem % tiles_x) * TF_W;
-  const int hy0 = MODE == MODE_FWD ? oy0 - a.pt : oy0 + a.pt - (KS - 1);
-  const int hx0 = MODE == MODE_FWD ? ox0 - a.pl : ox0 + a.pl - (KS - 1);
+  const int hy0 = S2F ? 2 * oy0 - a.pt : S2D ? oy0 - 1
+                  : MODE == MODE_FWD ? oy0 - a.pt : oy0 + a.pt - (KS - 1);
+  const int hx0 = S2F ? 2 * ox0 - a.pl : S2D ? ox0 - 1
+                  : MODE == MODE_FWD ? ox0 - a.pl : ox0 + a.pl - (KS - 1);
+  auto out_px = [&](int mt, int ph, int& oy, int& ox) {
+    const int ty = mt / TF_W, tx = mt % TF_W;
+    if constexpr (S2D) {
+      oy = 2 * (oy0 + ty) + (ph >> 1) - a.pt;
+      ox = 2 * (ox0 + tx) + (ph & 1) - a.pl;
+    } else {
+      oy = oy0 + ty;
+      ox = ox0 + tx;
+    }
+    return (unsigned)oy < (unsigned)OH && (unsigned)ox < (unsigned)OW;
+  };
+  auto clamp_px = [&](int oy, int ox) {
+    if constexpr (S2D) oy = max(oy, 0), ox = max(ox, 0);
+    return (int64_t)min(oy, OH - 1) * OW + min(ox, OW - 1);
+  };
   const int c_begin = split * a.k_per_split;
   const int c_end = min(a.K, c_begin + a.k_per_split);
 
@@ -1138,7 +1163,12 @@
     for (int j = 0; j < HS; ++j) {
       const int q = tid + NT * j;
       if (q < HQ) {
-        const int hp = q >> 3;
+        int hp = q >> 3;
+        if constexpr (S2F) {
+          const int hy = hp / HW, hx = hp - hy * HW;
+          hp = ((hy & 1) ? ((hx & 1) ? PB[1][1] : PB[1][0]) : ((hx & 1) ? PB[0][1] : PB[0][0])) +
+               (hy >> 1) * ((hx & 1) ? CW1 : CW0) + (hx >> 1);
+        }
         const int off = hp * 64 + ((((q & 7) >> 1) ^ x3_sw(hp)) << 4) + 8 * (q & 1);
         char* base = reinterpret_cast<char*>(Ah);
         if constexpr (NP == 1) {
@@ -1165,9 +1195,18 @@
     b_off[j] = ok ? (uint32_t)(((int64_t)p * a.b_plane + (int64_t)n * a.ldb + 8 * oct) * 2) : kOOB;
     b_lds[j] = o < BOCT ? (p * BN + row) * 4 + (oct ^ x3_sw(row)) : -1;
   }
+  auto tap_so = [&](int c, int t) {
+    if constexpr (S2D) {
+      const int r = t / KS, s = t % KS, ph = (r & 1) * 2 + (s & 1);
+      const int tl = (r >> 1) * (2 - (s & 1)) + (s >> 1);
+      return ((int)a.grp[ph].b_off + tl * a.kc + 32 * c) * 2;
+    } else {
+      return (t * a.kc + 32 * c) * 2;
+    }
+  };
   uint4 rb[BSL];
   auto load_b = [&](int c, int t) {
-    const int so = (t * a.kc + 32 * c) * 2;
+    const int so = tap_so(c, t);
 #pragma unroll
     for (int j = 0; j < BSL; ++j)
       rb[j] = __builtin_bit_cast(uint4, __builtin_amdgcn_raw_buffer_load_b128(rb_src, b_off[j], so, 0));
@@ -1192,29 +1231,37 @@
     bd_lds[k] = g < BDI ? (p * BN + rbk * 16) * 4 : -1;
   }
   auto dma_b = [&](int c, int t, int buf) {
-    const int so = (t * a.kc + 32 * c) * 2;
+    const int so = tap_so(c, t);
 #pragma unroll
     for (int k = 0; k < BDW; ++k)
       if (BDI % NW == 0 || bd_lds[k] >= 0)
         dma16_to_lds(rb_src, Bs + buf * NP * BN * 4 + bd_lds[k], bd_off[k], so);
   };
 
-  f32x4 acc4[SM][SN];
-#pragma unroll
-  for (int i = 0; i < SM; ++i)
-#pragma unroll
-    for (int j = 0; j < SN; ++j)
-#pragma unroll
-      for (int r = 0; r < 4; ++r) acc4[i][j][r] = 0.f;
+  f32x4 accp[NPH][SM][SN];
+#pragma unroll
+  for (int ph = 0; ph < NPH; ++ph)
+#pragma unroll
+    for (int i = 0; i < SM; ++i)
+#pragma unroll
+      for (int j = 0; j < SN; ++j)
+#pragma unroll
+        for (int r = 0; r < 4; ++r) accp[ph][i][j][r] = 0.f;
   const int wm0 = (wave / WAVES_N) * WM;
   const int wn0 = (wave % WAVES_N) * WN;
   const int l16 = lane & 15, lq = lane >> 4;
-  int a_hp16[SM];
+  int a_hp16[S2F ? 2 : 1][SM];
 #pragma unroll
   for (int i = 0; i < SM; ++i) {
     const int m = wm0 + 16 * i + l16;
     const int ty = m / TF_W, tx = m % TF_W;
-    a_hp16[i] = MODE == MODE_FWD ? ty * HW + tx : (ty + KS - 1) * HW + tx + KS - 1;
+    if constexpr (S2F) {
+      a_hp16[0][i] = ty * CW0 + tx;
+      a_hp16[1][i] = ty * CW1 + tx;
+    } else {
+      a_hp16[0][i] = S2D ? (ty + 1) * HW + tx + 1
+                     : MODE == MODE_FWD ? ty * HW + tx : (ty + KS - 1) * HW + tx + KS - 1;
+    }
   }
   const int b_frag = (wn0 + l16) * 4 + (lq ^ x3_sw(l16));
 
@@ -1241,11 +1288,14 @@
       }
       __builtin_amdgcn_sched_barrier(0);
       const int r = t / KS, s = t % KS;
-      const int dh = MODE == MODE_FWD ? r * HW + s : -(r * HW + s);
+      const int dh = S2F   ? PB[r & 1][s & 1] + (r >> 1) * ((s & 1) ? CW1 : CW0) + (s >> 1)
+                     : S2D ? -((r >> 1) * HW + (s >> 1))
+                     : MODE == MODE_FWD ? r * HW + s : -(r * HW + s);
+      f32x4 (&acc4)[SM][SN] = accp[S2D ? (r & 1) * 2 + (s & 1) : 0];
       bf16x8 av[NP][SM], bv[NP][SN];
 #pragma unroll
       for (int i = 0; i < SM; ++i) {
-        const int px = a_hp16[i] + dh;
+        const int px = a_hp16[S2F ? (s & 1) : 0][i] + dh;
         const int ai = px * 4 + (lq ^ x3_sw(px));
 #pragma unroll
         for (int p = 0; p < NP; ++p) av[p][i] = __builtin_bit_cast(bf16x8, Ah[p * HP * 4 + ai]);
@@ -1294,7 +1344,8 @@
 #pragma unroll
     for (int i = 0; i < SM; ++i)
 #pragma unroll
-      for (int j = 0; j < SN; ++j) v += acc4[i][j][0] + acc4[i][j][1] + acc4[i][j][2] + acc4[i][j][3];
+      for (int j = 0; j < SN; ++j)
+        v += accp[0][i][j][0] + accp[0][i][j][1] + accp[0][i][j][2] + accp[0][i][j][3];
     a.C[(img + (int64_t)oy0 * OW + ox0) * a.ldc + (n0 + wn0 + (lane & 31)) % a.N] = v;
     return;
   }
@@ -1303,17 +1354,17 @@
                 ((WM / 2) * (WN / 4)) % 64 == 0) {
     if (a.direct16) {
       direct_fwd_f32<SM, SN, WM, WN, TF_W>(
-          a, acc4, reinterpret_cast<char*>(smem) + wave * (WM / 2) * (WN * 4 + 32), lane, wm0,
+          a, accp[0], reinterpret_cast<char*>(smem) + wave * (WM / 2) * (WN * 4 + 32), lane, wm0,
           wn0, n0, oy0, ox0, OH, OW, img);
       return;
     }
   }
-  if constexpr (MODE == MODE_DGRAD && NT >= 512 && SM % 2 == 0 &&
+  if constexpr (MODE == MODE_DGRAD && S == 1 && NT >= 512 && SM % 2 == 0 &&
                 (NT / 64) * (WM / 2) * (WN * 4 + 32) <= LDS_B &&
                 ((WM / 2) * (WN / 4)) % 64 == 0) {
     if (a.direct16) {
       direct_dgrad_f32<SM, SN, WM, WN, TF_W>(
-          a, acc4, reinterpret_cast<char*>(smem) + wave * (WM / 2) * (WN * 4 + 32), lane, wm0,
+          a, accp[0], reinterpret_cast<char*>(smem) + wave * (WM / 2) * (WN * 4 + 32), lane, wm0,
           wn0, n0, oy0, ox0, OH, OW, img);
       return;
     }
@@ -1328,6 +1379,9 @@
 #pragma unroll
     for (int p = 0; p < NPASS; ++p) bsb[p] = bsg[p] = make_float4(0.f, 0.f, 0.f, 0.f);
 #pragma unroll
+    for (int ph = 0; ph < NPH; ++ph) {
+    f32x4 (&acc4)[SM][SN] = accp[ph];
+#pragma unroll
     for (int jp = 0; jp < SN; jp += EJ) {
 #pragma unroll
       for (int i = 0; i < SM; ++i)
@@ -1350,10 +1404,10 @@
           for (int g = 0; g < X3_EPB; ++g) {
             const int m = (q0 + g) * RPI + rr;
             v[g] = *reinterpret_cast<const float4*>(&E[m * EPW + 4 * c4]);
-            const int mt = wm0 + m;
-            const int oy = oy0 + mt / TF_W, ox = ox0 + mt % TF_W;
-            row[g] = img + (int64_t)min(oy, OH - 1) * OW + min(ox, OW - 1);
-            ok |= (oy < OH && ox < OW && n < a.N ? 1u : 0u) << g;
+            int oy, ox;
+            const bool in = out_px(wm0 + m, ph, oy, ox);
+            row[g] = img + clamp_px(oy, ox);
+            ok |= (in && n < a.N ? 1u : 0u) << g;
           }
           epilogue_rows4c<MODE, X3_EPB>(a, split, row, ok, n, min(n, a.N - 4), v);
         }
@@ -1368,9 +1422,8 @@
         for (int q = 0; q < WM / RPI; ++q) {
           const int m = q * RPI + rr;
           const float4 v = *reinterpret_cast<const float4*>(&E[m * EPW + 4 * c4]);
-          const int mt = wm0 + m;
-          const int oy = oy0 + mt / TF_W, ox = ox0 + mt % TF_W;
-          if (oy < OH && ox < OW && n < a.N)
+          int oy, ox;
+          if (out_px(wm0 + m, ph, oy, ox) && n < a.N)
             dgrad_store4_bnp(a, img + (int64_t)oy * OW + ox, n, v, bt, ig, bsb[jp / EJ],
                              bsg[jp / EJ]);
         }
@@ -1379,15 +1432,15 @@
         for (int q = 0; q < WM / RPI; ++q) {
           const int m = q * RPI + rr;
           const float4 v = *reinterpret_cast<const float4*>(&E[m * EPW + 4 * c4]);
-          const int mt = wm0 + m;
-          const int oy = oy0 + mt / TF_W, ox = ox0 + mt % TF_W;
-          if (oy < OH && ox < OW && n < a.N)
+          int oy, ox;
+          if (out_px(wm0 + m, ph, oy, ox) && n < a.N)
             epilogue_store4<MODE>(a, split, img + (int64_t)oy * OW + ox, n, v);
         }
       }
       __builtin_amdgcn_fence(__ATOMIC_RELEASE, "wavefront");
       __builtin_amdgcn_wave_barrier();
       __builtin_amdgcn_fence(__ATOMIC_ACQUIRE, "wavefront");
+    }
     }
     if (MODE == MODE_DGRAD && bnp) {
       constexpr int NWM = (NT / 64) / WAVES_N;
@@ -1427,6 +1480,8 @@
     return;
   }
 #pragma unroll
+  for (int ph = 0; ph < NPH; ++ph) {
+#pragma unroll
   for (int j = 0; j < SN; ++j) {
     const int n = n0 + wn0 + 16 * j + l16;
     if (n >= a.N) continue;
@@ -1435,29 +1490,35 @@
     EpAux aux[SM * 4];
 #pragma unroll
     for (int q = 0; q < SM * 4; ++q) {
-      const int m = wm0 + 16 * (q >> 2) + 4 * lq + (q & 3);
-      const int oy = oy0 + m / TF_W, ox = ox0 + m % TF_W;
-      aux[q] = a.splits == 1 && oy < OH && ox < OW
+      int oy, ox;
+      const bool in = out_px(wm0 + 16 * (q >> 2) + 4 * lq + (q & 3), ph, oy, ox);
+      aux[q] = a.splits == 1 && in
                    ? epilogue_aux<MODE>(a, img + (int64_t)oy * OW + ox, n) : EpAux{0.f, 0.f};
     }
 #pragma unroll
     for (int q = 0; q < SM * 4; ++q) {
-      const int m = wm0 + 16 * (q >> 2) + 4 * lq + (q & 3);
-      const int oy = oy0 + m / TF_W, ox = ox0 + m % TF_W;
-      if (oy >= OH || ox >= OW) continue;
+      int oy, ox;
+      if (!out_px(wm0 + 16 * (q >> 2) + 4 * lq + (q & 3), ph, oy, ox)) continue;
       const int64_t row = img + (int64_t)oy * OW + ox;
-      const float v = acc4[q >> 2][j][q & 3];
+      const float v = accp[ph][q >> 2][j][q & 3];
       if (a.splits > 1)
         a.slab[(int64_t)split * a.split_stride + row * a.slab_ld + n] = v;
       else
         epilogue_store<MODE>(a, row, n, v, bias, scale, shift, aux[q]);
     }
   }
+  }
 }
 
 template <int BN, int WAVES_M, int WAVES_N, int MODE, int TH, int NB = 2>
 __global__ __launch_bounds__(64 * WAVES_M * WAVES_N, NB == 1 ? 2 : 1) void conv_tile_x3(GemmArgs a) {
   tile_x3_body<BN, WAVES_M, WAVES_N, MODE, TH, NB, 3>(a);
+}
+
+template <int BN, int WAVES_M, int WAVES_N, int MODE, int TH, int NB>
+__global__ __launch_bounds__(64 * WAVES_M * WAVES_N, 2) void conv_tile_x3_s2(GemmArgs a) {
+  static_assert(WAVES_M * WAVES_N == 4, "two 4-wave workgroups per CU");
+  tile_x3_body<BN, WAVES_M, WAVES_N, MODE, TH, NB, 3, 2>(a);
 }
 
 constexpr int b16_min_waves(int w, int acc) { return w <= 8 && acc <= 48 ? (w + 1) / 2 : (w + 3) / 4; }
@@ -4742,6 +4803,58 @@
   return with_cfg(T[cfg], cfg);
 }
 
+static int g_s2_halo = 1;
+constexpr int S2_MIN_PX = 8192, S2_BN = 64, S2F_TH = 2, S2D_TH = 4;
+GemmArgs tile_s2_args(const of_conv_desc* d, const Geo& g, int mode) {
+  GemmArgs a = base_args(d);
+  const bool fwd = mode == MODE_FWD;
+  a.kc = fwd ? g.cin_p : g.cout_p;
+  a.N = fwd ? d->cout : g.cin_p;
+  a.nb = fwd ? d->cout : g.nd;
+  a.ldb = fwd ? g.kf16 : (int)g.kd16;
+  const int th = fwd ? S2F_TH : S2D_TH;
+  const int GH = fwd ? d->ho : (d->h - 1 + d->pad_top) / 2 + 1;
+  const int GW = fwd ? d->wo : (d->w - 1 + d->pad_left) / 2 + 1;
+  const int m_tiles = d->n * (int)cdiv(GH, th) * (int)cdiv(GW, TF_W);
+  a.bm = (fwd ? 1 : 4) * th * TF_W;
+  a.bn_tile = S2_BN;
+  a.ngroups = 1;
+  for (int c = 0; c < 4; ++c) {
+    a.grp[c] = Group{};
+    if (!fwd) a.grp[c].b_off = g.pg.row_begin16[c];
+  }
+  Group& G = a.grp[0];
+  G.M = fwd ? d->n * d->ho * d->wo : d->n * d->h * d->w;
+  G.m_tiles = m_tiles;
+  G.ns = 3;
+  G.ntaps = 9;
+  a.M = G.M;
+  a.n_tiles = (int)cdiv(a.N, S2_BN);
+  a.tiles_total = m_tiles * a.n_tiles;
+  a.K = (int)cdiv(a.kc, 32);
+  G.K = a.K;
+  a.k_per_split = (int)cdiv(a.K, best_split(a.K, a.tiles_total, 2 * device_cus(), g_x3t_ep));
+  a.splits = (int)cdiv(a.K, a.k_per_split);
+  return a;
+}
+bool s2_halo_ok(const of_conv_desc* d, int mode) {
+  if (!g_s2_halo || !(d->kh == 3 && d->kw == 3 && d->stride == 2)) return false;
+  if (g_s2_halo == 2) return true;
+  if ((int64_t)d->n * d->ho * d->wo < S2_MIN_PX) return false;
+  return mode == MODE_FWD || tile_s2_args(d, geo(d), MODE_DGRAD).splits == 1;
+}
+template <int MODE>
+constexpr Launch tile_x3_s2_rec() {
+  return {conv_tile_x3_s2<S2_BN, 2, 2, MODE, MODE == MODE_FWD ? S2F_TH : S2D_TH,
+                          MODE == MODE_FWD ? 1 : 2>,
+          256, kind(KIND_GEMM_X3, MODE, 0), "conv_tile_x3_s2"};
+}
+template <int MODE>
+Launch tile_x3_s2_launch(const GemmArgs& a) {
+  static const Launch L = tile_x3_s2_rec<MODE>();
+  return with_cfg(L, a.N > 64 ? 0 : 1);
+}
+
 template <int MODE>
 Launch tile_b16_launch(const GemmArgs& a) {
   static const Launch T[7] = {
@@ -4840,7 +4953,7 @@
 static int g_wgt_pf = 1;
 
 enum class Fam { narrow, gemm_f32, gemm_bf16, gemm_x3, gemm_b16, tile_bf16, tile_x3, tile_b16,
-                 tile_ws, stem };
+                 tile_ws, stem, tile_x3s2 };
 enum class WFam { narrow, stem, tile_x3, tile_b16, gemm_x3, gemm_b16, tile, gemm_bf16, gemm_f32 };
 
 Fam gemm_family(int prec, int mode) {
@@ -4856,17 +4969,20 @@
 Fam fwd_family(const of_conv_desc* d, int prec, bool plain, bool stem_kernel = true) {
   if (!prec) return narrow_ok(d) && plain ? Fam::narrow : Fam::gemm_f32;
   if (tile_ok(d)) return tile_family(d, prec, MODE_FWD);
+  if (prec == 2 && s2_halo_ok(d, MODE_FWD)) return Fam::tile_x3s2;
   if (stem_kernel && (prec == 2 || g_stem_bf16) && g_stem_x3 && stem_x3_ok(d)) return Fam::stem;
   return gemm_family(prec, MODE_FWD);
 }
-Fam dgrad_family(const of_conv_desc* d, int prec, bool bnp = false) {
+Fam dgrad_family(const of_conv_desc* d, int prec, bool bnp = false, bool s2_halo = true) {
   if (!prec) return narrow_ok(d) ? Fam::narrow : Fam::gemm_f32;
+  if (prec == 2 && s2_halo && s2_halo_ok(d, MODE_DGRAD)) return Fam::tile_x3s2;
   return tile_ok(d) ? tile_family(d, prec, MODE_DGRAD, bnp) : gemm_family(prec, MODE_DGRAD);
 }
 
 GemmArgs plan_args(const of_conv_desc* d, const Geo& g, int mode, Fam f, bool in_place = false) {
   if (f == Fam::tile_bf16 || f == Fam::tile_x3 || f == Fam::tile_b16 || f == Fam::tile_ws)
     return tile_args(d, g, mode, f == Fam::tile_x3, f == Fam::tile_b16, f == Fam::tile_ws);
+  if (f == Fam::tile_x3s2) return tile_s2_args(d, g, mode);
   const bool k16 = f != Fam::gemm_f32 && f != Fam::narrow;
   GemmArgs a = mode == MODE_FWD ? fwd_args(d, g, k16) : dgrad_args(d, g, k16, in_place);
   if (f == Fam::gemm_x3 || f == Fam::gemm_b16) gemm_x3_plan(a);
@@ -4877,6 +4993,7 @@
 int launch_family(Fam f, const GemmArgs& a, hipStream_t s, double flops) {
   switch (f) {
     case Fam::tile_x3: return launch<MODE>(tile_x3_launch<MODE>(a), a, s, flops);
+    case Fam::tile_x3s2: return launch<MODE>(tile_x3_s2_launch<MODE>(a), a, s, flops);
     case Fam::tile_ws:
       return launch<MODE>(with_cfg(tile_ws_launch(a, MODE), kind(KIND_TILE_WS, MODE, 0)), a, s, flops);
     case Fam::tile_b16: return launch<MODE>(tile_b16_launch<MODE>(a), a, s, flops);
@@ -5155,6 +5272,7 @@
   if (key == 38 && value >= 0 && value <= 131072) { g_det_lds_probe = value; return OF_OK; }
   if (key == 39 && (value == 0 || value == 1)) { g_abl_noact = value; return OF_OK; }
   if (key == 40 && (value == 0 || value == 1)) { g_wgx3b_stage = value; return OF_OK; }
+  if (key == 42 && value >= 0 && value <= 2) { g_s2_halo = value; return OF_OK; }
   return fail(OF_EINVAL, "of_set_tuning: unknown key/value " + std::to_string(key));
 }
 
@@ -5235,6 +5353,11 @@
 int of_conv_path(const of_conv_desc* d) {
   if (validate(d) != OF_OK) return -1;
   return narrow_ok(d) ? 1 : 0;
+}
+
+int of_conv_s2_halo(const of_conv_desc* d, int mode) {
+  if (validate(d) != OF_OK || (mode != MODE_FWD && mode != MODE_DGRAD)) return -1;
+  return !narrow_ok(d) && s2_halo_ok(d, mode) ? 1 : 0;
 }
 
 static int conv_fwd_impl(int prec, const of_conv_desc* d, const float* x, int ldx,
@@ -5280,7 +5403,7 @@
       if (f != Fam::gemm_bf16) gemm_x3_plan(a);
     }
   }
-  const bool tile = prec && tile_ok(d);
+  const bool tile = prec && (tile_ok(d) || f == Fam::tile_x3s2);
   if (f != Fam::stem) attach_slab(a, workspace, ws_bytes, tile ? 1 : prec ? BKH : BK);
   a.A = x;
   a.lda = ldx;
@@ -5301,7 +5424,7 @@
   hipStream_t s = as_stream(stream);
   const double flops = 2.0 * d->n * d->ho * d->wo * (double)d->cout * g.taps * d->cin;
   a.vec_ep = vec_ep_ok(a);
-  a.direct16 = f == Fam::tile_x3 && (g_x3_direct & 1) && a.splits == 1 && a.vec_ep && !residual &&
+  a.direct16 = (f == Fam::tile_x3 || f == Fam::tile_x3s2) && (g_x3_direct & 1) && a.splits == 1 && a.vec_ep && !residual &&
                !z && d->cout % 4 == 0 && ldy % 4 == 0 && ((uintptr_t)y & 15) == 0;
   if (pool) {
     if (f != Fam::stem || d->ho % 2 || d->wo % 2 || d->cout % 4)
@@ -5363,7 +5486,7 @@
                            const void* w_bwd, const float* act_src, int ld_act, int act,
                            float alpha, const float* add, int ld_add, float* dx, int lddx,
                            void* workspace, size_t ws_bytes, void* stream, int act_post = 0,
-                           const BnpArgs* bnp = nullptr) {
+                           const BnpArgs* bnp = nullptr, bool s2_halo = true) {
   int st = validate(d);
   if (st) return st;
   Geo g = geo(d);
@@ -5377,7 +5500,7 @@
   OF_CHECK_ARG(((uintptr_t)dy & 15) == 0 && ((uintptr_t)w_bwd & 15) == 0,
                "conv dgrad: dy / w must be 16-byte aligned");
   OF_CHECK_ARG(d->stride == 1 || d->stride == 2, "conv dgrad: stride must be 1 or 2");
-  const Fam f = dgrad_family(d, prec, bnp != nullptr);
+  const Fam f = dgrad_family(d, prec, bnp != nullptr, s2_halo);
   if (f == Fam::narrow) {
     OF_CHECK_ARG(!add && !act_post, "conv dgrad: the Cout <= 4 kernels take no added gradient");
     hipStream_t s = as_stream(stream);
@@ -5387,7 +5510,7 @@
     if (timing_on()) timing_end(s, kind(KIND_F32, MODE_DGRAD, KIND_NARROW), conv_flops(d));
     return st;
   }
-  const bool tile = prec && tile_ok(d);
+  const bool tile = prec && (tile_ok(d) || f == Fam::tile_x3s2);
   const bool in_place = add && add == dx && ld_add == lddx;
   GemmArgs a = plan_args(d, g, MODE_DGRAD, f, in_place);
   if (a.tiles_total == 0)
@@ -5415,11 +5538,14 @@
   a.vec_ep = vec_ep_ok(a);
   if (g_abl_noact && f == Fam::tile_x3 && !bnp) a.act_src = nullptr;
   a.direct16 = f == Fam::tile_x3 && (g_x3_direct & 2) && a.splits == 1 && a.vec_ep;
+  if (bnp && f == Fam::tile_x3s2 && !(X3_EPB == 1 && a.splits == 1 && a.vec_ep && act_src))
+    return conv_dgrad_impl(prec, d, dy, lddy, w_bwd, act_src, ld_act, act, alpha, add, ld_add, dx,
+                           lddx, workspace, ws_bytes, stream, act_post, bnp, false);
   if (bnp) {
     const int64_t m_tiles = a.n_tiles > 0 ? a.tiles_total / a.n_tiles : 0;
     int64_t rows = 0;
     for (int gq = 0; gq < a.ngroups; ++gq) rows += a.grp[gq].M;
-    const bool form = f == Fam::tile_x3 || f == Fam::tile_b16 ? X3_EPB == 1
+    const bool form = f == Fam::tile_x3 || f == Fam::tile_b16 || f == Fam::tile_x3s2 ? X3_EPB == 1
                       : f == Fam::tile_bf16 ? (bool)EPC_BATCH
                       : f == Fam::gemm_x3 && EPC_BATCH && rows == (int64_t)d->n * d->h * d->w;
     if (!(form && a.splits == 1 && a.vec_ep && act_src) ||
@@ -5482,12 +5608,18 @@
 
 size_t of_conv2d_fwd_x3_workspace(const of_conv_desc* d) {
   if (validate(d) != OF_OK || narrow_ok(d)) return 0;
-  return fd_workspace(plan_args(d, geo(d), MODE_FWD, fwd_family(d, 2, false, false)));
+  const Fam f = fwd_family(d, 2, false, false);
+  const size_t ws = fd_workspace(plan_args(d, geo(d), MODE_FWD, f));
+  if (f != Fam::tile_x3s2) return ws;
+  return std::max(ws, fd_workspace(plan_args(d, geo(d), MODE_FWD, Fam::gemm_x3)));
 }
 
 size_t of_conv2d_dgrad_x3_workspace(const of_conv_desc* d) {
   if (validate(d) != OF_OK || narrow_ok(d)) return 0;
-  return fd_workspace(plan_args(d, geo(d), MODE_DGRAD, dgrad_family(d, 2)));
+  const Fam f = dgrad_family(d, 2);
+  const size_t ws = fd_workspace(plan_args(d, geo(d), MODE_DGRAD, f));
+  if (f != Fam::tile_x3s2) return ws;
+  return std::max(ws, fd_workspace(plan_args(d, geo(d), MODE_DGRAD, Fam::gemm_x3)));
 }
 
 int of_conv2d_fwd_x3(const of_conv_desc* d, const float* x, int ldx, const void* w3_fwd,
@@ -5764,6 +5896,10 @@
     const GemmArgs a = plan_args(d, g, MODE_DGRAD, tile_ok(d) ? tiles[f] : Fam::gemm_x3, f == 1);
     if (a.n_tiles > 0) bytes = std::max(bytes, (size_t)(a.tiles_total / a.n_tiles) * 2 * a.N * 4);
   }
+  if (s2_halo_ok(d, MODE_DGRAD)) {
+    const GemmArgs a = tile_s2_args(d, g, MODE_DGRAD);
+    bytes = std::max(bytes, (size_t)(a.tiles_total / a.n_tiles) * 2 * a.N * 4);
+  }
   return bytes;
 }
 
```
